# feixh/VISMA

Hardware: AMD Instinct MI355X
Metric: icp_iterations_per_sec (higher is better)
Workload: dtype f32; 1 GPU; C4 S-surf 262144->4194304, 4040 ICP iterations of a fresh registration from T=I (cold pass + warm passes), median of 1; ns=262144, nt=4194304, solver=kabsch, nn=grid, search=exact, parallelism=1 GPU, ONE persistent launch per host loop

## Files before the change

include/visma_icp_testing.h:

```cpp
#ifndef VISMA_ICP_TESTING_H
#define VISMA_ICP_TESTING_H
#include "visma_icp.h"
#ifdef __cplusplus
extern "C" {
#endif

typedef struct {
    int (*set_source)(void *user, const float *xyzw, int64_t ns);
    int (*set_target)(void *user, const float *xyzw, int64_t nt);
    int (*set_target_normals)(void *user, const float *nxyzw, int64_t nt);
    int (*nn_pass)(void *user, const double T_centred[16], double max_dist);
    int (*reduce)(void *user, const double T_centred[16], const double frame_offset[3],
                  int point_to_plane, double stats[VISMA_ICP_NSTATS]);
    int (*get_correspondences)(void *user, int32_t *tgt_idx_per_src, float *d2);
} visma_icp_engine;
VISMA_ICP_API int visma_icp_create_with_engine(visma_icp_ctx **out,
                                               const visma_icp_engine *engine,
                                               void *user);

VISMA_ICP_API int visma_icp_get_search_kernel_used(visma_icp_ctx *ctx, int *kernel);
VISMA_ICP_API int visma_icp_forget_winners(visma_icp_ctx *ctx);

VISMA_ICP_API int visma_icp_set_device_loop(visma_icp_ctx *ctx, int enabled);

VISMA_ICP_API int visma_icp_test_stall_command(visma_icp_ctx *ctx, int nth, double ms);

VISMA_ICP_API int visma_icp_get_sweep_info(visma_icp_ctx *ctx, double *launches, double *aborts);

VISMA_ICP_API int visma_icp_plan_ring_grid(const float mn[3], const float mx[3], double max_dist, double cell, int dims[3],
                                           double *cell_out, int *rings);
VISMA_ICP_API int visma_icp_ring_visiting_order(int rings, int capacity, short *dy, short *dz, float *base, int *nrows);

VISMA_ICP_API int visma_icp_get_tile_config(int *s_tile, int *t_chunk, int *block);
VISMA_ICP_API int visma_icp_get_launch_config(visma_icp_ctx *ctx, int *src_tiles,
                                              int *tgt_splits);

VISMA_ICP_API int visma_icp_last_mesh_kernel_ms(visma_icp_ctx *ctx, double *query_ms, double *build_ms);
VISMA_ICP_API int visma_icp_set_mesh_search(visma_icp_ctx *ctx, int method);

VISMA_ICP_API int visma_icp_selftest_so3(const double *w, double *R, double *w_back, int n);
VISMA_ICP_API int visma_icp_selftest_so3_jac(const double *w, int n, double *R, double *dR_dw,
                                             double *w_back, double *dw_dR, double *proj);

VISMA_ICP_API int visma_icp_selftest_se3(const double *g, const double *h, const double *v, int n,
                                         double *gh, double *gv, double *g_inv);

#ifdef __cplusplus
}
#endif
#endif
```

visma_amd/csrc/driver.cpp:

```cpp
#include "driver_ctx.hpp"
#ifdef VISMA_TEST_SEAMS
#include "../../include/visma_icp_testing.h"
#endif

namespace {

#ifdef VISMA_TEST_SEAMS
class HookEngine : public Engine {
public:
    HookEngine(const visma_icp_engine &vt, void *user) : vt_(vt), user_(user) {}
    int set_source(const float *p, int64_t n) override { ns_ = n; return wrap(vt_.set_source(user_, p, n)); }
    int set_target(const float *p, int64_t n) override { nt_ = n; has_normals_ = false; return wrap(vt_.set_target(user_, p, n)); }
    int set_target_normals(const float *p, int64_t n) override
    {
        if (!vt_.set_target_normals) { err_ = "engine has no normals support"; return VISMA_ICP_ERR_ENGINE; }
        has_normals_ = true;
        return wrap(vt_.set_target_normals(user_, p, n));
    }
    int nn_pass(const Mat4 &Tc, double r) override { return wrap(vt_.nn_pass(user_, Tc.m, r)); }
    int reduce(const Mat4 &Tc, bool plane, const double offset[3], double *st) override
    {
        const double zero[3] = {0, 0, 0};
        return wrap(vt_.reduce(user_, Tc.m, offset ? offset : zero, plane ? 1 : 0, st));
    }
    int get_correspondences(int32_t *idx, float *d2) override
    {
        std::vector<float> tmp;
        if (!d2) { tmp.resize((size_t)(ns_ > 0 ? ns_ : 1)); d2 = tmp.data(); }
        return wrap(vt_.get_correspondences(user_, idx, d2));
    }

private:
    int wrap(int rc)
    {
        if (rc == 0) return VISMA_ICP_OK;
        err_ = "engine callback returned " + std::to_string(rc);
        return VISMA_ICP_ERR_ENGINE;
    }
    visma_icp_engine vt_;
    void *user_;
};
#endif


}

namespace {

void pack_f64_to(const double *xyz, int64_t n, int stride, const double c[3], float *out, bool par)
{
    auto body = [&](int64_t ch) {
        const int64_t lo = ch * kHostChunk, hi = std::min(n, lo + kHostChunk);
        for (int64_t i = lo; i < hi; i++) {
            const double *p = xyz + (size_t)i * stride;
            out[4 * i + 0] = (float)(p[0] - c[0]);
            out[4 * i + 1] = (float)(p[1] - c[1]);
            out[4 * i + 2] = (float)(p[2] - c[2]);
            out[4 * i + 3] = 0.f;
        }
    };
    const int64_t nch = (n + kHostChunk - 1) / kHostChunk;
    if (par) parallel_for(nch, 1, body);
    else for (int64_t ch = 0; ch < nch; ch++) body(ch);
}

int pack_f64(const double *xyz, int64_t n, int stride, const double c[3], std::vector<float> &out)
{
    out.resize((size_t)(n > 0 ? n : 1) * 4);
    pack_f64_to(xyz, n, stride, c, out.data(), false);
    return 0;
}

void pack_f32_to(const float *xyz, int64_t n, int stride, float *out)
{
    for (int64_t i = 0; i < n; i++) {
        const float *p = xyz + (size_t)i * stride;
        out[4 * i + 0] = p[0];
        out[4 * i + 1] = p[1];
        out[4 * i + 2] = p[2];
        out[4 * i + 3] = 0.f;
    }
}

void centroid_f64(const double *xyz, int64_t n, int stride, double c[3], bool par)
{
    c[0] = c[1] = c[2] = 0.0;
// ... 886 lines not shown
{
    if (!(share > 0.0) || share > 1.0) return VISMA_ICP_ERR_INVALID;
    persist_cu_share_ref().store(share);
    return VISMA_ICP_OK;
}

int visma_icp_get_persistent_info(visma_icp_ctx *ctx, visma_icp_persistent_info *out)
{
    CTX_CHECK();
    if (!out || out->struct_size < (int)sizeof(visma_icp_persistent_info))
        return ctx->fail(VISMA_ICP_ERR_INVALID, "visma_icp_persistent_info: set struct_size = sizeof(visma_icp_persistent_info)");
    const int sz = out->struct_size;
    std::memset(out, 0, sizeof(*out));
    out->struct_size = sz;
    out->cu_share = 1.0;
    ctx->eng->get_persistent_info(out);
    return VISMA_ICP_OK;
}

int visma_icp_set_ring_search(visma_icp_ctx *ctx, int mode)
{
    CTX_CHECK();
    ctx->eng->set_ring_search(mode);
    return VISMA_ICP_OK;
}

int visma_icp_get_ring_search(visma_icp_ctx *ctx, int *rings, double *cell, double *occupancy)
{
    CTX_CHECK();
    ctx->eng->get_ring_search(rings, cell, occupancy);
    return VISMA_ICP_OK;
}

int visma_icp_get_sweep_info(visma_icp_ctx *ctx, double *launches, double *aborts)
{
    CTX_CHECK();
    ctx->eng->get_sweep_info(launches, aborts);
    return VISMA_ICP_OK;
}

int visma_icp_test_stall_command(visma_icp_ctx *ctx, int nth, double ms)
{
    CTX_CHECK();
    if (nth < 0 || !(ms >= 0.0) || ms > 10000.0) return ctx->fail(VISMA_ICP_ERR_INVALID, "bad stall arguments");
    ctx->eng->stall_command(nth, ms);
    return VISMA_ICP_OK;
}

int visma_icp_set_profiling(visma_icp_ctx *ctx, int enabled)
{
    CTX_CHECK();
    ctx->eng->set_profiling(enabled);
    return VISMA_ICP_OK;
}

int visma_icp_get_timing(visma_icp_ctx *ctx, visma_icp_timing *out, int reset)
{
    CTX_CHECK();
    if (!out) return ctx->fail(VISMA_ICP_ERR_INVALID, "out is NULL");
    ctx->eng->get_timing(out, reset != 0);
    return VISMA_ICP_OK;
}

int visma_icp_get_timing_sized(visma_icp_ctx *ctx, void *out, size_t struct_size, int reset)
{
    CTX_CHECK();
    if (!out) return ctx->fail(VISMA_ICP_ERR_INVALID, "out is NULL");
    visma_icp_timing t;
    ctx->eng->get_timing(&t, reset != 0);
    std::memcpy(out, &t, struct_size < sizeof(t) ? struct_size : sizeof(t));
    return VISMA_ICP_OK;
}

int visma_icp_plan_ring_grid(const float mn[3], const float mx[3], double max_dist, double cell, int dims[3], double *cell_out, int *rings)
{
    if (!mn || !mx) return VISMA_ICP_ERR_INVALID;
    const visma::GridParams g = visma::grid_plan_ring(mn, mx, max_dist, cell, visma::kGridMaxCells);
    if (dims) for (int a = 0; a < 3; a++) dims[a] = g.dim[a];
    if (cell_out) *cell_out = (double)g.h;
    if (rings) *rings = g.ring;
    return VISMA_ICP_OK;
}

int visma_icp_ring_visiting_order(int rings, int capacity, short *dy, short *dz, float *base, int *nrows)
{
    const std::vector<visma::RingRow> rows = visma::ring_visiting_order(rings);
    if (nrows) *nrows = (int)rows.size();
    if (rows.empty()) return VISMA_ICP_ERR_INVALID;
    for (int k = 0; k < (int)rows.size() && k < capacity; k++) {
        if (dy) dy[k] = rows[k].dy;
        if (dz) dz[k] = rows[k].dz;
        if (base) base[k] = rows[k].base;
    }
    return VISMA_ICP_OK;
}

int visma_icp_get_tile_config(int *s_tile, int *t_chunk, int *block)
{
    if (s_tile) *s_tile = kSTile;
    if (t_chunk) *t_chunk = kTChunk;
    if (block) *block = kBlock;
    return VISMA_ICP_OK;
}

int visma_icp_get_launch_config(visma_icp_ctx *ctx, int *src_tiles, int *tgt_splits)
{
    CTX_CHECK();
    int a = 0, b = 0;
    ctx->eng->launch_config(&a, &b);
    if (src_tiles) *src_tiles = a;
    if (tgt_splits) *tgt_splits = b;
    return VISMA_ICP_OK;
}

int visma_icp_comm_unique_id(void *out_id)
{
    if (!out_id) return VISMA_ICP_ERR_INVALID;
    if (!g_rccl.load()) { g_create_error = g_rccl.error; return VISMA_ICP_ERR_RCCL; }
    NcclId id;
    int rc = g_rccl.GetUniqueId(&id);
    if (rc != 0) { g_create_error = "ncclGetUniqueId failed"; return VISMA_ICP_ERR_RCCL; }
    std::memcpy(out_id, &id, sizeof(id));
    return VISMA_ICP_OK;
}

int visma_icp_comm_init(visma_icp_ctx *ctx, int rank, int nranks, const void *unique_id)
{
    CTX_CHECK();
    if (!unique_id || nranks < 1 || rank < 0 || rank >= nranks) return ctx->fail(VISMA_ICP_ERR_INVALID, "bad comm arguments");
    int rc = ctx->eng->comm_init(rank, nranks, unique_id);
    if (rc) return ctx->eng_fail(rc);
    ctx->rank = rank;
    ctx->nranks = nranks;
    return VISMA_ICP_OK;
}

int visma_icp_comm_ipc_export(visma_icp_ctx *ctx, void *out_handle)
{
    CTX_CHECK();
    if (!out_handle) return ctx->fail(VISMA_ICP_ERR_INVALID, "out_handle is NULL");
    int rc = ctx->eng->ipc_export(out_handle);
    if (rc) return ctx->eng_fail(rc);
    return VISMA_ICP_OK;
}

int visma_icp_comm_ipc_init(visma_icp_ctx *ctx, int rank, int nranks, const void *handles)
{
    CTX_CHECK();
    if (!handles || nranks < 1 || rank < 0 || rank >= nranks) return ctx->fail(VISMA_ICP_ERR_INVALID, "bad comm arguments");
    int rc = ctx->eng->ipc_init(rank, nranks, handles);
    if (rc) return ctx->eng_fail(rc);
    ctx->rank = rank;
    ctx->nranks = nranks;
    return VISMA_ICP_OK;
}

int visma_icp_set_allreduce(visma_icp_ctx *ctx, visma_icp_allreduce_fn fn, void *user, int rank, int nranks)
{
    CTX_CHECK();
    if (nranks < 1 || rank < 0 || rank >= nranks) return ctx->fail(VISMA_ICP_ERR_INVALID, "bad rank arguments");
    ctx->host_allreduce = fn;
    ctx->host_allreduce_user = user;
    ctx->rank = rank;
    ctx->nranks = nranks;
    return VISMA_ICP_OK;
}
// ... 46 lines not shown
```

visma_amd/csrc/grid.hip:

```cpp
#include "device_common.h"

#include <stdlib.h>
#include <algorithm>

#include <math.h>
#include <string.h>

namespace visma {

__device__ __forceinline__ unsigned f2ord(float f)
{
    const unsigned u = __float_as_uint(f);
    return (u & 0x80000000u) ? ~u : (u | 0x80000000u);
}

__global__ void bbox_init_kernel(unsigned *box)
{
    if (threadIdx.x < 3) box[threadIdx.x] = 0xFFFFFFFFu;
    else if (threadIdx.x < 6) box[threadIdx.x] = 0u;
}

__global__ __launch_bounds__(256) void bbox_kernel(const float4 *__restrict__ pts, int n,
                                                   unsigned *__restrict__ box)
{
    float mn[3] = {INFINITY, INFINITY, INFINITY}, mx[3] = {-INFINITY, -INFINITY, -INFINITY};
    for (int i = blockIdx.x * 256 + threadIdx.x; i < n; i += gridDim.x * 256) {
        const float4 q = pts[i];
        mn[0] = fminf(mn[0], q.x); mx[0] = fmaxf(mx[0], q.x);
        mn[1] = fminf(mn[1], q.y); mx[1] = fmaxf(mx[1], q.y);
        mn[2] = fminf(mn[2], q.z); mx[2] = fmaxf(mx[2], q.z);
    }
#pragma unroll
    for (int a = 0; a < 3; a++) {
#pragma unroll
        for (int off = 32; off > 0; off >>= 1) {
            mn[a] = fminf(mn[a], __shfl_down(mn[a], off, 64));
            mx[a] = fmaxf(mx[a], __shfl_down(mx[a], off, 64));
        }
    }
    __shared__ float wmn[4][3], wmx[4][3];
    const int w = threadIdx.x >> 6;
    if ((threadIdx.x & 63) == 0) {
#pragma unroll
        for (int a = 0; a < 3; a++) { wmn[w][a] = mn[a]; wmx[w][a] = mx[a]; }
    }
    __syncthreads();
    if (threadIdx.x < 3) {
        const int a = threadIdx.x;
        const float lo = fminf(fminf(wmn[0][a], wmn[1][a]), fminf(wmn[2][a], wmn[3][a]));
        const float hi = fmaxf(fmaxf(wmx[0][a], wmx[1][a]), fmaxf(wmx[2][a], wmx[3][a]));
        atomicMin(&box[a], f2ord(lo));
        atomicMax(&box[3 + a], f2ord(hi));
    }
}

__global__ __launch_bounds__(256) void cell_count_kernel(const float4 *__restrict__ pts, int n,
                                                         GridParams g,
                                                         uint2 *__restrict__ cell_rank,
                                                         unsigned *__restrict__ count)
{
    const int i = blockIdx.x * 256 + threadIdx.x;
    if (i >= n) return;
    const float4 q = pts[i];
    int cx = cell_coord(q.x, g.mn[0], g.inv_h, g.dim[0]);
    int cy = cell_coord(q.y, g.mn[1], g.inv_hs, g.dim[1]);
    int cz = cell_coord(q.z, g.mn[2], g.inv_hs, g.dim[2]);
    cx = min(max(cx, 0), g.dim[0] - 1);
    cy = min(max(cy, 0), g.dim[1] - 1);
    cz = min(max(cz, 0), g.dim[2] - 1);
    const unsigned c = (unsigned)((cz * g.dim[1] + cy) * g.dim[0] + cx);
    cell_rank[i] = make_uint2(c, atomicAdd(&count[c], 1u));
}

constexpr int kScanPerBlock = 2048;

__global__ __launch_bounds__(256) void scan_block_sum_kernel(const unsigned *__restrict__ count,
                                                             long long n,
                                                             unsigned *__restrict__ bsum)
{
    __shared__ unsigned w[4];
    const long long base = (long long)blockIdx.x * kScanPerBlock + threadIdx.x * 8;
    unsigned s = 0;
#pragma unroll
// ... 12 lines not shown
    const int per = (nb + 1023) / 1024;
    const int lo = threadIdx.x * per, hi = min(lo + per, nb);
    unsigned s = 0;
    for (int i = lo; i < hi; i++) s += bsum[i];
    part[threadIdx.x] = s;
    __syncthreads();
    for (int off = 1; off < 1024; off <<= 1) {
        unsigned v = (threadIdx.x >= off) ? part[threadIdx.x - off] : 0u;
        __syncthreads();
        part[threadIdx.x] += v;
        __syncthreads();
    }
    unsigned run = part[threadIdx.x] - s;
    for (int i = lo; i < hi; i++) {
        const unsigned v = bsum[i];
        bsum[i] = run;
        run += v;
    }
}

__global__ __launch_bounds__(256) void scan_apply_kernel(const unsigned *__restrict__ count,
                                                         long long n,
                                                         const unsigned *__restrict__ bsum,
                                                         unsigned *__restrict__ start)
{
    __shared__ unsigned tsum[256];
    const long long base = (long long)blockIdx.x * kScanPerBlock + threadIdx.x * 8;
    unsigned v[8], s = 0;
#pragma unroll
    for (int k = 0; k < 8; k++) {
        v[k] = (base + k < n) ? count[base + k] : 0u;
        s += v[k];
    }
    tsum[threadIdx.x] = s;
    __syncthreads();
    for (int off = 1; off < 256; off <<= 1) {
        unsigned t = (threadIdx.x >= off) ? tsum[threadIdx.x - off] : 0u;
        __syncthreads();
        tsum[threadIdx.x] += t;
        __syncthreads();
    }
    unsigned run = bsum[blockIdx.x] + tsum[threadIdx.x] - s;
#pragma unroll
    for (int k = 0; k < 8; k++) {
        if (base + k < n) start[base + k] = run;
        run += v[k];
    }
    if (base <= n - 1 && n - 1 < base + 8) start[n] = run;
}

__global__ void scan_total_kernel(const unsigned *__restrict__ count, long long n, unsigned *__restrict__ start)
{
    start[n] = start[n - 1] + count[n - 1];
}

__global__ __launch_bounds__(256) void cell_scatter_kernel(const float4 *__restrict__ pts, int n,
                                                           const uint2 *__restrict__ cell_rank,
                                                           const unsigned *__restrict__ start,
                                                           float4 *__restrict__ sorted,
                                                           const Pt64 *__restrict__ pts64,
                                                           Pt64 *__restrict__ sorted64)
{
    const int i = blockIdx.x * 256 + threadIdx.x;
    if (i >= n) return;
    const uint2 cr = cell_rank[i];
    const unsigned pos = start[cr.x] + cr.y;
    const float4 q = pts[i];
    sorted[pos] = make_float4(q.x, q.y, q.z, __uint_as_float((unsigned)i));
    if (pts64) {
        Pt64 q8 = pts64[i];
        q8.w = (unsigned long long)(unsigned)i;
        sorted64[pos] = q8;
    }
}

__global__ void pack12_kernel(const float4 *__restrict__ src, float *__restrict__ dst, long long n)
{
    const long long i = (long long)blockIdx.x * blockDim.x + threadIdx.x;
    if (i < n) { const float4 p = src[i]; dst[3 * i] = p.x; dst[3 * i + 1] = p.y; dst[3 * i + 2] = p.z; }
}
hipError_t launch_pack12(const float4 *src, float *dst, int64_t n, hipStream_t stream)
{
    if (n > 0) hipLaunchKernelGGL(pack12_kernel, dim3((unsigned)((n + 255) / 256)), dim3(256), 0, stream, src, dst, (long long)n);
    return hipGetLastError();
}

hipError_t launch_grid_bbox(const float4 *tgt, int64_t nt, unsigned *box6, hipStream_t stream)
{
    hipLaunchKernelGGL(bbox_init_kernel, dim3(1), dim3(64), 0, stream, box6);
    if (nt > 0) {
        int blocks = (int)((nt + 255) / 256);
        if (blocks > 1024) blocks = 1024;
        hipLaunchKernelGGL(bbox_kernel, dim3(blocks), dim3(256), 0, stream, tgt, (int)nt, box6);
    }
    return hipGetLastError();
}

void grid_decode_bbox(const unsigned box6[6], float mn[3], float mx[3])
{
    for (int a = 0; a < 6; a++) {
        const unsigned o = box6[a];
        const unsigned u = (o & 0x80000000u) ? (o & 0x7FFFFFFFu) : ~o;
        float f;
        memcpy(&f, &u, sizeof(f));
        (a < 3 ? mn[a] : mx[a - 3]) = f;
    }
}

GridParams grid_plan(const float mn[3], const float mx[3], double max_dist, int64_t max_cells, int max_sub)
{
    GridParams g;
    float h = (float)(max_dist * 1.001);
    if (const char *e = getenv("VISMA_ICP_GRID_CELL")) {
        const double f = atof(e);
        if (f >= 1.0 && f <= 64.0) h = (float)(max_dist * 1.001 * f);
    }
    if (!(h > 0.f) || !isfinite(h)) h = 1.0f;
    double ext[3];
    for (int a = 0; a < 3; a++) {
        ext[a] = (double)mx[a] - (double)mn[a];
        if (!(ext[a] >= 0.0) || !isfinite(ext[a])) ext[a] = 0.0;
    }
    for (;;) {
        double n = 1.0;
        bool too_long = false;
        for (int a = 0; a < 3; a++) {
            double d = floor(ext[a] / h) + 1.0;
            if (d > 2.0e9) d = 2.0e9;
            if (d > (double)kGridMaxDim) too_long = true;
            g.dim[a] = (int)d;
            n *= d;
        }
        if (n <= (double)max_cells && !too_long) break;
        h *= 1.26f;
    }
    g.sub = 1;
    if (max_sub >= 2) {
        const double dy = floor(ext[1] / (0.5 * h)) + 1.0, dz = floor(ext[2] / (0.5 * h)) + 1.0;
        if ((double)g.dim[0] * dy * dz <= (double)kGridMaxCellsFine) {
            g.sub = 2;
            g.dim[1] = (int)dy;
            g.dim[2] = (int)dz;
        }
    }
    for (int a = 0; a < 3; a++) g.mn[a] = mn[a];
    g.h = h;
    g.inv_h = 1.0f / h;
    g.hs = g.sub == 2 ? 0.5f * h : h;
    g.inv_hs = 1.0f / g.hs;
    g.ncell = (int64_t)g.dim[0] * g.dim[1] * g.dim[2];
    g.ring = 0;
    return g;
}

GridParams grid_plan_ring(const float mn[3], const float mx[3], double max_dist, double cell, int64_t max_cells)
{
    GridParams g = grid_plan(mn, mx, max_dist, max_cells);
    float h = (float)cell;
    if (!(h > 0.f) || !isfinite(h) || !(h < g.h)) return g;
    h = std::max(h, (float)(max_dist * 1.001 / (double)(kRingMaxRings - 2)));
    double ext[3];
    for (int a = 0; a < 3; a++) {
        ext[a] = (double)mx[a] - (double)mn[a];
        if (!(ext[a] >= 0.0) || !isfinite(ext[a])) ext[a] = 0.0;
    }
    GridParams f = g;
// ... 536 lines not shown
                    w8.w = 0xFFFFFFFFull | lbw;
                    if (bpos != 0xFFFFFFFFu) { w8 = sorted64[bpos]; w8.w = (w8.w & 0xFFFFFFFFull) | lbw; }
                    prevq_out[i] = w8;
                }
            }
            if constexpr (S64) {
#ifdef VISMA_GRID_DEBUG_TRIPS
                {
                    int wmax = dbg_trips, wmax_m = bpos == 0xFFFFFFFFu ? 0 : dbg_trips;
                    for (int m = 32; m > 0; m >>= 1) {
                        wmax = max(wmax, __shfl_xor(wmax, m, 64));
                        wmax_m = max(wmax_m, __shfl_xor(wmax_m, m, 64));
                    }
                    idx_out[i] = dbg_trips | ((bpos != 0xFFFFFFFFu) << 7) | (wmax << 8) | (wmax_m << 16);
                }
#else
                idx_out[i] = (bpos == 0xFFFFFFFFu) ? -1 : (int)bidx;
#endif
                d2_out[i] = (float)bd;
                if (d64_out) d64_out[i] = bd;
            } else {
                idx_out[i] = (bpos == 0xFFFFFFFFu) ? -1 : (int)(unsigned)bkey;
                d2_out[i] = __uint_as_float((unsigned)(bkey >> 32));
            }
        }
        if ((it % G) == sub) { keep_s = s4; keep_i = i; keep_pos = bpos; }
        if constexpr (KEEPQ) { keep_p[0] = pxd; keep_p[1] = pyd; keep_p[2] = pzd; }
        if (!ONE && (it % G) == G - 1) flush();
    }
    flush();
    block_reduce_store<NACC>(acc, partials, fold.tickets != nullptr);
    if (cand_count) {
        unsigned long long c = ncand, ca = ncand_all;
#pragma unroll
        for (int o = 32; o > 0; o >>= 1) {
            c += __shfl_down(c, o, 64);
            ca += __shfl_down(ca, o, 64);
        }
        if ((threadIdx.x & 63) == 0 && ca) {
            unsigned long long *slot = cand_count + 2 * (blockIdx.x & 4095);
            atomicAdd(slot, c);
            atomicAdd(slot + 1, ca);
        }
    }
    if (fold.tickets) fused_fold<PLANE, kBlock, false, kSolveInFold>(fold, partials, row0, lb, bpp, prob);
}

template <bool PLANE, int G, int U>
static void launch_grid_t(int nblocks, hipStream_t stream, const float4 *src, int ns,
                          const float4 *sorted, const unsigned *start, const GridParams &g,
                          const float4 *nrm, const Xform32 &T32, const Xform64 &T64,
                          const Offset64 &off, float r2f, int *idx_out, float *d2_out,
                          double *partials, unsigned long long *cand, const DevIcpState *st,
                          int nprob, long long out_stride, const Pt64 *src64, const Pt64 *sorted64, double r2d,
                          const Pt64 *nrm64, int exact, const FoldArgs &fold, double *d64_out, Pt64 *prevq_out)
{
    const long long total_groups = (long long)nblocks * (kBlock / G);
    const bool one = ((long long)ns + total_groups - 1) / total_groups <= G;
#define VISMA_GRID_LAUNCH(ONE_, F64_, HYB_)                                                                     \
    hipLaunchKernelGGL((nn_grid_reduce_kernel<PLANE, G, U, ONE_, F64_, HYB_>), dim3(nblocks * nprob),             \
                       dim3(kBlock), 0, stream, src, ns, sorted, start, g, nrm, T32, T64, off, r2f, idx_out,      \
                       d2_out, partials, cand, st, nblocks, out_stride, (const ProbDesc *)nullptr, nprob, src64,  \
                       sorted64, r2d, nrm64, fold, d64_out, prevq_out)
    if (src64 && exact) {
        if (one) VISMA_GRID_LAUNCH(true, false, true); else VISMA_GRID_LAUNCH(false, false, true);
    } else if (src64) {
        if (one) VISMA_GRID_LAUNCH(true, true, false); else VISMA_GRID_LAUNCH(false, true, false);
    } else {
        if (one) VISMA_GRID_LAUNCH(true, false, false); else VISMA_GRID_LAUNCH(false, false, false);
    }
#undef VISMA_GRID_LAUNCH
}

hipError_t launch_nn_grid_reduce(const float4 *src, int64_t ns, const float4 *sorted,
                                 const unsigned *start, const GridParams &g,
                                 const float4 *tgt_normals, const Xform32 &T32, const Xform64 &T64,
                                 const double frame_offset[3], float r2f, int point_to_plane,
                                 int32_t *idx_out, float *d2_out, double *partials,
                                 int max_partial_blocks, int *nblocks_out, int lanes_per_query,
                                 unsigned long long *cand_count, const DevIcpState *st,
                                 int nprob, int64_t out_stride, hipStream_t stream, const Pt64 *src64,
                                 const Pt64 *sorted64, double r2d, const Pt64 *nrm64, int exact,
                                 const FoldArgs *fold, double *d64_out, Pt64 *prevq_io, int warm, const Xform64 *Tprev,
                                 const PersistArgs *persist, Pt64 *ru_io, const RingTable *ring)
{
    if ((src64 == nullptr) != (sorted64 == nullptr)) return hipErrorInvalidValue;
    if (persist && !(lanes_per_query == kCoopLanes && src64 && exact && g.sub == 1 && prevq_io)) return hipErrorInvalidValue;
    Offset64 off;
    for (int a = 0; a < 3; a++) off.v[a] = frame_offset ? frame_offset[a] : 0.0;
    const FoldArgs fa = fold ? *fold : FoldArgs{};
    const int G = lanes_per_query % 100;
    int U = lanes_per_query / 100;
    if (U == 0) U = (G >= 8) ? 2 : 4;
    int64_t want = (ns * G + kBlock - 1) / kBlock;
    int nblocks = (int)(want > max_partial_blocks ? max_partial_blocks : want);
    if (nblocks < 1) nblocks = 1;
    if (g.ring > 0) {
        if (!src64 || persist || !ring) return hipErrorInvalidValue;
        hipError_t e = launch_nn_ring(G, nblocks, nprob, (int)ns, src64, sorted64, exact ? (const float *)sorted : nullptr, start, g,
                                      *ring, tgt_normals, nrm64, T64, off, r2f,
                                      point_to_plane, idx_out, d2_out, d64_out, prevq_io, warm & 1, partials, cand_count, st,
                                      (long long)out_stride, fa, stream);
        if (nblocks_out) *nblocks_out = nblocks;
        return e;
    }
    if (lanes_per_query == kCoopLanes) {
        if (src64 && exact && g.sub == 1 && prevq_io) {
            const bool one = (ns + (int64_t)nblocks * kBlock - 1) / ((int64_t)nblocks * kBlock) <= 1;
            hipError_t e = launch_nn_coop(nblocks * nprob, nblocks, nprob, nullptr, (int)ns, (const float *)sorted, start, g,
                                          tgt_normals, nrm64, T64, off, r2f, point_to_plane, one ? 1 : 0, idx_out, d2_out,
                                          partials, cand_count, st, (long long)out_stride, src64, sorted64, fa, d64_out,
                                          prevq_io, warm, stream, Tprev, persist, ru_io);
            if (nblocks_out) *nblocks_out = nblocks;
            return e;
        }
        U = 8;
    }
#define VISMA_GRID_CASE(GG, UU)                                                                    \
    if (G == GG && U == UU) {                                                                      \
        if (point_to_plane)                                                                        \
            launch_grid_t<true, GG, UU>(nblocks, stream, src, (int)ns, sorted, start, g,           \
                                        tgt_normals, T32, T64, off, r2f, idx_out, d2_out,          \
                                        partials, cand_count, st, nprob, (long long)out_stride, src64, sorted64, r2d, nrm64, exact, fa, d64_out, prevq_io);   \
        else                                                                                       \
            launch_grid_t<false, GG, UU>(nblocks, stream, src, (int)ns, sorted, start, g,          \
                                         tgt_normals, T32, T64, off, r2f, idx_out, d2_out,         \
                                         partials, cand_count, st, nprob, (long long)out_stride, src64, sorted64, r2d, nrm64, exact, fa, d64_out, prevq_io);  \
        launched = true;                                                                           \
    }
    bool launched = false;
    VISMA_GRID_CASE(1, 8) VISMA_GRID_CASE(1, 12) VISMA_GRID_CASE(2, 4) VISMA_GRID_CASE(2, 8)
    VISMA_GRID_CASE(4, 8) VISMA_GRID_CASE(8, 4)
    if (!launched) return hipErrorInvalidValue;
#undef VISMA_GRID_CASE
    if (nblocks_out) *nblocks_out = nblocks;
    return hipGetLastError();
}

template <int G, int U, bool ONE, bool F64, bool HYB, bool PLANE = false>
static void launch_grid_batch_t(int total_blocks, hipStream_t stream, const float4 *src,
                                const float4 *sorted, const unsigned *start, const ProbDesc *descs,
                                int nprob, int *idx_out, float *d2_out, double *partials,
                                const DevIcpState *st, const Pt64 *src64, const Pt64 *sorted64, const FoldArgs &fold,
                                unsigned long long *cand, const float4 *nrm = nullptr, const Pt64 *nrm64 = nullptr,
                                Pt64 *prevq_out = nullptr)
{
    const Xform32 T32{};
    const Xform64 T64{};
    const Offset64 off{};
    const GridParams g{};
    hipLaunchKernelGGL((nn_grid_reduce_kernel<PLANE, G, U, ONE, F64, HYB>), dim3(total_blocks), dim3(kBlock), 0, stream,
                       src, 0, sorted, start, g, nrm, T32, T64, off, 0.f, idx_out,
                       d2_out, partials, cand, st, 1, 0ll, descs, nprob, src64, sorted64, 0.0,
                       nrm64, fold, (double *)nullptr, prevq_out);
}

hipError_t launch_nn_grid_reduce_batch(const float4 *src, const float4 *sorted, const unsigned *start,
                                       const ProbDesc *descs, int nprob, int total_blocks,
                                       int32_t *idx_out, float *d2_out, double *partials,
                                       int lanes_per_query, int one_per_lane, const DevIcpState *st,
                                       hipStream_t stream, const Pt64 *src64, const Pt64 *sorted64, int exact,
                                       const FoldArgs *fold, unsigned long long *cand_count,
                                       const float4 *nrm, const Pt64 *nrm64, Pt64 *prevq_io, int warm)
{
    if (!st || !descs || (src64 == nullptr) != (sorted64 == nullptr)) return hipErrorInvalidValue;
    const bool plane = nrm != nullptr || nrm64 != nullptr;
    if (plane && src64 && !exact) return hipErrorInvalidValue;
    const FoldArgs fa = fold ? *fold : FoldArgs{};
    const int G = lanes_per_query % 100;
    int U = lanes_per_query / 100;
    if (lanes_per_query == kCoopLanes) {
        if (src64 && exact && prevq_io) {
            const Xform64 T64{};
            const Offset64 off{};
            const GridParams g{};
            return launch_nn_coop(total_blocks, 1, nprob, descs, 0, (const float *)sorted, start, g, nrm, nrm64, T64, off,
                                  0.f, plane ? 1 : 0, one_per_lane, idx_out, d2_out, partials, cand_count, st, 0ll, src64,
                                  sorted64, fa, nullptr, prevq_io, warm, stream);
        }
        U = 8;
    }
    bool launched = false;
#define VISMA_BATCH_ARGS total_blocks, stream, src, sorted, start, descs, nprob, idx_out, d2_out, partials, st
#define VISMA_BATCH_CASE(GG, UU)                                                                              \
    if (G == GG && U == UU && plane) {                                                                        \
        if (src64 && one_per_lane)                                                                            \
            launch_grid_batch_t<GG, UU, true, false, true, true>(VISMA_BATCH_ARGS, src64, sorted64, fa, cand_count, nrm, nrm64, prevq_io);   \
        else if (src64)                                                                                       \
            launch_grid_batch_t<GG, UU, false, false, true, true>(VISMA_BATCH_ARGS, src64, sorted64, fa, cand_count, nrm, nrm64, prevq_io);  \
        else if (one_per_lane)                                                                                \
            launch_grid_batch_t<GG, UU, true, false, false, true>(VISMA_BATCH_ARGS, nullptr, nullptr, fa, cand_count, nrm, nrm64, prevq_io); \
        else                                                                                                  \
            launch_grid_batch_t<GG, UU, false, false, false, true>(VISMA_BATCH_ARGS, nullptr, nullptr, fa, cand_count, nrm, nrm64, prevq_io); \
        launched = true;                                                                                      \
    } else if (G == GG && U == UU) {                                                                          \
// ... 23 lines not shown
```

visma_amd/csrc/grid_coop.hip:

```cpp
#include <cstdlib>

#include "device_common.h"
#include "grid_coop_probe.h"

namespace visma {

namespace {

struct P12 { float x, y, z; };
#ifndef VISMA_COOP_RU
#define VISMA_COOP_RU 0
#endif
#ifndef VISMA_COOP_CAP
#define VISMA_COOP_CAP (VISMA_COOP_RU ? 344 : 352)
#endif
constexpr bool kCoopRu = VISMA_COOP_RU != 0;
constexpr int kCoopCap = VISMA_COOP_CAP;
#ifndef VISMA_COOP_DEPTH
#define VISMA_COOP_DEPTH 7
#endif
constexpr int kCoopDepth = VISMA_COOP_DEPTH;
#ifndef VISMA_COOP_ROOM
#define VISMA_COOP_ROOM 0.04f
#endif
constexpr float kCoopRoom = VISMA_COOP_ROOM;

__device__ __forceinline__ float octet_min(float d)
{
    float r;
    asm volatile("s_nop 1\n\t"
                 "v_min_f32_dpp %0, %1, %1 quad_perm:[1,0,3,2] row_mask:0xf bank_mask:0xf\n\t"
                 "s_nop 1\n\t"
                 "v_min_f32_dpp %0, %0, %0 quad_perm:[2,3,0,1] row_mask:0xf bank_mask:0xf\n\t"
                 "s_nop 1\n\t"
                 "v_min_f32_dpp %0, %0, %0 row_half_mirror row_mask:0xf bank_mask:0xf"
                 : "=&v"(r)
                 : "v"(d));
    return r;
}

__device__ __forceinline__ unsigned pack_sec(float sec, float third, unsigned lane)
{
    if constexpr (!kCoopRu) return __float_as_uint(sec);
    return (__float_as_uint(sec) & 0xFFFF0000u) | (((__float_as_uint(third) >> 18) & 0x1FFFu) << 3) | (lane & 7u);
}
__device__ __forceinline__ float sec_of(unsigned w) { return __uint_as_float(kCoopRu ? (w & 0xFFFF0000u) : w); }
[[maybe_unused]] __device__ __forceinline__ float third_of(unsigned w) { return __uint_as_float(((w >> 3) & 0x1FFFu) << 18); }

__device__ __forceinline__ unsigned wave_scan_incl(unsigned v, int)
{
    v += (unsigned)__builtin_amdgcn_update_dpp(0, (int)v, 0x111, 0xf, 0xf, false);
    v += (unsigned)__builtin_amdgcn_update_dpp(0, (int)v, 0x112, 0xf, 0xf, false);
    v += (unsigned)__builtin_amdgcn_update_dpp(0, (int)v, 0x114, 0xf, 0xf, false);
    v += (unsigned)__builtin_amdgcn_update_dpp(0, (int)v, 0x118, 0xf, 0xf, false);
    v += (unsigned)__builtin_amdgcn_update_dpp(0, (int)v, 0x142, 0xa, 0xf, false);
    v += (unsigned)__builtin_amdgcn_update_dpp(0, (int)v, 0x143, 0xc, 0xf, false);
    return v;
}

}

struct CoopRes {
    double (*q64)[3];
    float *idx;
    float *lb;
    float *lb3;
    int first;
    double sx, sy, sz;
    int have_src;
};

template <int NTH>
__device__ __forceinline__ void coop_query_range(int ns, int bpp, int lb, int tid, int &vb, int &per_group, long long &i_begin,
                                                 long long &i_end)
{
    vb = lb;
    if ((bpp & 7) == 0) vb = (lb & 7) * (bpp >> 3) + (lb >> 3);
    const int total_groups = bpp * NTH;
    per_group = (ns + total_groups - 1) / total_groups;
    const int gid = vb * NTH + tid;
    i_begin = (long long)gid * per_group;
    i_end = i_begin + per_group < ns ? i_begin + per_group : ns;
}

template <bool PLANE, bool ONE, int NTH, bool PERSIST = false>
__device__ __forceinline__ bool coop_body(
    int ns, const float *__restrict__ s12f, const unsigned *__restrict__ start, GridParams g,
    const float4 *__restrict__ nrm, Xform64 T64, Offset64 off, float r2f, int *__restrict__ idx_out,
    float *__restrict__ d2_out, double *__restrict__ partials, unsigned long long *__restrict__ cand_count,
    const DevIcpState *__restrict__ st, int bpp, long long out_stride, const ProbDesc *__restrict__ descs,
    int nprob, const Pt64 *__restrict__ src64, const Pt64 *__restrict__ sorted64,
    const Pt64 *__restrict__ nrm64, const FoldArgs &fold, double *__restrict__ d64_out,
    Pt64 *__restrict__ wst_io, int warm, Xform64 Tprev, Pt64 *__restrict__ ru_io, unsigned *work_out = nullptr,
    const CoopRes res = CoopRes{})
{
    constexpr int NACC = Acc<PLANE>::N;
    const P12 *s12 = reinterpret_cast<const P12 *>(s12f);
    int prob, lb;
    long long row0;
    if (descs) {
        if (warm & 2) {
            prob = reinterpret_cast<const int *>(descs + nprob)[blockIdx.x];
        } else {
            int lo = 0, hi = nprob - 1;
            while (lo < hi) {
                const int mid = (lo + hi + 1) >> 1;
                if (descs[mid].first_block <= (int)blockIdx.x) lo = mid; else hi = mid - 1;
            }
            prob = lo;
        }
        const ProbDesc d = descs[prob];
        lb = (int)blockIdx.x - d.first_block;
        bpp = d.nblocks;
        src64 += d.src_off;
        ns = d.ns;
        s12 += d.sorted_off;
        sorted64 += d.sorted_off;
        if constexpr (PLANE) {
            if (nrm) nrm += d.sorted_off;
            if (nrm64) nrm64 += d.sorted_off;
        }
        row0 = d.first_block;
        start += d.start_off;
        g = d.g;
        out_stride = 0;
        idx_out += d.out_off;
        d2_out += d.out_off;
        wst_io += d.out_off;
        if (ru_io) ru_io += d.out_off;
    } else {
        prob = blockIdx.x / bpp;
        lb = blockIdx.x - prob * bpp;
        row0 = (long long)prob * bpp;
    }
    if (st) st += prob;
    {
        Xform32 T32_unused;
        if (!load_loop_state(st, T32_unused, T64, off, r2f)) return false;
        if (st) {
            warm &= ~4;
            if (st->have_prev && !(warm & 8)) {
                warm |= 4;
#pragma unroll
                for (int k = 0; k < 12; k++) Tprev.m[k] = st->Tc_prev[k];
            }
        }
        if (!(warm & 1)) warm &= ~4;
    }
    const double r2d = (double)r2f;
    COOP_PROBE_BEGIN();
    idx_out += (long long)prob * out_stride;
    d2_out += (long long)prob * out_stride;
    wst_io += (long long)prob * out_stride;
    if (ru_io) ru_io += (long long)prob * out_stride;
    double acc[NACC];
#pragma unroll
    for (int a = 0; a < NACC; a++) acc[a] = 0.0;

    const int tid = thread_number<PERSIST, NTH>(), lane = tid & 63, wave = tid >> 6;
    const int oct = lane >> 3, l8 = lane & 7;
    constexpr int NW = NTH / 64;
    constexpr unsigned kCapAll = (unsigned)(NW * kCoopCap);
    int vb, per_group;
    long long i_begin, i_end;
    coop_query_range<NTH>(ns, bpp, lb, tid, vb, per_group, i_begin, i_end);

    __shared__ float4 s_qp[NTH];
    __shared__ uint2 s_item[kCapAll];
    __shared__ unsigned s_sec[kCapAll];
    __shared__ double s_p64[NTH][3];
    __shared__ double s_q64_own[PERSIST ? 1 : NTH][3];
    __shared__ float s_dprev_own[PERSIST ? 1 : NTH];
    double (*s_q64)[3] = s_q64_own;
    float *s_dprev = s_dprev_own;
    if constexpr (PERSIST) { s_q64 = res.q64; s_dprev = res.idx; }
    __shared__ unsigned short s_home[NTH];
    __shared__ unsigned s_need[NW];
    __shared__ unsigned s_m[NW];
    __shared__ unsigned short s_queue[NW][64];

    auto emit = [&](long long i, unsigned ht, bool cert, double bd, unsigned bidx, bool found, double qx, double qy, double qz,
                    float lb_new) {
        if constexpr (PERSIST) {
            res.lb[ht] = lb_new;
            return;
        }
        const unsigned long long lbw = (unsigned long long)__float_as_uint(lb_new) << 32;
        idx_out[i] = found ? (int)bidx : -1;
        if (cert) {
            reinterpret_cast<unsigned *>(&wst_io[i].w)[1] = __float_as_uint(lb_new);
        } else {
            Pt64 o8;
            o8.x = o8.y = o8.z = __longlong_as_double(-1ll);
            o8.w = 0xFFFFFFFFull | lbw;
            if (found) { o8.x = qx; o8.y = qy; o8.z = qz; o8.w = (unsigned long long)bidx | lbw; }
            wst_io[i] = o8;
        }
        d2_out[i] = (float)bd;
        if (d64_out) d64_out[i] = bd;
    };
    auto emit_ru = [&](long long i, unsigned ht, bool have, double ux, double uy, double uz, unsigned uidx, float lb3) {
        if constexpr (kCoopRu) {
            if (!ru_io) return;
            Pt64 o8;
            o8.x = o8.y = o8.z = __longlong_as_double(-1ll);
            o8.w = ~0ull;
            if (have) { o8.x = ux; o8.y = uy; o8.z = uz; o8.w = (unsigned long long)uidx | ((unsigned long long)__float_as_uint(lb3) << 32); }
            ru_io[i] = o8;
            if constexpr (PERSIST) res.lb3[ht] = have ? lb3 : __uint_as_float(0xFFFFFFFFu);
        }
    };
    auto query_p = [&](unsigned h, double (&out)[3]) { out[0] = s_p64[h][0]; out[1] = s_p64[h][1]; out[2] = s_p64[h][2]; };
    auto moments = [&](double pxd, double pyd, double pzd, unsigned bidx, double qx, double qy, double qz) {
        double nx = 0.0, ny = 0.0, nz = 0.0;
        if (PLANE) {
            if (nrm64) { const Pt64 n8 = nrm64[bidx]; nx = n8.x; ny = n8.y; nz = n8.z; }
            else { const float4 n4 = nrm[bidx]; nx = n4.x; ny = n4.y; nz = n4.z; }
        }
        accumulate_pq_d<PLANE>(acc, pxd, pyd, pzd, qx, qy, qz, nx, ny, nz, off);
    };
    auto list_rows = [&](const float px, const float py, const float pz, const float E, const float bound0, const bool want,
                         unsigned (&xb)[9], unsigned (&xe)[9], float &lbgeo2, unsigned &looked) {
        const int cx = cell_coord(px, g.mn[0], g.inv_h, g.dim[0]);
        const int cy = cell_coord(py, g.mn[1], g.inv_hs, g.dim[1]);
        const int cz = cell_coord(pz, g.mn[2], g.inv_hs, g.dim[2]);
        const int x0 = max(cx - 1, 0), x1 = min(cx + 1, g.dim[0] - 1);
        const int span = x1 + 1 - x0;
        typedef unsigned u4a __attribute__((ext_vector_type(4), aligned(4)));
        const bool yok[3] = {cy - 1 >= 0 && cy - 1 < g.dim[1], cy >= 0 && cy < g.dim[1], cy + 1 >= 0 && cy + 1 < g.dim[1]};
        const bool zok[3] = {cz - 1 >= 0 && cz - 1 < g.dim[2], cz >= 0 && cz < g.dim[2], cz + 1 >= 0 && cz + 1 < g.dim[2]};
        const int row_c = (cz * g.dim[1] + cy) * g.dim[0] + x0, pitch_y = g.dim[0], pitch_z = g.dim[1] * g.dim[0];
        auto load_row = [&](int k, bool wanted) {
            const bool ok = wanted && span > 0 && zok[k / 3] && yok[k % 3];
            u4a v = {0u, 0u, 0u, 0u};
            if (ok) v = *reinterpret_cast<const u4a *>(reinterpret_cast<const char *>(start) + (unsigned)(row_c + (k / 3 - 1) * pitch_z + (k % 3 - 1) * pitch_y) * 4u);
            return v;
        };
        const float fx = (px - g.mn[0]) * g.inv_h - (float)cx;
        const float fy = (py - g.mn[1]) * g.inv_hs - (float)cy;
        const float fz = (pz - g.mn[2]) * g.inv_hs - (float)cz;
        const float mgn = 1e-3f + 4.0f * E * g.inv_hs;
        const float lo_x = fmaxf(fx - mgn, 0.f), hi_x = fmaxf(1.0f - fx - mgn, 0.f);
        const float lo_y = fmaxf(fy - mgn, 0.f), hi_y = fmaxf(1.0f - fy - mgn, 0.f);
// ... 153 lines not shown
                float lb3 = __uint_as_float((unsigned)(u8.w >> 32));
                if constexpr (PERSIST) { if (!res.first) lb3 = res.lb3[tid]; }
                const float t3 = (lb3 - del) * (1.0f - 2.4e-7f);
                if (ru_io && active && has_w && has_u) {
                    if (cert) {
                        if constexpr (PERSIST) res.lb3[tid] = t3;
                        else reinterpret_cast<unsigned *>(&ru_io[i].w)[1] = __float_as_uint(t3);
                    } else if (lb_old > 0.f && t3 > 0.f) {
                        const unsigned uidx = (unsigned)u8.w;
                        const double dx = u8.x - hp[0], dy = u8.y - hp[1], dz = u8.z - hp[2];
                        double d2u = dx * dx;
                        d2u += dy * dy;
                        d2u += dz * dz;
                        const bool u_wins = d2u < d2w || (d2u == d2w && uidx < widx);
                        const double dm = u_wins ? d2u : d2w, dother = u_wins ? d2w : d2u;
                        if (dm < r2d && dm < (double)t3 * (double)t3 * (1.0 - 1e-6)) {
                            cert = true;
                            const float lbn = fminf(t3, sqrtf((float)dother) * (1.0f - 1e-6f));
                            if (u_wins) {
                                const Pt64 ow = w8;
                                w8.x = u8.x; w8.y = u8.y; w8.z = u8.z;
                                w8.w = (unsigned long long)uidx | ((unsigned long long)__float_as_uint(lbn) << 32);
                                widx = uidx;
                                emit_ru(i, (unsigned)tid, true, ow.x, ow.y, ow.z, (unsigned)ow.w, t3);
                                if constexpr (!PERSIST) wst_io[i] = w8;
                            } else {
                                if constexpr (PERSIST) res.lb3[tid] = t3;
                                else reinterpret_cast<unsigned *>(&ru_io[i].w)[1] = __float_as_uint(t3);
                            }
                            emit(i, (unsigned)tid, true, dm, widx, true, w8.x, w8.y, w8.z, lbn);
                        }
                    }
                } else if (ru_io && active && cert) {
                    if constexpr (PERSIST) res.lb3[tid] = __uint_as_float(0xFFFFFFFFu);
                }
            }
        }
        const bool need = active && !cert;
        const bool cfound = cert && has_w;
        s_p64[tid][0] = hp[0]; s_p64[tid][1] = hp[1]; s_p64[tid][2] = hp[2];
        if (need) {
            const float dp = sqdist_f32(make_float4((float)w8.x, (float)w8.y, (float)w8.z, 0.f), (float)hp[0], (float)hp[1], (float)hp[2]);
            const float sq = sqrtf(dp) + kCoopRoom * sqrtf(r2f);
            s_dprev[tid] = sq * sq;
        } else {
            s_q64[tid][0] = w8.x; s_q64[tid][1] = w8.y; s_q64[tid][2] = w8.z;
            s_dprev[tid] = __uint_as_float(cfound ? widx : 0xFFFFFFFFu);
        }
        if (cand_count) {
            const unsigned cc = (unsigned)__builtin_popcountll(__builtin_amdgcn_ballot_w64(cert));
            if (lane == 0 && cc) atomicAdd(cand_count + 2 * 4096 + (blockIdx.x & 4095), (unsigned long long)cc);
        }
        const unsigned long long needers = __builtin_amdgcn_ballot_w64(need);
        const unsigned rank = (unsigned)__builtin_popcountll(needers & ((1ull << lane) - 1ull));
        if (need) s_queue[wave][rank] = (unsigned short)tid;
        if (lane == 0) s_need[wave] = (unsigned)__builtin_popcountll(needers);
        COOP_MARK(9);
        __syncthreads();
        COOP_MARK(10);
        set_phase_prio(1);
        unsigned nq_all = 0;
        unsigned home = 0;
#pragma unroll
        for (int w = 0; w < NW; w++) {
            const unsigned c = (unsigned)__builtin_amdgcn_readfirstlane((int)s_need[w]);
            if ((unsigned)tid >= nq_all && (unsigned)tid < nq_all + c) home = s_queue[w][(unsigned)tid - nq_all];
            nq_all += c;
        }
        const bool searching = (unsigned)(wave * 64) < nq_all;
        const bool sact = (unsigned)tid < nq_all;
        if (nq_all != 0u) {
            unsigned xb[9], xe[9];
            float lbgeo2 = 0.f;
            unsigned nq = 0, off_q = 0;
            if (searching) {
                s_home[tid] = (unsigned short)home;
                double hq[3];
                query_p(home, hq);
                const double pxd = hq[0], pyd = hq[1], pzd = hq[2];
                const float dprev = sact ? s_dprev[home] : __uint_as_float(~0u);
                const float px = (float)pxd, py = (float)pyd, pz = (float)pzd;
                COOP_MARK(0);
                const float rup = sqrtf(r2f) * (1.0f + 2.4e-7f);
                const float E = 2.4e-7f * (fabsf(px) + fabsf(py) + fabsf(pz) + rup) + 4.8e-7f * rup;
                const float tlim = rup + 2.0f * E;
                const float L = tlim * tlim * (1.0f + 6e-7f);
                const float W = (4.0f * E * tlim + 4.0f * E * E) * (1.0f + 1e-6f) + L * 5e-7f;
                s_qp[tid] = make_float4(px, py, pz, W);
                float bound0 = L;
                if (dprev < L) bound0 = dprev;
                unsigned looked;
                list_rows(px, py, pz, E, bound0, sact, xb, xe, lbgeo2, looked);
                asm volatile("" : "+v"(lbgeo2));
                if (cand_count) {
                    unsigned long long c = 0, ca = looked;
#pragma unroll
                    for (int k = 0; k < 9; k++) c += xe[k] - xb[k];
#pragma unroll
                    for (int o = 32; o > 0; o >>= 1) {
                        c += __shfl_down(c, o, 64);
                        ca += __shfl_down(ca, o, 64);
                    }
#ifndef VISMA_COOP_LB_PROBE
                    if (lane == 0 && ca) {
                        unsigned long long *slot = cand_count + 2 * (blockIdx.x & 4095);
                        atomicAdd(slot, c);
                        atomicAdd(slot + 1, ca);
                    }
#endif
                }
                COOP_MARK(1);
#pragma unroll
                for (int k = 0; k < 9; k++) nq += (xe[k] - xb[k] + 7u) >> 3;
                const unsigned incl = wave_scan_incl(nq, lane);
                off_q = incl - nq;
                if (lane == 63) s_m[wave] = incl;
            } else {
                if (lane == 0) s_m[wave] = 0u;
            }
            __syncthreads();
            unsigned m_all = 0;
#pragma unroll
            for (int w = 0; w < NW; w++) {
                const unsigned c = (unsigned)__builtin_amdgcn_readfirstlane((int)s_m[w]);
                if (w < wave) off_q += c;
                m_all += c;
            }
            if (work_out) *work_out = nq_all | (m_all << 12);
            float gh0 = INFINITY, gh1 = INFINITY, gh2 = INFINITY;
            float gsec = INFINITY;
            unsigned gb0 = 0xFFFFFFFFu, gb1 = 0xFFFFFFFFu, gm0 = 0u, gm1 = 0u;
            unsigned gs0 = 0x7F800000u | (0x1FE0u << 3);
            auto chunk_insert = [&](float m, unsigned b, unsigned flags, unsigned side) {
                const bool c1 = m < gh0, c2 = m < gh1;
                gh2 = __builtin_amdgcn_fmed3f(gh1, gh2, m);
                gh1 = __builtin_amdgcn_fmed3f(gh0, gh1, m);
                gh0 = fminf(gh0, m);
                gb1 = c2 ? b : gb1; gm1 = c2 ? flags : gm1;
                gb1 = c1 ? gb0 : gb1; gm1 = c1 ? gm0 : gm1;
                gb0 = c1 ? b : gb0; gm0 = c1 ? flags : gm0;
                if constexpr (kCoopRu) gs0 = c1 ? side : gs0;
            };
            for (unsigned w0 = 0; w0 < m_all; w0 += kCapAll) {
                if (searching) {
                    const unsigned own = (unsigned)tid << 4;
                    unsigned j = off_q - w0;
#pragma unroll
                    for (int k = 0; k < 9; k++) {
                        unsigned b = xb[k];
                        while (b < xe[k]) {
                            if (j < kCapAll) s_item[j] = make_uint2(b, own | (min(xe[k] - b, 8u) << 16));
                            j++;
                            b += 8u;
                        }
                    }
                    COOP_MARK(2);
                }
                __syncthreads();
                set_phase_prio(2);
                const unsigned mw = min(m_all - w0, kCapAll);
                for (unsigned tb = 0; tb < mw; tb += (unsigned)(NW * 8 * kCoopDepth)) {
                    const unsigned t = tb + (unsigned)(wave * 8 + oct);
                    P12 c4[kCoopDepth];
                    unsigned meta[kCoopDepth];
#pragma unroll
                    for (int u = 0; u < kCoopDepth; u++) {
                        const unsigned c = t + (unsigned)(u * NW * 8);
                        uint2 dsc = make_uint2(0u, 0u);
                        if (c < mw) dsc = s_item[c];
                        meta[u] = dsc.y;
                        c4[u] = *reinterpret_cast<const P12 *>(reinterpret_cast<const char *>(s12) + (((dsc.x * 3u) << 2) + (unsigned)l8 * 12u));
                    }
#pragma unroll
                    for (int u = 0; u < kCoopDepth; u++) {
                        const unsigned c = t + (unsigned)(u * NW * 8);
                        const unsigned cnt = meta[u] >> 16;
                        const float4 p = *reinterpret_cast<const float4 *>(reinterpret_cast<const char *>(s_qp) + (meta[u] & 0xFFF0u));
                        float d = sqdist_f32(make_float4(c4[u].x, c4[u].y, c4[u].z, 0.f), p.x, p.y, p.z);
                        const bool mine = (unsigned)l8 < cnt;
                        d = mine ? d : INFINITY;
                        const float m = octet_min(d);
                        const bool fl = d <= m + p.w;
                        const unsigned long long bal = __builtin_amdgcn_ballot_w64(fl);
                        const unsigned flags = (unsigned)(bal >> (oct * 8)) & 0xFFu;
                        const float dn = fl ? INFINITY : d;
                        const float sec = octet_min(dn);
                        unsigned secl = 0u;
                        float third = INFINITY;
                        if constexpr (kCoopRu) {
                            const unsigned long long bs = __builtin_amdgcn_ballot_w64(dn == sec && sec < INFINITY);
                            const unsigned b8 = (unsigned)(bs >> (oct * 8)) & 0xFFu;
                            secl = b8 ? (unsigned)__builtin_ctz(b8) : 0u;
                            third = octet_min((b8 != 0u && (unsigned)l8 == secl) ? INFINITY : dn);
                        }
                        if (l8 == 0 && mine) {
                            s_item[c].y = (__float_as_uint(m) & 0xFFFFFF00u) | flags;
                            s_sec[c] = pack_sec(sec, third, secl);
                        }
                    }
                }
                if (searching) COOP_MARK(3);
                __syncthreads();
                set_phase_prio(3);
                if (searching) {
                    for (unsigned c0 = 0; __builtin_amdgcn_ballot_w64(c0 < nq) != 0ull; c0 += 4u) {
                        uint2 r[4];
                        unsigned rs[4];
                        bool in[4];
#pragma unroll
                        for (int u = 0; u < 4; u++) {
                            const unsigned j = off_q - w0 + c0 + (unsigned)u;
                            in[u] = c0 + (unsigned)u < nq && j < kCapAll;
                            r[u] = s_item[in[u] ? j : 0u];
                            rs[u] = s_sec[in[u] ? j : 0u];
                        }
#pragma unroll
                        for (int u = 0; u < 4; u++) {
                            chunk_insert(in[u] ? __uint_as_float(r[u].y & 0xFFFFFF00u) : INFINITY, r[u].x, r[u].y & 0xFFu, rs[u]);
                            gsec = fminf(gsec, in[u] ? sec_of(rs[u]) : INFINITY);
                        }
                    }
                    COOP_MARK(4);
                }
                if (w0 + kCapAll < m_all) __syncthreads();
            }
            if constexpr (kCoopRu) __syncthreads();
            if (searching) {
                const bool need = sact, active = sact;
                float lb_new = 0.f;
                double bd = r2d;
                unsigned bidx = 0xFFFFFFFFu, bpos = 0xFFFFFFFFu;
                Pt64 bq = Pt64{0.0, 0.0, 0.0, 0ull};
                auto tail = [&](const double pxd, const double pyd, const double pzd, const float px, const float py, const float pz,
                                const float W) {
                const float rup = sqrtf(r2f) * (1.0f + 2.4e-7f);
                const float E = 2.4e-7f * (fabsf(px) + fabsf(py) + fabsf(pz) + rup) + 4.8e-7f * rup;
                const float tlim = rup + 2.0f * E;
                const float L = tlim * tlim * (1.0f + 6e-7f);
                auto rank = [&](const Pt64 &c8, unsigned pos) {
                    const double dx = c8.x - pxd, dy = c8.y - pyd, dz = c8.z - pzd;
                    double d = dx * dx;
                    d += dy * dy;
                    d += dz * dz;
                    const unsigned id = (unsigned)c8.w;
                    const bool lt = d < bd || (d == bd && id < bidx && bidx != 0xFFFFFFFFu);
                    bd = lt ? d : bd;
                    bidx = lt ? id : bidx;
                    bpos = lt ? pos : bpos;
                    bq.x = lt ? c8.x : bq.x; bq.y = lt ? c8.y : bq.y; bq.z = lt ? c8.z : bq.z; bq.w = lt ? c8.w : bq.w;
                };
                bool slow = false;
                const float g_up = gh0 * (1.0f + 6.2e-5f);
                int n = 0;
                unsigned rupos = 0xFFFFFFFFu;
                float lb3_2 = 0.f;
                if (need && gh0 < L) {
                    const float thr = g_up + W;
                    unsigned c[4] = {0u, 0u, 0u, 0u};
                    slow = gh2 <= thr;
                    auto add = [&](unsigned b, unsigned flags) {
                        while (flags) {
                            const unsigned pos = b + (unsigned)__builtin_ctz(flags);
                            flags &= flags - 1u;
                            if (n == 0) c[0] = pos; else if (n == 1) c[1] = pos; else if (n == 2) c[2] = pos; else if (n == 3) c[3] = pos;
                            else slow = true;
                            n++;
                        }
                    };
                    add(gb0, gm0);
                    if (gh1 <= thr) add(gb1, gm1);
                    if constexpr (kCoopRu) {
                        if (ru_io && n == 1 && !slow) {
                            const float secA = sec_of(gs0);
                            if (secA < INFINITY && secA <= gh1) {
                                rupos = gb0 + (gs0 & 7u);
                                lb3_2 = fminf(gh1, third_of(gs0));
                            } else if (gh1 < INFINITY && __builtin_popcount(gm1) == 1) {
                                rupos = gb1 + (unsigned)__builtin_ctz(gm1);
                                lb3_2 = fminf(gh2, gsec);
                            }
                            lb3_2 = fminf(lb3_2, lbgeo2);
                        }
                    }
                    Pt64 c8a = Pt64{0.0, 0.0, 0.0, 0ull}, c8b = c8a;
                    if (n > 0) c8a = sorted64[c[0]];
                    if (n > 1) c8b = sorted64[c[1]];
                    if (n > 0) rank(c8a, c[0]);
                    if (n > 1) rank(c8b, c[1]);
                    if (n > 2) rank(sorted64[c[2]], c[2]);
                    if (n > 3) rank(sorted64[c[3]], c[3]);
                }
                for (unsigned long long rem = __builtin_amdgcn_ballot_w64(slow); rem; rem &= rem - 1ull) {
                    const int q = (int)__builtin_ctzll(rem);
                    auto bcast_u = [&](unsigned v) { return (unsigned)__builtin_amdgcn_readlane((int)v, q); };
                    auto bcast_f = [&](float v) { return __uint_as_float(bcast_u(__float_as_uint(v))); };
                    auto bcast_d = [&](double v) {
                        const unsigned long long u = (unsigned long long)__double_as_longlong(v);
                        return __longlong_as_double((long long)(((unsigned long long)bcast_u((unsigned)(u >> 32)) << 32) | bcast_u((unsigned)u)));
                    };
                    const float qx = bcast_f(px), qy = bcast_f(py), qz = bcast_f(pz);
                    const double qxd = bcast_d(pxd), qyd = bcast_d(pyd), qzd = bcast_d(pzd);
                    const float qrup = rup, qE = bcast_f(E);
                    const float sl = fminf(sqrtf(bcast_f(g_up)), qrup) + 2.0f * qE;
                    const float Ls = sl * sl * (1.0f + 6e-7f);
                    unsigned qb[9], pre[10];
                    pre[0] = 0u;
                    {
                        unsigned sb[9], se[9], looked_unused;
                        float geo_unused;
                        list_rows(px, py, pz, E, Ls, lane == q, sb, se, geo_unused, looked_unused);
        #pragma unroll
                        for (int k = 0; k < 9; k++) {
                            qb[k] = bcast_u(sb[k]);
                            pre[k + 1] = pre[k] + (bcast_u(se[k]) - qb[k]);
                        }
                    }
                    double ld = r2d;
                    unsigned lid = 0xFFFFFFFFu, lpos = 0xFFFFFFFFu;
                    Pt64 lq = Pt64{0.0, 0.0, 0.0, 0ull};
                    for (unsigned f0 = 0; f0 < pre[9]; f0 += 128u) {
                        unsigned j[2];
                        bool in[2];
                        P12 t[2];
        #pragma unroll
                        for (int u = 0; u < 2; u++) {
                            const unsigned f = f0 + (unsigned)u * 64u + (unsigned)lane;
                            in[u] = f < pre[9];
                            unsigned jj = 0u;
        #pragma unroll
                            for (int k = 0; k < 9; k++)
                                if (f >= pre[k] && f < pre[k + 1]) jj = qb[k] + (f - pre[k]);
                            j[u] = jj;
                            t[u] = P12{0.f, 0.f, 0.f};
                            if (in[u]) t[u] = s12[jj];
                        }
                        Pt64 c8[2];
        #pragma unroll
                        for (int u = 0; u < 2; u++) {
                            in[u] = in[u] && sqdist_f32(make_float4(t[u].x, t[u].y, t[u].z, 0.f), qx, qy, qz) <= Ls;
                            c8[u] = Pt64{0.0, 0.0, 0.0, 0ull};
                            if (in[u]) c8[u] = sorted64[j[u]];
                        }
        #pragma unroll
                        for (int u = 0; u < 2; u++)
                            if (in[u]) {
                                const double dx = c8[u].x - qxd, dy = c8[u].y - qyd, dz = c8[u].z - qzd;
                                double d = dx * dx;
                                d += dy * dy;
                                d += dz * dz;
                                const unsigned id = (unsigned)c8[u].w;
                                const bool lt = d < ld || (d == ld && id < lid && lid != 0xFFFFFFFFu);
                                if (lt) { ld = d; lid = id; lpos = j[u]; lq = c8[u]; }
                            }
                    }
                    double rd = ld;
                    unsigned rid = lid;
        #pragma unroll
                    for (int o = 32; o > 0; o >>= 1) {
                        const double od = __shfl_xor(rd, o, 64);
                        const unsigned oid = (unsigned)__shfl_xor((int)rid, o, 64);
                        const bool lt = oid != 0xFFFFFFFFu && (od < rd || (od == rd && oid < rid));
                        rd = lt ? od : rd;
                        rid = lt ? oid : rid;
                    }
                    if (rid != 0xFFFFFFFFu) {
                        const unsigned long long holders = __builtin_amdgcn_ballot_w64(lid == rid && ld == rd);
                        const int wl = (int)__builtin_ctzll(holders);
                        auto from_w = [&](unsigned v) { return (unsigned)__builtin_amdgcn_readlane((int)v, wl); };
                        auto from_w64 = [&](unsigned long long u) { return ((unsigned long long)from_w((unsigned)(u >> 32)) << 32) | from_w((unsigned)u); };
                        Pt64 w8;
                        w8.x = __longlong_as_double((long long)from_w64((unsigned long long)__double_as_longlong(lq.x)));
                        w8.y = __longlong_as_double((long long)from_w64((unsigned long long)__double_as_longlong(lq.y)));
                        w8.z = __longlong_as_double((long long)from_w64((unsigned long long)__double_as_longlong(lq.z)));
                        w8.w = from_w64(lq.w);
                        const unsigned wpos = from_w(lpos);
                        if (lane == q) {
                            const bool lt = rd < bd || (rd == bd && rid < bidx && bidx != 0xFFFFFFFFu);
                            if (lt) { bd = rd; bidx = rid; bpos = wpos; bq = w8; }
                        }
                    }
                }
                if (need) {
                    float lb2 = fminf(lbgeo2, fminf(gh1, gsec));
                    if (bpos == 0xFFFFFFFFu) lb2 = fminf(lb2, gh0);
                    float lb = sqrtf(lb2) * (1.0f - 1e-6f) - 4.0f * E;
                    if (slow || n > 1) lb = 0.f;
                    lb_new = fminf(fmaxf(lb, 0.f), 3.0e38f);
#ifdef VISMA_COOP_LB_PROBE
                    if (cand_count && bpos != 0xFFFFFFFFu && !(slow || n > 1)) {
                        const float cb = fminf(gh1, gsec);
                        if (cb < lbgeo2) {
                            unsigned long long *slot = cand_count + 2 * (blockIdx.x & 4095);
                            atomicAdd(slot, (unsigned long long)((sqrtf(fminf(lbgeo2, 4.0f * r2f)) - sqrtf(cb)) * 1e6f));
                            atomicAdd(slot + 1, 1ull);
                        }
                    }
#endif
                }
                const bool found = bpos != 0xFFFFFFFFu;
                COOP_MARK(5);
                if (active) {
                    const long long i = (long long)(vb * NTH + (int)s_home[tid]) * per_group + it;
                    emit(i, (unsigned)s_home[tid], false, bd, bidx, found, bq.x, bq.y, bq.z, lb_new);
                    if constexpr (kCoopRu) {
                        const float lb3 = sqrtf(lb3_2) * (1.0f - 1e-6f) - 4.0f * E;
                        const bool have = found && rupos != 0xFFFFFFFFu && !(slow || n > 1) && lb3 > 0.f && lb_new > 0.f;
                        if (ru_io) s_item[s_home[tid]] = make_uint2(have ? rupos : 0xFFFFFFFFu, __float_as_uint(fminf(lb3, 3.0e38f)));
                    }
                }
                if (active) {
                    const unsigned h = s_home[tid];
                    const double none = __longlong_as_double(-1ll);
                    s_q64[h][0] = found ? bq.x : none; s_q64[h][1] = found ? bq.y : none; s_q64[h][2] = found ? bq.z : none;
                    s_dprev[h] = __uint_as_float(found ? bidx : 0xFFFFFFFFu);
                }
                };
                const float4 me = s_qp[tid];
                const unsigned h = s_home[tid];
                double hq[3];
                query_p(h, hq);
                tail(hq[0], hq[1], hq[2], me.x, me.y, me.z, me.w);
                COOP_MARK(11);
            }
        }
        __syncthreads();
        COOP_MARK(12);
        set_phase_prio(4);
        if constexpr (kCoopRu) {
            ru_go = false;
            if (ru_io && ((needers >> lane) & 1ull)) {
                const uint2 h = s_item[tid];
                ru_go = true;
                ru_it = it;
                ru_lb3 = __uint_as_float(h.y);
                ru_have = h.x != 0xFFFFFFFFu;
                if (ru_have) ru_pending = sorted64[h.x];
            }
        }
        {
            const unsigned pidx = __float_as_uint(s_dprev[tid]);
            if (active && pidx != 0xFFFFFFFFu) {
                double hq[3];
                query_p((unsigned)tid, hq);
                moments(hq[0], hq[1], hq[2], pidx, s_q64[tid][0], s_q64[tid][1], s_q64[tid][2]);
            }
        }
        if constexpr (!ONE) {
            ru_finish();
            __syncthreads();
        }
    };
    if constexpr (ONE) {
        round(0);
        COOP_MARK(13);
    } else {
        for (int it = 0; it < per_group; it++) round(it);
    }
    COOP_MARK(6);
    COOP_WAVE_DONE();
    bool published = false;
    if constexpr (PERSIST) {
        const unsigned tag = fold_row_tag(fold.seq);
        block_reduce_store<NACC, NW, true>(acc, partials, true, fold.rows_tagged, tag);
        ru_finish();
        COOP_MARK(7);
        published = polled_fold<PLANE, NTH>(fold, lb, bpp, tag);
    } else {
        block_reduce_store<NACC, NW, false>(acc, partials, fold.tickets != nullptr);
        if constexpr (ONE) ru_finish();
        COOP_MARK(7);
        if (fold.tickets) published = fused_fold<PLANE, NTH, false, false>(fold, partials, row0, lb, bpp, prob);
    }
    COOP_MARK(8);
    return published;
}

#define VISMA_COOP_PARAMS                                                                                         \
    int ns, const float *__restrict__ s12f, const unsigned *__restrict__ start, GridParams g,                    \
        const float4 *__restrict__ nrm, Xform64 T64, Offset64 off, float r2f, int *__restrict__ idx_out,         \
        float *__restrict__ d2_out, double *__restrict__ partials, unsigned long long *__restrict__ cand_count,  \
        const DevIcpState *__restrict__ st, int bpp, long long out_stride, const ProbDesc *__restrict__ descs,   \
        int nprob, const Pt64 *__restrict__ src64, const Pt64 *__restrict__ sorted64,                            \
        const Pt64 *__restrict__ nrm64, const FoldArgs fold, double *__restrict__ d64_out,                       \
        Pt64 *__restrict__ wst_io, int warm, Xform64 Tprev, Pt64 *__restrict__ ru_io
#define VISMA_COOP_ARGS                                                                                          \
    ns, s12f, start, g, nrm, T64, off, r2f, idx_out, d2_out, partials, cand_count, st, bpp, out_stride, descs,   \
        nprob, src64, sorted64, nrm64, fold, d64_out, wst_io, warm, Tprev, ru_io
template <bool PLANE>
__global__ __launch_bounds__(kBlock) __attribute__((amdgpu_waves_per_eu(4, 4))) void nn_coop_kernel_one(VISMA_COOP_PARAMS)
{
    (void)coop_body<PLANE, true, kBlock>(VISMA_COOP_ARGS);
}
template <bool PLANE>
__global__ __launch_bounds__(kBlock) void nn_coop_kernel_many(VISMA_COOP_PARAMS)
{
    (void)coop_body<PLANE, false, kBlock>(VISMA_COOP_ARGS);
}

__device__ __forceinline__ unsigned long long persist_wait(const PersistArgs &pa, unsigned tag, bool poller, int pass, int lane)
{
    const bool mine = lane < kPersistWords;
    unsigned long long w = 0ull;
    const bool direct = pa.direct != 0;
    if (poller && lane == 0)
        __hip_atomic_store(pa.relay + kPersistPublished, (unsigned long long)tag, __ATOMIC_RELAXED, __HIP_MEMORY_SCOPE_AGENT);
    long long t_ref = (long long)wall_clock64();
    bool published = poller;
    for (;;) {
        if (mine) {
            if (poller || direct) w = __hip_atomic_load(pa.host_cmd + lane, __ATOMIC_RELAXED, __HIP_MEMORY_SCOPE_SYSTEM);
            else w = __hip_atomic_load(pa.relay + lane, __ATOMIC_RELAXED, __HIP_MEMORY_SCOPE_AGENT);
        }
        const bool ok = !mine || (unsigned)(w >> 32) == tag;
        if (__builtin_amdgcn_ballot_w64(ok) == ~0ull) break;
        const long long now = (long long)wall_clock64();
        bool all_here = true, dead = false;
        if (!published) {
            const unsigned long long m = __hip_atomic_load(pa.relay + kPersistPublished, __ATOMIC_RELAXED, __HIP_MEMORY_SCOPE_AGENT);
            if ((unsigned)m == tag) { published = true; t_ref = now; }
            else {
                all_here = __hip_atomic_load(pa.relay + kPersistStarted, __ATOMIC_RELAXED, __HIP_MEMORY_SCOPE_AGENT) >= (unsigned long long)gridDim.x;
                dead = __hip_atomic_load(pa.relay + kPersistDead, __ATOMIC_RELAXED, __HIP_MEMORY_SCOPE_AGENT) != 0ull;
            }
        }
        const long long limit = published ? pa.wait_ticks : (!all_here ? (pa.start_ticks > 0 ? pa.start_ticks : pa.wait_ticks) : pa.hard_ticks);
        if (dead || now - t_ref > limit) {
            w = ((unsigned long long)tag << 32) | (lane == kPersistWords - 1 ? kPersistAbort : 0u);
            if (lane == 0) {
                __hip_atomic_store(pa.relay + kPersistDead, 1ull, __ATOMIC_RELAXED, __HIP_MEMORY_SCOPE_AGENT);
                __hip_atomic_store(pa.host_flag, (unsigned)pass, __ATOMIC_RELAXED, __HIP_MEMORY_SCOPE_SYSTEM);
            }
            break;
        }
#ifndef VISMA_PERSIST_SLEEP
#define VISMA_PERSIST_SLEEP 1
#endif
        if (poller) __builtin_amdgcn_s_sleep(1); else __builtin_amdgcn_s_sleep(VISMA_PERSIST_SLEEP);
    }
    if (poller && mine && !direct) __hip_atomic_store(pa.relay + lane, w, __ATOMIC_RELAXED, __HIP_MEMORY_SCOPE_AGENT);
    return w;
}

struct CoopPersistParams {
    int ns; const float *s12f; const unsigned *start; GridParams g; const float4 *nrm; Xform64 T64; Offset64 off; float r2f;
    int *idx_out; float *d2_out; double *partials; unsigned long long *cand_count; int bpp; const Pt64 *src64;
    const Pt64 *sorted64; const Pt64 *nrm64; FoldArgs fold; Pt64 *wst_io; int warm; Xform64 Tprev; PersistArgs pa;
    Pt64 *ru_io;
};

template <class T>
__device__ __forceinline__ T ld_karg(const T __attribute__((address_space(4))) *p)
{
    static_assert(sizeof(T) % 4 == 0, "words");
    constexpr int N = (int)(sizeof(T) / 4);
    union U { T v; unsigned w[N]; __device__ U() {} } u;
    typedef const unsigned __attribute__((address_space(4))) *WordPtr;
    const WordPtr pw = (WordPtr)p;
#pragma unroll
    for (int k = 0; k < N; k++) u.w[k] = pw[k];
    return u.v;
}

template <bool PLANE>
__global__ __launch_bounds__(kBlock) __attribute__((amdgpu_waves_per_eu(4, 4))) void nn_coop_kernel_persist(const CoopPersistParams P)
{
    __shared__ unsigned s_tw[2][24];
    __shared__ unsigned s_cmdw;
    __shared__ double r_q64[kBlock][3];
    __shared__ float r_idx[kBlock], r_lb[kBlock], r_lb3[kCoopRu ? kBlock : 1];
    if (threadIdx.x == 0) {
        __hip_atomic_fetch_add(P.pa.relay + kPersistStarted, 1ull, __ATOMIC_RELAXED, __HIP_MEMORY_SCOPE_AGENT);
#pragma unroll
        for (int k = 0; k < 12; k++) {
            const unsigned long long c = (unsigned long long)__double_as_longlong(P.T64.m[k]);
            const unsigned long long q = (unsigned long long)__double_as_longlong(P.Tprev.m[k]);
            s_tw[0][2 * k] = (unsigned)c; s_tw[0][2 * k + 1] = (unsigned)(c >> 32);
            s_tw[1][2 * k] = (unsigned)q; s_tw[1][2 * k + 1] = (unsigned)(q >> 32);
        }
    }
    __syncthreads();
    typedef const CoopPersistParams __attribute__((address_space(4))) *KernargPtr;
#ifndef VISMA_PERSIST_PREFETCH
#define VISMA_PERSIST_PREFETCH 1
#endif
    double nsx = 0.0, nsy = 0.0, nsz = 0.0;
    const int tag_shift = P.pa.wait_first ? 1 : 0;
    if (P.pa.wait_first) {
        const int tidx = thread_number<true>();
        if (tidx < 64) {
            const unsigned long long cw = persist_wait(P.pa, P.pa.tag0, blockIdx.x == 0, 0, tidx);
            if (tidx < 24) s_tw[0][tidx] = (unsigned)cw;
            if (tidx == kPersistWords - 1) s_cmdw = (unsigned)cw;
        }
        __syncthreads();
        if ((unsigned)__builtin_amdgcn_readfirstlane((int)s_cmdw) != kPersistGo) return;
    }
    for (int pass = 1;; pass++) {
        KernargPtr kp = (KernargPtr)__builtin_amdgcn_kernarg_segment_ptr();
        asm volatile("" : "+s"(kp));
#define VISMA_KARG(F_) ld_karg(&kp->F_)
        const unsigned long long t_begin = VISMA_KARG(pa.timeline) ? wall_clock64() : 0ull;
        unsigned work = 0u;
        const int cur = (pass - 1) & 1;
        Xform64 Tc, Tp;
#pragma unroll
        for (int k = 0; k < 12; k++) {
            const unsigned lo = (unsigned)__builtin_amdgcn_readfirstlane((int)s_tw[cur][2 * k]);
            const unsigned hi = (unsigned)__builtin_amdgcn_readfirstlane((int)s_tw[cur][2 * k + 1]);
            Tc.m[k] = __longlong_as_double((long long)(((unsigned long long)hi << 32) | lo));
            Tp.m[k] = 0.0;
        }
        if (pass == 1 || !VISMA_PERSIST_PP_LDS) {
#pragma unroll
            for (int k = 0; k < 12; k++) {
                const unsigned plo = (unsigned)__builtin_amdgcn_readfirstlane((int)s_tw[cur ^ 1][2 * k]);
                const unsigned phi = (unsigned)__builtin_amdgcn_readfirstlane((int)s_tw[cur ^ 1][2 * k + 1]);
                Tp.m[k] = __longlong_as_double((long long)(((unsigned long long)phi << 32) | plo));
            }
        }
        int w = VISMA_KARG(warm);
        if (pass > 1) { w |= 1; if (!(w & 8)) w |= 4; }
        FoldArgs f{};
        f.tickets = VISMA_KARG(fold.tickets); f.partials2 = VISMA_KARG(fold.partials2);
        f.ticket_stride = VISMA_KARG(fold.ticket_stride); f.stats_out = VISMA_KARG(fold.stats_out);
        f.stats_stride = VISMA_KARG(fold.stats_stride); f.host_out = VISMA_KARG(fold.host_out);
        f.seq = VISMA_KARG(fold.seq) + (unsigned long long)(pass - 1);
        f.ipc_n = VISMA_KARG(fold.ipc_n); f.ipc_rank = VISMA_KARG(fold.ipc_rank); f.ipc_seq_dev = VISMA_KARG(fold.ipc_seq_dev);
        f.ipc_flag = VISMA_KARG(fold.ipc_flag); f.ipc_spins = VISMA_KARG(fold.ipc_spins); f.peer_table = VISMA_KARG(fold.peer_table);
        f.rows_tagged = VISMA_KARG(fold.rows_tagged); f.rows2_tagged = VISMA_KARG(fold.rows2_tagged);
        f.dead_flag = VISMA_KARG(fold.dead_flag); f.poll_ticks = VISMA_KARG(fold.poll_ticks);
        const bool published = coop_body<PLANE, true, kBlock, true>(
            VISMA_KARG(ns), VISMA_KARG(s12f), VISMA_KARG(start), VISMA_KARG(g), VISMA_KARG(nrm), Tc, VISMA_KARG(off), VISMA_KARG(r2f),
            VISMA_KARG(idx_out), VISMA_KARG(d2_out), VISMA_KARG(partials), VISMA_KARG(cand_count), nullptr, VISMA_KARG(bpp), 0ll,
            nullptr, 1, VISMA_KARG(src64), VISMA_KARG(sorted64), VISMA_KARG(nrm64), f, nullptr, VISMA_KARG(wst_io), w, Tp,
            VISMA_KARG(ru_io), t_begin ? &work : nullptr, CoopRes{r_q64, r_idx, r_lb, r_lb3, pass == 1 ? 1 : 0, nsx, nsy, nsz,
                                                                        (VISMA_PERSIST_PREFETCH && pass > 1) ? 1 : 0});
        const PersistArgs pa = VISMA_KARG(pa);
        if (pa.timeline && pass <= pa.timeline_passes && thread_number<true>() == 0) {
            unsigned long long *slot = pa.timeline + ((unsigned long long)(pass - 1) * gridDim.x + blockIdx.x) * 2ull;
            slot[0] = t_begin;
            slot[1] = (wall_clock64() & 0xFFFFFFFFFFFull) | ((unsigned long long)work << 44);
        }
        bool last = pass >= pa.max_passes;
        nsx = nsy = nsz = 0.0;
        if (VISMA_PERSIST_PREFETCH && !last) {
            const int tidx = thread_number<true>();
            const int bpp = VISMA_KARG(bpp);
            int vb, per_group;
            long long i_begin, i_end;
            coop_query_range<kBlock>(VISMA_KARG(ns), bpp, (int)blockIdx.x % bpp, tidx, vb, per_group, i_begin, i_end);
            if (i_begin < i_end) {
                const Pt64 s8 = VISMA_KARG(src64)[i_begin];
                nsx = s8.x; nsy = s8.y; nsz = s8.z;
            }
        }
        if (!last) {
            const int tidx = thread_number<true>();
            if (tidx < 64) {
                const bool poller = __builtin_amdgcn_readfirstlane((int)published) != 0;
                const unsigned long long cw = persist_wait(pa, pa.tag0 + (unsigned)(pass - 1 + tag_shift), poller, pass, tidx);
                if (tidx < 24) s_tw[cur ^ 1][tidx] = (unsigned)cw;
                if (tidx == kPersistWords - 1) s_cmdw = (unsigned)cw;
            }
            __syncthreads();
            asm volatile("" : "+v"(nsx), "+v"(nsy), "+v"(nsz));
            const unsigned cmd = (unsigned)__builtin_amdgcn_readfirstlane((int)s_cmdw);
            last = cmd != kPersistGo;
        }
        if (last) {
            const int tidx = thread_number<true>();
            const int bpp = VISMA_KARG(bpp);
            int vb, per_group;
            long long i_begin, i_end;
            coop_query_range<kBlock>(VISMA_KARG(ns), bpp, (int)blockIdx.x % bpp, tidx, vb, per_group, i_begin, i_end);
            if (i_begin < i_end) {
                const unsigned pid = __float_as_uint(r_idx[tidx]);
                Pt64 o8;
                o8.x = r_q64[tidx][0]; o8.y = r_q64[tidx][1]; o8.z = r_q64[tidx][2];
                o8.w = (unsigned long long)pid | ((unsigned long long)__float_as_uint(r_lb[tidx]) << 32);
                float d2 = VISMA_KARG(r2f);
                if (pid != 0xFFFFFFFFu) {
                    double Tl[12];
#pragma unroll
                    for (int k = 0; k < 12; k++)
                        Tl[k] = __longlong_as_double((long long)(((unsigned long long)s_tw[cur][2 * k + 1] << 32) | s_tw[cur][2 * k]));
                    const Pt64 s8 = VISMA_KARG(src64)[i_begin];
                    const double sv[3] = {s8.x, s8.y, s8.z};
                    double hp[3];
                    se3_act(Tl, sv, hp);
                    const double dx = o8.x - hp[0], dy = o8.y - hp[1], dz = o8.z - hp[2];
                    double d = dx * dx;
                    d += dy * dy;
                    d += dz * dz;
                    d2 = (float)d;
                }
                VISMA_KARG(idx_out)[i_begin] = (int)pid;
                VISMA_KARG(d2_out)[i_begin] = d2;
                VISMA_KARG(wst_io)[i_begin] = o8;
                if constexpr (kCoopRu) {
                    Pt64 *ru = VISMA_KARG(ru_io);
                    if (ru) reinterpret_cast<unsigned *>(&ru[i_begin].w)[1] = __float_as_uint(r_lb3[tidx]);
                }
            }
            break;
        }
#undef VISMA_KARG
    }
}
#undef VISMA_COOP_PARAMS
#undef VISMA_COOP_ARGS

#define VISMA_COOP_LAUNCH(KERNEL_)                                                                               \
    hipLaunchKernelGGL(KERNEL_, dim3(total_blocks), dim3(kBlock), 0, stream, ns, s12, start, g, nrm, T64, off,   \
                       r2f, idx_out, d2_out, partials, cand_count, st, bpp, out_stride, descs, nprob, src64,     \
                       sorted64, nrm64, fold, d64_out, wst_io, warm, Tp, ru_io)

hipError_t launch_nn_coop(int total_blocks, int bpp, int nprob, const ProbDesc *descs, int ns, const float *s12,
                          const unsigned *start, const GridParams &g, const float4 *nrm, const Pt64 *nrm64,
                          const Xform64 &T64, const Offset64 &off, float r2f, int point_to_plane, int one,
                          int32_t *idx_out, float *d2_out, double *partials, unsigned long long *cand_count,
                          const DevIcpState *st, long long out_stride, const Pt64 *src64, const Pt64 *sorted64,
                          const FoldArgs &fold, double *d64_out, Pt64 *wst_io, int warm, hipStream_t stream,
                          const Xform64 *Tprev, const PersistArgs *persist, Pt64 *ru_io)
{
    if (!src64 || !sorted64 || !s12 || !wst_io) return hipErrorInvalidValue;
    if (persist) {
        if (fold.solve) return hipErrorInvalidValue;
        if (descs || nprob != 1 || !one || st || !fold.rows_tagged || !fold.rows2_tagged || !fold.dead_flag || !fold.host_out ||
            (fold.ipc_n > 1 && !fold.peer_table) || d64_out ||
            persist->max_passes < 1 || !persist->host_cmd || !persist->relay || !persist->host_flag ||
            total_blocks > coop_persist_capacity(point_to_plane))
            return hipErrorInvalidValue;
        CoopPersistParams P{};
        P.ns = ns; P.s12f = s12; P.start = start; P.g = g; P.nrm = nrm; P.T64 = T64; P.off = off; P.r2f = r2f;
        P.idx_out = idx_out; P.d2_out = d2_out; P.partials = partials; P.cand_count = cand_count; P.bpp = bpp;
        P.src64 = src64; P.sorted64 = sorted64; P.nrm64 = nrm64; P.fold = fold; P.wst_io = wst_io;
        if (Tprev) { P.Tprev = *Tprev; warm |= 4; } else warm &= ~4;
        P.warm = warm; P.pa = *persist; P.ru_io = ru_io;
        if (point_to_plane) hipLaunchKernelGGL(nn_coop_kernel_persist<true>, dim3(total_blocks), dim3(kBlock), 0, stream, P);
        else hipLaunchKernelGGL(nn_coop_kernel_persist<false>, dim3(total_blocks), dim3(kBlock), 0, stream, P);
        return hipGetLastError();
    }
    static const int forced = [] {
        const char *e = std::getenv("VISMA_ICP_COOP_KERNEL");
        return !e ? 0 : (e[0] == 'c' ? 1 : (e[0] == 'w' ? 2 : 0));
    }();
    if (forced == 2 || (forced == 0 && (descs || nprob > 1)))
        return launch_nn_wave(total_blocks, bpp, nprob, descs, ns, s12, start, g, nrm, nrm64, T64, off, r2f, point_to_plane, one,
                              idx_out, d2_out, partials, cand_count, st, out_stride, src64, sorted64, fold, d64_out, wst_io,
                              warm & (3 | 8), stream);
    if (fold.solve) return hipErrorInvalidValue;
    Xform64 Tp{};
    if (Tprev) { Tp = *Tprev; warm |= 4; } else warm &= ~4;
    if (point_to_plane) {
        if (one) VISMA_COOP_LAUNCH(nn_coop_kernel_one<true>); else VISMA_COOP_LAUNCH(nn_coop_kernel_many<true>);
    } else {
        if (one) VISMA_COOP_LAUNCH(nn_coop_kernel_one<false>); else VISMA_COOP_LAUNCH(nn_coop_kernel_many<false>);
    }
    return hipGetLastError();
}
#undef VISMA_COOP_LAUNCH

int coop_persist_capacity(int point_to_plane)
{
    static int cap[2][64];
    static bool known[2][64];
    int dev = 0;
    if (hipGetDevice(&dev) != hipSuccess || dev < 0 || dev >= 64) { (void)hipGetLastError(); return 0; }
    const int p = point_to_plane ? 1 : 0;
    if (!known[p][dev]) {
        int per_cu = 0, cus = 0;
        hipError_t e = point_to_plane
                           ? hipOccupancyMaxActiveBlocksPerMultiprocessor(&per_cu, nn_coop_kernel_persist<true>, kBlock, 0)
                           : hipOccupancyMaxActiveBlocksPerMultiprocessor(&per_cu, nn_coop_kernel_persist<false>, kBlock, 0);
        if (e == hipSuccess) e = hipDeviceGetAttribute(&cus, hipDeviceAttributeMultiprocessorCount, dev);
        if (e != hipSuccess) { (void)hipGetLastError(); per_cu = 0; cus = 0; }
        cap[p][dev] = per_cu * cus;
        known[p][dev] = true;
    }
    return cap[p][dev];
}

}
```

visma_amd/csrc/hip_engine.hpp:

```cpp
#pragma once
#include "engine.hpp"

namespace visma {
namespace drv {

class HipEngine : public Engine {
public:
    explicit HipEngine(int device) : device_(device) {}
    ~HipEngine() override
    {
        if (!inited_) { (void)hipGetLastError(); return; }
        (void)hipSetDevice(device_);
        if (sess_live_) (void)end_session();
        if (comm_) g_rccl.CommDestroy(comm_);
        for (int r = 0; r < ipc_n_; r++)
            if (r != ipc_rank_ && peers_.box[r]) (void)hipIpcCloseMemHandle(peers_.box[r]);
        free_dev(d_mbox_); free_dev(d_ipc_flag_); free_dev(d_raw_); free_dev(d_sorted12_); free_dev(bt_sorted12_);
        free_dev(d_pend_count_); free_dev(d_pend_q32_); free_dev(d_pend_q64_); free_dev(d_pend_best_); free_dev(d_pend_idx_);
        for (hipEvent_t e : ev_) (void)hipEventDestroy(e);
        free_dev(d_src_); free_dev(d_tgt_); free_dev(d_nrm_); free_dev(d_keys_); free_dev(d_gkeys_);
        free_dev(d_claim_); free_dev(d_d64_);
        free_dev(d_src64_); free_dev(d_tgt64_); free_dev(d_sorted64_); free_dev(d_nrm64_);
        for (int i = 0; i < 4; i++) if (pin_[i]) (void)hipHostFree(pin_[i]);
        free_dev(d_idx_); free_dev(d_d2_); free_dev(d_pos_); free_dev(d_ru_); free_dev(d_partials_); free_dev(d_stats_);
        if (d_vox_out_) (void)hipFree(d_vox_out_);
        free_dev(d_box_); free_dev(d_sorted_); free_dev(d_cell_of_); free_dev(d_count_); free_dev(d_occ_); free_dev(d_ring_tab_);
        free_dev(d_start_); free_dev(d_bsum_); free_dev(d_cand_); free_dev(d_state_);
        free_dev(d_partials2_); free_dev(d_tickets_); free_dev(d_tstats_); free_dev(d_second_);
        free_dev(bt_src_); free_dev(bt_idx_); free_dev(bt_d2_); free_dev(bt_pos_); free_dev(bt_tgt_); free_dev(bt_sorted_);
        free_dev(bt_nrm_); free_dev(bt_nrm64_); free_dev(bt_raw_);
        free_dev(bt_src64_); free_dev(bt_tgt64_); free_dev(bt_sorted64_);
        free_dev(bt_cell_of_); free_dev(bt_count_); free_dev(bt_start_); free_dev(bt_bsum_); free_dev(bt_descs_);
        if (h_state_) (void)hipHostFree(h_state_);
        if (h_stats_) (void)hipHostFree(h_stats_);
        if (h_cmd_ && !cmd_direct_) (void)hipHostFree(h_cmd_);
        if (d_cmd_block_) (void)hipFree(d_cmd_block_);
        if (h_flag_) (void)hipHostFree(h_flag_);
        free_dev(d_relay_); free_dev(d_timeline_); free_dev(d_peer_table_); free_dev(d_fold_tag_);
        if (d_sweep_relay_) (void)hipFree(d_sweep_relay_);
        pool_trim(0);
        if (d_raw_src_) (void)hipFree(d_raw_src_);
        if (stream_src_) (void)hipStreamDestroy(stream_src_);
        if (stream_) (void)hipStreamDestroy(stream_);
    }

    int init();

    int set_target_f64(const double *xyz, int64_t nt, int stride, double *c, bool compute_centre, bool want64) override;
    bool last_upload_f32_ = false;
    bool host_box_valid_ = false;
    float host_mn_[3] = {0, 0, 0}, host_mx_[3] = {0, 0, 0};

    int set_target_voxel_f64(const double *xyz, int64_t n, int stride, double voxel, double *c, bool compute_centre,
                             bool want64, int64_t *nt_out) override;
    int get_voxel_target(double *out, int64_t n) override
    {
        HIP_TRY(hipSetDevice(device_));
        if (n != vox_out_n_) { err_ = "no down-sampled target of that size"; return VISMA_ICP_ERR_STATE; }
        if (n > 0) HIP_TRY(hipMemcpy(out, d_vox_out_, sizeof(double) * 3 * (size_t)n, hipMemcpyDeviceToHost));
        return VISMA_ICP_OK;
    }
    double *d_vox_out_ = nullptr;
    int64_t vox_out_n_ = -1;
    int prepare_search(int64_t ns, bool want64, double max_dist) override;
    int64_t prepared_ns_ = -1;
    bool prepared_want64_ = false;
    int begin_raw_source(int64_t ns, bool want64, std::vector<int32_t> &order);
    int ensure_raw(size_t points)
    {
        if (points * 24 > raw_bytes_) {
            free_dev(d_raw_);
            int rc = pool_alloc(&d_raw_, points * 24);
            if (rc) return rc;
            raw_bytes_ = points * 24;
        }
        return VISMA_ICP_OK;
    }
    int finish_raw_source(int64_t ns, const double *c, std::vector<int32_t> &order, const void *raw = nullptr, hipStream_t st = nullptr);
    int set_source_f64(const double *xyz, int64_t ns, int stride, const double *c, bool want64,
                       std::vector<int32_t> &order) override;
    int set_source_meshes_f64(const MeshSource *meshes, int n_meshes, int quirks, unsigned long long seed, const double *c,
                              bool want64, std::vector<int32_t> &order, int64_t *ns_out) override;
    int get_mesh_source(double *out, int64_t ns) override
    {
        HIP_TRY(hipSetDevice(device_));
        if (ns != raw_source_points_ || !d_raw_) { err_ = "no mesh-sampled source of that size on this context"; return VISMA_ICP_ERR_STATE; }
        if (ns > 0) HIP_TRY(hipMemcpy(out, d_raw_, sizeof(double) * 3 * (size_t)ns, hipMemcpyDeviceToHost));
        return VISMA_ICP_OK;
    }
    int64_t raw_source_points_ = 0;
    int set_source64(const Pt64 *src) override
    {
        HIP_TRY(hipSetDevice(device_));
        free_dev(d_src64_); free_dev(d_sorted64_); free_dev(d_nrm64_);
        grid_valid_ = false;
        { int irc = invalidate_pos(); if (irc) return irc; }
        if (!src || !d_tgt64_) { err_ = "set_source64 without an f64 target"; return VISMA_ICP_ERR_STATE; }
        { int prc = pool_alloc(&d_src64_, sizeof(Pt64) * (size_t)std::max<int64_t>(ns_, 1)); if (prc) return prc; }
        if (ns_ > 0) HIP_TRY(hipMemcpyAsync(d_src64_, src, sizeof(Pt64) * ns_, hipMemcpyHostToDevice, stream_));
        HIP_TRY(hipStreamSynchronize(stream_));
        return VISMA_ICP_OK;
    }
    void *d_raw_ = nullptr;
    size_t raw_bytes_ = 0;
    void *d_sorted12_ = nullptr;
    const float4 *search_sorted() const
    {
        if (exact_ && d_src64_ && d_sorted64_ && d_sorted12_) return (const float4 *)d_sorted12_;
        return (const float4 *)d_sorted_;
    }
    int set_clouds64(const Pt64 *src, const Pt64 *tgt) override
    {
        HIP_TRY(hipSetDevice(device_));
        free_dev(d_src64_); free_dev(d_tgt64_); free_dev(d_sorted64_); free_dev(d_nrm64_);
        grid_valid_ = false;
        { int irc = invalidate_pos(); if (irc) return irc; }
        if (!src || !tgt) return VISMA_ICP_OK;
        { int prc = pool_alloc(&d_src64_, sizeof(Pt64) * (size_t)std::max<int64_t>(ns_, 1)); if (prc) return prc; }
        { int prc = pool_alloc(&d_tgt64_, sizeof(Pt64) * (size_t)std::max<int64_t>(nt_, 1)); if (prc) return prc; }
        if (ns_ > 0) HIP_TRY(hipMemcpyAsync(d_src64_, src, sizeof(Pt64) * ns_, hipMemcpyHostToDevice, stream_));
        if (nt_ > 0) HIP_TRY(hipMemcpyAsync(d_tgt64_, tgt, sizeof(Pt64) * nt_, hipMemcpyHostToDevice, stream_));
        HIP_TRY(hipStreamSynchronize(stream_));
        return VISMA_ICP_OK;
    }
    bool search_is_f64() const override { return last_mode_ == 2; }
    bool search_is_exact() const override { return last_mode_ != 0; }
    int grid_search_mode() const { return (use_grid_ && d_src64_ && d_sorted64_) ? (exact_ ? 1 : 2) : (brute_exact() ? 1 : 0); }
    bool brute_exact() const { return !use_grid_ && exact_ && d_src64_ && d_tgt64_ && !tshard_; }
    int ensure_second(int64_t ns_pad, int splits);
    void *d_pend_count_ = nullptr, *d_pend_q32_ = nullptr, *d_pend_q64_ = nullptr, *d_pend_best_ = nullptr,
         *d_pend_idx_ = nullptr;
    BruteExact bex_store_{};
    const BruteExact *bex_ptr()
    {
        if (!brute_exact()) return nullptr;
        bex_store_ = brute_ex();
        return &bex_store_;
    }
    BruteExact brute_ex() const
    {
        BruteExact e;
        e.src64 = (const Pt64 *)d_src64_;
        e.tgt64 = (const Pt64 *)d_tgt64_;
        e.nrm64 = (const Pt64 *)d_nrm64_;
        e.second = (const float *)d_second_;
        e.nt = nt_;
        e.pend = BrutePend{};
        if (d_pend_count_ && 2 * reduce_max_blocks() <= (int)partial_rows_) {
            e.pend.count = (int *)d_pend_count_;
            e.pend.q32 = (float4 *)d_pend_q32_;
            e.pend.q64 = (Pt64 *)d_pend_q64_;
            e.pend.best = (unsigned long long *)d_pend_best_;
            e.pend.best_idx = (unsigned *)d_pend_idx_;
        }
        return e;
    }
    void set_exact(bool on) override { exact_ = on; }
    int set_target_normals64(const Pt64 *n) override;

    float *staging(int slot, size_t nfloats) override
    {
        slot &= 3;
        if (pin_cap_[slot] < nfloats) {
            if (pin_[slot]) (void)hipHostFree(pin_[slot]);
            pin_[slot] = nullptr;
            pin_cap_[slot] = 0;
            const size_t want = nfloats + nfloats / 4 + 1024;
            if (hipSetDevice(device_) != hipSuccess ||
                hipHostMalloc((void **)&pin_[slot], want * sizeof(float), hipHostMallocDefault) != hipSuccess) {
                (void)hipGetLastError();
                pin_[slot] = nullptr;
                return Engine::staging(slot, nfloats);
            }
            pin_cap_[slot] = want;
        }
        return pin_[slot];
    }
    int set_source(const float *xyzw, int64_t ns) override
    {
        HIP_TRY(hipSetDevice(device_));
        int rc = ensure_source(ns);
        if (rc) return rc;
        if (ns > 0) HIP_TRY(hipMemcpyAsync(d_src_, xyzw, sizeof(float4) * ns, hipMemcpyHostToDevice, stream_));
        HIP_TRY(hipStreamSynchronize(stream_));
        return VISMA_ICP_OK;
    }
    int set_source_device(const void *d, int64_t ns) override
    {
        HIP_TRY(hipSetDevice(device_));
        int rc = ensure_source(ns);
        if (rc) return rc;
        if (ns > 0) HIP_TRY(hipMemcpyAsync(d_src_, d, sizeof(float4) * ns, hipMemcpyDeviceToDevice, stream_));
// ... 229 lines not shown
    NcclComm comm_ = nullptr;
    void *d_mbox_ = nullptr, *d_ipc_flag_ = nullptr;
    IpcPeers peers_{};
    int ipc_rank_ = 0, ipc_n_ = 0;
    unsigned long long *ipc_seq_dev() const { return reinterpret_cast<unsigned long long *>((char *)d_ipc_flag_ + 8); }
    bool tshard_ = false;
    int64_t tgt_offset_ = 0, tgt_global_ = 0, gkeys_cap_ = 0;
    void *d_gkeys_ = nullptr, *d_claim_ = nullptr, *d_d64_ = nullptr;
    int64_t d64_cap_ = 0;
    bool shard_f64_protocol() const { return tshard_ && d_src64_ && d_tgt64_ && nn_mode_ != VISMA_ICP_NN_BRUTE; }
    double *shard_d64()
    {
        if (!shard_f64_protocol()) return nullptr;
        if (ns_ > d64_cap_) {
            free_dev(d_d64_);
            if (hipMalloc(&d_d64_, sizeof(double) * std::max<int64_t>(ns_, 1)) != hipSuccess) { (void)hipGetLastError(); d_d64_ = nullptr; d64_cap_ = 0; return nullptr; }
            d64_cap_ = ns_;
        }
        return (double *)d_d64_;
    }
    std::vector<unsigned long long> h_gkeys_;
    visma_icp_minreduce_fn minreduce_ = nullptr;
    void *minreduce_user_ = nullptr;
    int nn_mode_ = VISMA_ICP_NN_AUTO;
    bool use_grid_ = false, grid_valid_ = false, grid_pending_ = false, brute_reduced_ = false;
    double grid_radius_ = 0.0;
    GridParams grid_{};
    void *d_box_ = nullptr, *d_sorted_ = nullptr, *d_cell_of_ = nullptr, *d_count_ = nullptr;
    void *d_start_ = nullptr, *d_bsum_ = nullptr, *d_cand_ = nullptr;
    void *d_state_ = nullptr;
    DevIcpState *h_state_ = nullptr;
    int state_cap_ = 0;
    size_t partial_rows_ = 0;
    void *bt_src_ = nullptr, *bt_idx_ = nullptr, *bt_d2_ = nullptr, *bt_pos_ = nullptr, *bt_tgt_ = nullptr, *bt_sorted_ = nullptr;
    void *bt_src64_ = nullptr, *bt_tgt64_ = nullptr, *bt_sorted64_ = nullptr;
    int64_t bt_src64_cap_ = 0, bt_tgt64_cap_ = 0;
    void *bt_sorted12_ = nullptr;
    int64_t bt_sorted12_cap_ = 0;
    void *bt_raw_ = nullptr;
    size_t bt_raw_bytes_ = 0;
    void *bt_nrm_ = nullptr, *bt_nrm64_ = nullptr;
    int64_t bt_nrm_cap_ = 0, bt_nrm64_cap_ = 0;
    void *bt_cell_of_ = nullptr, *bt_count_ = nullptr, *bt_start_ = nullptr, *bt_bsum_ = nullptr, *bt_descs_ = nullptr;
    int64_t bt_src_cap_ = 0, bt_tgt_cap_ = 0, bt_cell_cap_ = 0, bt_out_cap_ = 0;
    int bt_bsum_cap_ = 0;
    size_t bt_desc_cap_ = 0;
    std::vector<char> bt_desc_host_;
    int64_t view_offset_ = 0, loop_out_stride_ = 0;
    static constexpr int kGridMaxBlocks = 32768;
    double r2d_ = 0.0;
    const Pt64 *f64_src() const { return d_sorted64_ ? (const Pt64 *)d_src64_ : nullptr; }
    const Pt64 *f64_sorted() const { return d_src64_ ? (const Pt64 *)d_sorted64_ : nullptr; }
    int grid_sub_ = 1;
    int grid_blocks_env_ = 0;
    int grid_blocks() const
    {
        if (grid_blocks_env_ > 0) return grid_blocks_env_;
        if (grid_.ring > 0) return (int)std::min<int64_t>(kGridMaxBlocks, std::max<int64_t>(1024, (ns_ * (ring_lanes() - 200) + kBlock - 1) / kBlock));
        if (ns_ <= 262144) return 1024;
        return (int)std::min<int64_t>(kGridMaxBlocks, (ns_ + kBlock - 1) / kBlock);
    }
    void *d_pos_ = nullptr;
    bool pos_fresh_ = false;
    void *d_ru_ = nullptr;
    int runner_up_ = 0;
    Pt64 *ru_state() const { return runner_up_ ? (Pt64 *)d_ru_ : nullptr; }
    Xform64 prev_T_{};
    bool prev_T_valid_ = false;
    int cert_enabled_ = 1;
    const Xform64 *cert_prev() const { return (cert_enabled_ && prev_T_valid_ && pos_fresh_) ? &prev_T_ : nullptr; }
    void note_state_pass(const Xform64 &T) { prev_T_ = T; prev_T_valid_ = true; }
    int last_kernel_ = 0;
    int coop_enabled_ = 1;
    int invalidate_pos()
    {
        pos_fresh_ = false;
        prev_T_valid_ = false;
        if (d_pos_ && aux_cap_ > 0) HIP_TRY(hipMemsetAsync(d_pos_, 0xFF, sizeof(Pt64) * (size_t)aux_cap_, stream_));
        if (d_ru_ && aux_cap_ > 0) HIP_TRY(hipMemsetAsync(d_ru_, 0xFF, sizeof(Pt64) * (size_t)aux_cap_, stream_));
        return VISMA_ICP_OK;
    }
    bool coop_ok() const
    {
        return coop_enabled_ && exact_ && d_src64_ && d_sorted64_ && d_sorted12_ && d_pos_ && grid_.sub == 1 && grid_.ring == 0 &&
               (nt_ + kSortedSlack) * 12 < (1ll << 32);
    }
    int pass_kernel(int lanes) const { return grid_.ring > 0 ? 3 : ((lanes == kCoopLanes && coop_ok()) ? 2 : 1); }
    int pass_lanes(int nprob = 1) const
    {
        if (grid_.ring > 0) return ring_lanes();
        if (grid_lanes_ > 0) return grid_lanes_;
        if (coop_ok() && pos_fresh_) return kCoopLanes;
        if (nprob == 1 && cold_in_launch_ && ns_ >= cold_in_launch_min_ns_ && loop_scope_ && loop_budget_ >= 2 && coop_ok() &&
            persist_static_ok())
            return kCoopLanes;
        return grid_lanes(nprob);
    }
    int cold_in_launch_ = 0;
    int64_t cold_in_launch_min_ns_ = 131072;
    int grid_lanes_ = 0;
    int ring_lanes_ = 8;
    bool ring_lanes_auto_ = true;
    double ring_lanes_t84_ = 1.6, ring_lanes_t42_ = 0.8;
    int ring_lanes() const { return 200 + ((ring_lanes_auto_ && !pos_fresh_) ? 8 : ring_lanes_); }
    void note_ring_stats(const double *stats)
    {
        if (!ring_lanes_auto_ || grid_.ring <= 0) return;
        ring_lanes_ = 8;
        if (stats[0] > 0.0 && stats[1] >= 0.0 && loop_scope_) {
            const double cells = std::sqrt(stats[1] / stats[0]) / (double)grid_.h;
            ring_lanes_ = cells < ring_lanes_t42_ ? 2 : (cells < ring_lanes_t84_ ? 4 : 8);
            while (ring_lanes_ < 8 && ns_ * ring_lanes_ < 8192 * 64) ring_lanes_ *= 2;
        }
    }
    int ring_mode_ = -1;
    double ring_occ_min_ = 48.0, ring_occ_target_ = 8.0;
    double ring_occ_min_single_ = 20.0;
    bool caller_sweep_ = false, ring_for_sweep_ = false;
    int ring_flips_ = 0;
    double ring_threshold() const { return (caller_sweep_ || ring_flips_ >= 3) ? ring_occ_min_ : std::min(ring_occ_min_single_, ring_occ_min_); }
    bool ring_replan_needed() const
    {
        if (ring_mode_ != -1 || !(grid_occupancy_ > 0.0) || ring_flips_ >= 3) return false;
        if (!(grid_occupancy_ >= ring_occ_min_single_ && grid_occupancy_ < ring_occ_min_)) return false;
        return ring_for_sweep_ != caller_sweep_;
    }
    void *d_occ_ = nullptr, *d_ring_tab_ = nullptr;
    int ring_tab_rings_ = 0;
    RingTable ring_tab_{nullptr, 0};
    static int nrows_of_rings(int rings) { return (2 * rings + 1) * (2 * rings + 1); }
    const RingTable *ring_table() const { return grid_.ring > 0 ? &ring_tab_ : nullptr; }
    double grid_occupancy_ = 0.0;
    int grid_lanes(int nprob = 1) const
    {
        if (grid_.ring > 0) return ring_lanes();
        if (grid_lanes_ > 0) return grid_lanes_;
        const int64_t q = ns_ * (int64_t)nprob;
        if (f64_src() && exact_)
            return nprob > 1 ? (q <= 32768 ? 408 : (q <= 98304 ? 402 : 801))
                             : (q <= 32768 ? 804 : (q <= 98304 ? 802 : (q <= 196608 ? 1201 : 801)));
        if (f64_src())
            return q <= 32768 ? 408 : (nprob > 1 ? 402 : (q <= 131072 ? 802 : 801));
        if (nprob > 1) return q <= 32768 ? 804 : 402;
        return ns_ <= 32768 ? 804 : (ns_ <= 98304 ? 802 : 1201);
    }
    int64_t sorted_cap_ = 0, cell_cap_ = 0;

    bool exact_ = true;
    int tile_enabled_ = 0;
    int fused_fold_ = 1;
    int tile_config_ = -1;
    int tile_fallback_ = 0;
    int tile_fused_fold_ = 1;
    void *d_partials2_ = nullptr, *d_tickets_ = nullptr, *d_tstats_ = nullptr;
    size_t tickets_cap_ = 0;
    Xform64 T64_last_{};
    void *d_second_ = nullptr;
    size_t second_bytes_ = 0;
    int last_mode_ = 0;
    bool use_tile() const
    {
#ifdef VISMA_WITH_TILE
        return tile_enabled_ && use_grid_ && exact_ && d_src64_ && d_sorted64_ && grid_.sub == 1 && grid_.ring == 0 && !tshard_;
#else
        return false;
#endif
    }
// ... 140 lines not shown
```

visma_amd/csrc/hip_engine_clouds.cpp:

```cpp
#include "hip_engine.hpp"

namespace visma {
namespace drv {

int HipEngine::init()
{
    int count = 0;
    if (hipGetDeviceCount(&count) != hipSuccess || count <= 0) {
        err_ = "no HIP device visible (this library has no CPU fallback)";
        return VISMA_ICP_ERR_NO_DEVICE;
    }
    if (device_ < 0 || device_ >= count) {
        err_ = "device index out of range";
        return VISMA_ICP_ERR_INVALID;
    }
    HIP_TRY(hipSetDevice(device_));
    hipDeviceProp_t prop;
    HIP_TRY(hipGetDeviceProperties(&prop, device_));
    if (std::strncmp(prop.gcnArchName, "gfx950", 6) != 0) {
        err_ = std::string("device is ") + prop.gcnArchName + ", this build targets gfx950 only";
        return VISMA_ICP_ERR_NO_DEVICE;
    }
    HIP_TRY(hipStreamCreateWithFlags(&stream_, hipStreamNonBlocking));
    HIP_TRY(hipStreamCreateWithFlags(&stream_src_, hipStreamNonBlocking));
    if (const char *e = std::getenv("VISMA_ICP_UPLOAD_OVERLAP")) upload_overlap_ = std::atoi(e) != 0;
    if (const char *e = std::getenv("VISMA_ICP_GRID_SUB")) {
        const int v = std::atoi(e);
        if (v == 1 || v == 2) grid_sub_ = v;
    }
    if (const char *e = std::getenv("VISMA_ICP_GRID_BLOCKS")) {
        const int v = std::atoi(e);
        if (v >= 1 && v <= kGridMaxBlocks) grid_blocks_env_ = v;
    }
    HIP_TRY(hipMalloc(&d_partials_, sizeof(double) * kReduceAcc * kGridMaxBlocks));
    partial_rows_ = (size_t)kGridMaxBlocks;
    HIP_TRY(hipMalloc(&d_stats_, sizeof(double) * kNStats));
    HIP_TRY(hipMalloc(&d_cand_, 3 * 4096 * sizeof(unsigned long long)));
    HIP_TRY(hipMemset(d_cand_, 0, 3 * 4096 * sizeof(unsigned long long)));
    if (const char *e = std::getenv("VISMA_ICP_COOP")) coop_enabled_ = std::atoi(e) != 0;
    if (const char *e = std::getenv("VISMA_ICP_CERT")) cert_enabled_ = std::atoi(e) != 0;
    if (const char *e = std::getenv("VISMA_ICP_RUNNER_UP")) runner_up_ = std::atoi(e) != 0;
    if (const char *e = std::getenv("VISMA_ICP_GRID_LANES")) {
        const int v = std::atoi(e);
        if (v > 0) grid_lanes_ = v;
    }
    if (const char *e = std::getenv("VISMA_ICP_TILE")) tile_enabled_ = std::atoi(e) != 0;
    if (const char *e = std::getenv("VISMA_ICP_TILE_CONFIG")) { const int v = std::atoi(e); if (v >= 0 && v <= 10) tile_config_ = v; }
    if (const char *e = std::getenv("VISMA_ICP_TILE_FALLBACK")) tile_fallback_ = std::atoi(e) != 0;
    if (const char *e = std::getenv("VISMA_ICP_TILE_FOLD")) tile_fused_fold_ = std::atoi(e) != 0;
    if (const char *e = std::getenv("VISMA_ICP_FUSED_FOLD")) fused_fold_ = std::atoi(e) != 0;
    if (const char *e = std::getenv("VISMA_ICP_SOLVE_IN_FOLD")) solve_in_fold_ = std::atoi(e) != 0;
    HIP_TRY(hipHostMalloc(&h_stats_, sizeof(double) * 2 * kNStats,
                          hipHostMallocMapped | hipHostMallocCoherent));
    std::memset(h_stats_, 0, sizeof(double) * 2 * kNStats);
    HIP_TRY(hipHostGetDevicePointer((void **)&h_stats_dev_, h_stats_, 0));
    if (const char *e = std::getenv("VISMA_ICP_PERSIST")) persist_enabled_ = std::atoi(e) != 0;
    if (const char *e = std::getenv("VISMA_ICP_PERSIST_EARLY")) persist_early_ = std::atoi(e) != 0;
    if (const char *e = std::getenv("VISMA_ICP_SWEEP_PERSIST")) sweep_persist_ = std::atoi(e) != 0;
    if (const char *e = std::getenv("VISMA_ICP_RING")) ring_mode_ = std::atoi(e) > 0 ? 1 : 0;
    if (const char *e = std::getenv("VISMA_ICP_RING_LANES")) { const int v = std::atoi(e); if (v == 1 || v == 2 || v == 4 || v == 8) { ring_lanes_ = v; ring_lanes_auto_ = false; } }
    if (const char *e = std::getenv("VISMA_ICP_RING_T84")) { const double v = std::atof(e); if (v >= 0.0) ring_lanes_t84_ = v; }
    if (const char *e = std::getenv("VISMA_ICP_RING_T42")) { const double v = std::atof(e); if (v >= 0.0) ring_lanes_t42_ = v; }
    if (const char *e = std::getenv("VISMA_ICP_RING_OCCUPANCY")) { const double v = std::atof(e); if (v >= 1.0) ring_occ_min_ = v; }
    if (const char *e = std::getenv("VISMA_ICP_RING_TARGET")) { const double v = std::atof(e); if (v >= 1.0 && v <= 1024.0) ring_occ_target_ = v; }
    if (const char *e = std::getenv("VISMA_ICP_PERSIST_RANKS")) persist_ranks_ = std::atoi(e) != 0;
    if (const char *e = std::getenv("VISMA_ICP_COLD_IN_LAUNCH")) cold_in_launch_ = std::atoi(e) != 0;
    if (const char *e = std::getenv("VISMA_ICP_COLD_IN_LAUNCH_MIN_NS")) cold_in_launch_min_ns_ = std::max<long long>(0, std::atoll(e));
    if (const char *e = std::getenv("VISMA_ICP_PERSIST_TIMEOUT_MS")) { const double v = std::atof(e); if (v >= 1.0 && v <= 5000.0) persist_timeout_ms_ = v; }
    if (const char *e = std::getenv("VISMA_ICP_PERSIST_PRIO")) { const int v = std::atoi(e); if (v >= 0 && v <= 2) persist_prio_ = v; }
    if (const char *e = std::getenv("VISMA_ICP_PERSIST_START_MS")) { const double v = std::atof(e); if (v >= 0.0 && v <= 5000.0) persist_start_ms_ = v; }
    if (const char *e = std::getenv("VISMA_ICP_PERSIST_TIMELINE")) timeline_path_ = e;
    {
        int large_bar = 0;
        if (hipDeviceGetAttribute(&large_bar, hipDeviceAttributeIsLargeBar, device_) != hipSuccess) { (void)hipGetLastError(); large_bar = 0; }
        const char *e = std::getenv("VISMA_ICP_PERSIST_CMD");
        const bool want_direct = e ? (e[0] == 'd') : large_bar != 0;
        if (want_direct && large_bar &&
            hipExtMallocWithFlags(&d_cmd_block_, sizeof(unsigned long long) * 64, hipDeviceMallocFinegrained) == hipSuccess) {
            HIP_TRY(hipMemset(d_cmd_block_, 0, sizeof(unsigned long long) * 64));
            HIP_TRY(hipDeviceSynchronize());
            h_cmd_ = h_cmd_dev_ = (unsigned long long *)d_cmd_block_;
            cmd_direct_ = true;
        } else {
// ... 453 lines not shown
        free_dev(d_idx_); free_dev(d_d2_); free_dev(d_pos_); free_dev(d_ru_);
        HIP_TRY(hipMalloc(&d_idx_, sizeof(int32_t) * (ns_pad > 0 ? ns_pad : 1)));
        HIP_TRY(hipMalloc(&d_d2_, sizeof(float) * (ns_pad > 0 ? ns_pad : 1)));
        HIP_TRY(hipMalloc(&d_pos_, sizeof(Pt64) * (ns_pad > 0 ? ns_pad : 1)));
        if (runner_up_) HIP_TRY(hipMalloc(&d_ru_, sizeof(Pt64) * (ns_pad > 0 ? ns_pad : 1)));
        aux_cap_ = ns_pad;
        return invalidate_pos();
    }
    return VISMA_ICP_OK;
}

int HipEngine::choose_mode(double max_dist)
{
    if (nn_mode_ == VISMA_ICP_NN_BRUTE || nt_ == 0) { use_grid_ = false; return VISMA_ICP_OK; }
    {
        int rc = ensure_f64_views();
        if (rc) return rc;
    }
    if (grid_valid_ && grid_radius_ == max_dist && ring_replan_needed()) {
        ring_flips_++;
        grid_valid_ = false;
    }
    if (!(grid_valid_ && grid_radius_ == max_dist)) {
        int rc = build_grid(max_dist);
        if (rc) return rc;
    }
    if (nn_mode_ == VISMA_ICP_NN_GRID) { use_grid_ = true; return VISMA_ICP_OK; }
    use_grid_ = grid_.ncell >= 512;
    if (shard_f64_protocol()) use_grid_ = true;
    if (!use_grid_ && d_src64_ && d_tgt64_ && (double)ns_ * (double)nt_ <= 2.0e8) use_grid_ = true;
    return VISMA_ICP_OK;
}

int HipEngine::build_grid(double max_dist)
{
    int e0 = -1;
    if (profiling_) { e0 = next_event_pair(); HIP_TRY(hipEventRecord(ev_[e0], stream_)); }
    float mn[3], mx[3];
    static const bool check_box = std::getenv("VISMA_ICP_CHECK_BOX") != nullptr;
    if (!host_box_valid_ || check_box) {
        if (!d_box_) HIP_TRY(hipMalloc(&d_box_, sizeof(unsigned) * 8));
        HIP_TRY(launch_grid_bbox((const float4 *)d_tgt_, nt_, (unsigned *)d_box_, stream_));
        unsigned box[6];
        HIP_TRY(hipMemcpyAsync(box, d_box_, sizeof(box), hipMemcpyDeviceToHost, stream_));
        HIP_TRY(hipStreamSynchronize(stream_));
        grid_decode_bbox(box, mn, mx);
        if (host_box_valid_ && (std::memcmp(mn, host_mn_, sizeof(mn)) != 0 || std::memcmp(mx, host_mx_, sizeof(mx)) != 0)) {
            err_ = "bounding box from the staging pass differs from the device's";
            return VISMA_ICP_ERR_ENGINE;
        }
    } else {
        std::memcpy(mn, host_mn_, sizeof(mn));
        std::memcpy(mx, host_mx_, sizeof(mx));
    }
    grid_ = grid_plan(mn, mx, max_dist, kGridMaxCells, grid_sub_);
    grid_occupancy_ = 0.0;
    auto build = [&]() -> int {
        if ((int64_t)nt_ > sorted_cap_) {
            free_dev(d_sorted_); free_dev(d_cell_of_);
            HIP_TRY(hipMalloc(&d_sorted_, sizeof(float4) * (nt_ + kSortedSlack)));
            HIP_TRY(hipMalloc(&d_cell_of_, 2 * sizeof(unsigned) * nt_));
            sorted_cap_ = nt_;
        }
        if (grid_.ncell + 1 > cell_cap_) {
            free_dev(d_count_); free_dev(d_start_); free_dev(d_bsum_);
            HIP_TRY(hipMalloc(&d_count_, sizeof(unsigned) * (grid_.ncell + 1)));
            HIP_TRY(hipMalloc(&d_start_, sizeof(unsigned) * (grid_.ncell + 8)));
            HIP_TRY(hipMemsetAsync(d_start_, 0, sizeof(unsigned) * (grid_.ncell + 8), stream_));
            HIP_TRY(hipMalloc(&d_bsum_, sizeof(unsigned) * (grid_scan_blocks(grid_.ncell) + 1)));
            cell_cap_ = grid_.ncell + 1;
        }
        free_dev(d_sorted64_);
        if (d_tgt64_ && d_src64_) { int prc = pool_alloc(&d_sorted64_, sizeof(Pt64) * (size_t)std::max<int64_t>(nt_, 1)); if (prc) return prc; }
        HIP_TRY(launch_grid_build((const float4 *)d_tgt_, nt_, grid_, (unsigned *)d_cell_of_,
                                  (unsigned *)d_count_, (unsigned *)d_bsum_, (unsigned *)d_start_,
                                  (float4 *)d_sorted_, stream_, d_sorted64_ ? (const Pt64 *)d_tgt64_ : nullptr,
                                  (Pt64 *)d_sorted64_));
        free_dev(d_sorted12_);
        if (d_sorted64_) {
            int prc = pool_alloc(&d_sorted12_, sizeof(float) * 3 * (size_t)(nt_ + kSortedSlack));
            if (prc) return prc;
            HIP_TRY(launch_pack12((const float4 *)d_sorted_, (float *)d_sorted12_, nt_, stream_));
        }
        return VISMA_ICP_OK;
    };
    {
        int brc = build();
        if (brc) return brc;
    }
    const bool ring_possible = ring_mode_ != 0 && d_tgt64_ && d_src64_ && nt_ > 0 && grid_sub_ <= 1 && grid_.sub == 1 &&
                               nn_mode_ != VISMA_ICP_NN_BRUTE;
    const double occ_guess = (double)nt_ / (double)std::max<int64_t>(grid_.ncell, 1) *
                             (double)std::max(grid_.dim[0], std::max(grid_.dim[1], grid_.dim[2]));
    ring_for_sweep_ = caller_sweep_;
    if (ring_possible && (ring_mode_ > 0 || occ_guess >= ring_occ_min_)) {
        if (!d_occ_) HIP_TRY(hipMalloc(&d_occ_, sizeof(unsigned long long)));
        HIP_TRY(hipMemsetAsync(d_occ_, 0, sizeof(unsigned long long), stream_));
        HIP_TRY(launch_count_occupied((const unsigned *)d_count_, grid_.ncell, (unsigned long long *)d_occ_, stream_));
        unsigned long long occupied = 0ull;
        HIP_TRY(hipMemcpyAsync(&occupied, d_occ_, sizeof(occupied), hipMemcpyDeviceToHost, stream_));
        HIP_TRY(hipStreamSynchronize(stream_));
        grid_occupancy_ = occupied ? (double)nt_ / (double)occupied : 0.0;
        if (grid_occupancy_ > ring_occ_target_ && (ring_mode_ > 0 || grid_occupancy_ >= ring_threshold())) {
            const double cell = (double)grid_.h * std::sqrt(ring_occ_target_ / grid_occupancy_);
            const GridParams fine = grid_plan_ring(mn, mx, max_dist, cell, kGridMaxCells);
            if (fine.ring > 0) {
                if (!d_ring_tab_ || ring_tab_rings_ != fine.ring) {
                    free_dev(d_ring_tab_);
                    ring_tab_rings_ = 0;
                    int nrows = 0;
                    HIP_TRY(build_ring_table(fine.ring, &d_ring_tab_, &nrows));
                    ring_tab_rings_ = fine.ring;
                }
                grid_ = fine;
                ring_tab_ = RingTable{(const RingRow *)d_ring_tab_, nrows_of_rings(fine.ring)};
                int brc = build();
                if (brc) return brc;
            }
        }
    }
    if (profiling_) { HIP_TRY(hipEventRecord(ev_[e0 + 1], stream_)); pending_.push_back({e0, 2}); }
    grid_valid_ = true;
    grid_radius_ = max_dist;
    return invalidate_pos();
}

int HipEngine::collect_timing()
{
    for (const auto &p : pending_) {
        float ms = 0.f;
        HIP_TRY(hipEventElapsedTime(&ms, ev_[p.first], ev_[p.first + 1]));
        if (p.second == 0) { timing_.nn_ms += ms; timing_.nn_launches++; }
        else if (p.second == 1) { timing_.reduce_ms += ms; timing_.reduce_launches++; }
        else { timing_.aux_ms += ms; timing_.aux_launches++; }
    }
    pending_.clear();
    for (const auto &p : sess_pending_) {
        float ms = 0.f;
        HIP_TRY(hipEventElapsedTime(&ms, ev_[p.first], ev_[p.first + 1]));
        timing_.nn_ms += ms;
        timing_.nn_launches += p.second;
        timing_.persist_ms += ms;
        timing_.persist_launches += 1.0;
        timing_.persist_passes += (double)p.second;
    }
    sess_pending_.clear();
    ev_used_ = 0;
    return VISMA_ICP_OK;
}

int HipEngine::ensure_tile_buffers(size_t rows, size_t ticket_words)
{
    if (rows > partial_rows_) {
        free_dev(d_partials_);
        HIP_TRY(hipMalloc(&d_partials_, sizeof(double) * kReduceAcc * rows));
        partial_rows_ = rows;
    }
    if (ticket_words > tickets_cap_) {
        free_dev(d_partials2_); free_dev(d_tickets_);
        HIP_TRY(hipMalloc(&d_partials2_, sizeof(double) * kReduceAcc * ticket_words));
        HIP_TRY(hipMalloc(&d_tickets_, sizeof(unsigned) * ticket_words));
        HIP_TRY(hipMemsetAsync(d_tickets_, 0, sizeof(unsigned) * ticket_words, stream_));
        tickets_cap_ = ticket_words;
    }
    if (!d_tstats_) {
        HIP_TRY(hipMalloc(&d_tstats_, sizeof(unsigned long long) * 24 * 512));
// ... 25 lines not shown
```

visma_amd/csrc/hip_engine_passes.cpp:

```cpp
#include "hip_engine.hpp"

#if defined(__x86_64__) || defined(_M_X64)
#include <immintrin.h>
#define VISMA_STORE_FENCE() _mm_sfence()
#else
#define VISMA_STORE_FENCE() std::atomic_thread_fence(std::memory_order_seq_cst)
#endif

namespace visma {
namespace drv {

int HipEngine::nn_pass(const Mat4 &Tc, double max_dist)
{
    HIP_TRY(hipSetDevice(device_));
    if (!d_src_ || !d_tgt_) { err_ = "clouds not set"; return VISMA_ICP_ERR_STATE; }
    last_was_batch_ = false;
    if (sess_live_ && (float)(max_dist * max_dist) != sess_r2f_) {
        int rc = end_session();
        if (rc) return rc;
    }
    const int64_t ns_min_pad = ((ns_ + kBlock - 1) / kBlock) * kBlock;
    for (int i = 0; i < 12; i++) { T32_.m[i] = (float)Tc.m[i]; T64_last_.m[i] = Tc.m[i]; }
    r2f_ = (float)(max_dist * max_dist);
    r2d_ = (double)r2f_;
// ... 221 lines not shown
        seen = all_tagged();
        if (!seen) {
            timing_.persist_aborts += 1.0; persist_aborts_total_ += 1.0;
            if (trace_persist())
                std::fprintf(stderr, "[visma_icp] persistent launch gave up: pass %d of %d, its flag %u, tag %u (first %u)\n", sess_pass_, sess_max_,
                             *reinterpret_cast<volatile unsigned *>(h_flag_), cmd_tag_, sess_tag0_);
            finish_session();
            persist_cooldown_ = kPersistCooldownLoops;
            in_session = false;
            if (d_tickets_ && tickets_cap_ > 0) HIP_TRY(hipMemsetAsync(d_tickets_, 0, sizeof(unsigned) * tickets_cap_, stream_));
            { int irc = invalidate_pos(); if (irc) return irc; }
            int nblocks = 1;
            int rc = launch_grid_pass(T64, plane, offset, seq, false, nullptr, &nblocks, &ipc_done);
            if (rc) return rc;
            seen = wait_published();
        }
    }
    if (in_session && seen && posted) note_state_pass(T64);
    if (!in_session && seen && sess_live_ && sess_early_) t_stats_seen_ = std::chrono::steady_clock::now();
    if (in_session && seen) {
        const auto now = std::chrono::steady_clock::now();
        if (posted && trace_persist()) wait_us_ += std::chrono::duration<double, std::micro>(now - t_posted_).count();
        t_stats_seen_ = now;
    }
    if (in_session && seen && sess_live_ && sess_pass_ >= sess_max_) finish_session();
    if (!seen) {
        HIP_TRY(hipStreamSynchronize(stream_));
        if (!all_tagged()) {
            int flag = 0;
            if (d_ipc_flag_) (void)hipMemcpy(&flag, d_ipc_flag_, sizeof(int), hipMemcpyDeviceToHost);
            err_ = flag ? "all-reduce: rank " + std::to_string(flag - 1) + " never delivered its statistics"
                        : std::string("statistics were not published");
            return VISMA_ICP_ERR_HIP;
        }
    }
    std::atomic_thread_fence(std::memory_order_acquire);
    for (int i = 0; i < kNStats; i++) {
        const unsigned long long v = g[2 * i];
        std::memcpy(&stats[i], &v, sizeof(double));
    }
    note_ring_stats(stats);
    return sess_live_ ? VISMA_ICP_OK : maybe_collect_timing();
}

int HipEngine::launch_grid_pass(const Xform64 &T64, bool plane, const double offset[3], unsigned long long seq, bool prof,
                                const PersistArgs *persist, int *nblocks_out, bool *ipc_done, bool early)
{
    const bool ipc = ipc_n_ > 1;
    double *pub = (comm_ || ipc) ? nullptr : h_stats_dev_;
    const bool fused = fused_fold_ && !tshard_;
    const int lanes = pass_lanes();
    int nblocks = 1, e0 = -1;
    FoldArgs fa{};
    if (fused) {
        int rc = make_fold(grid_launch_blocks(ns_, lanes, grid_blocks()), 1, (double *)d_stats_, 0,
                           ipc ? h_stats_dev_ : pub, seq, &fa);
        if (rc) return rc;
        if (ipc) { add_ipc(&fa); *ipc_done = true; }
        if (persist) {
            constexpr size_t kRows = 2048, kGroups = (kRows + kFoldGroup - 1) / kFoldGroup, kRowBytes = 32 * 16;
            static_assert(kFoldGroup >= 1 && kGroups <= kRows, "group rows of the polled fold");
            if (!d_fold_tag_) {
                HIP_TRY(hipMalloc(&d_fold_tag_, (kRows + kGroups) * kRowBytes));
                HIP_TRY(hipMemsetAsync(d_fold_tag_, 0, (kRows + kGroups) * kRowBytes, stream_));
            }
            if ((size_t)grid_launch_blocks(ns_, lanes, grid_blocks()) > kRows) { err_ = "persistent launch larger than its fold rows"; return VISMA_ICP_ERR_STATE; }
            if (seq % kFoldTagPeriod + (unsigned long long)persist->max_passes >= kFoldTagPeriod)
                HIP_TRY(hipMemsetAsync(d_fold_tag_, 0, (kRows + kGroups) * kRowBytes, stream_));
            fa.rows_tagged = d_fold_tag_;
            fa.rows2_tagged = (char *)d_fold_tag_ + kRows * kRowBytes;
            fa.dead_flag = (unsigned long long *)d_relay_ + kPersistDead;
            fa.poll_ticks = persist->hard_ticks;
        }
    }
    if (prof) { e0 = next_event_pair(); HIP_TRY(hipEventRecord(ev_[e0], stream_)); }
    HIP_TRY(launch_nn_grid_reduce((const float4 *)d_src_, ns_, search_sorted(),
                                  (const unsigned *)d_start_, grid_, (const float4 *)d_nrm_,
                                  T32_, T64, offset, r2f_, plane ? 1 : 0, (int32_t *)d_idx_,
                                  (float *)d_d2_, (double *)d_partials_, grid_blocks(),
                                  &nblocks, lanes,
                                  prof ? (unsigned long long *)d_cand_ : nullptr, nullptr,
                                  1, 0, stream_, f64_src(), f64_sorted(), r2d_, (const Pt64 *)d_nrm64_,
                                  exact_ ? 1 : 0, fused ? &fa : nullptr, shard_d64(), (Pt64 *)d_pos_, 1 | (persist ? persist_prio_ << 5 : 0), cert_prev(), persist, ru_state(),
                                  ring_table()));
    if (!early) {
        last_kernel_ = pass_kernel(lanes);
        pos_fresh_ = d_pos_ != nullptr;
        note_state_pass(T64);
    }
    if (prof) {
        HIP_TRY(hipEventRecord(ev_[e0 + 1], stream_));
        if (persist) sess_e0_ = e0;
        else pending_.push_back({e0, 0});
    }
    if (!tshard_ && !fused) {
        if (prof) { e0 = next_event_pair(); HIP_TRY(hipEventRecord(ev_[e0], stream_)); }
        HIP_TRY(launch_finalize((const double *)d_partials_, nblocks, plane ? 1 : 0,
                                (double *)d_stats_, stream_, pub, seq));
        if (prof) { HIP_TRY(hipEventRecord(ev_[e0 + 1], stream_)); pending_.push_back({e0, 1}); }
    }
    *nblocks_out = nblocks;
    return VISMA_ICP_OK;
}

namespace {
std::atomic<int> g_persist_slot[64];
}

bool HipEngine::persist_possible(int lanes, int nblocks, bool fused, bool plane) const
{
    static const bool trace = std::getenv("VISMA_ICP_PERSIST_TRACE") != nullptr;
    auto no = [&](const char *why) {
        if (trace) std::fprintf(stderr, "[visma_icp] no persistent launch: %s\n", why);
        return false;
    };
    if (!persist_enabled_) return no("switched off");
    if (persist_cooldown_ > 0) return no("cooling down after a launch that gave up");
    if (!fused || tshard_ || comm_ || minreduce_ || (ipc_n_ > 1 && !persist_ranks_ok())) return no("sharded ranks / fold in a second launch");
    if (lanes != kCoopLanes || !coop_ok()) return no("not a pass of the certificate kernel");
    if (grid_lanes_ > 0 && grid_lanes_ != kCoopLanes) return no("lanes forced");
    if (std::getenv("VISMA_ICP_COOP_KERNEL")) return no("kernel forced");
    if ((int64_t)nblocks * kBlock < ns_) return no("several queries per lane");
    const int cap = coop_persist_capacity(plane ? 1 : 0);
    persist_slots_seen_ = cap;
    const int allowed = (int)((double)cap * persist_cu_share());
    if (trace) std::fprintf(stderr, "[visma_icp] persistent launch: %d workgroups, device holds %d, this process may hold %d\n", nblocks, cap, allowed);
    return nblocks <= allowed;
}

void HipEngine::fill_persist_args(PersistArgs *pa)
{
    pa->host_cmd = h_cmd_dev_;
    pa->relay = (unsigned long long *)d_relay_;
    pa->direct = cmd_direct_ ? 1 : 0;
    pa->host_flag = h_flag_dev_;
    pa->max_passes = sess_max_;
    pa->tag0 = sess_tag0_;
    pa->wait_ticks = (long long)(4.0 * persist_timeout_ms_ * 1e5) + 1000000ll;
    pa->hard_ticks = 60ll * 100000000ll;
    pa->start_ticks = (long long)(persist_start_ms_ * 1e5);
}

int HipEngine::start_session(const Xform64 &, bool plane, const double offset[3], unsigned long long seq, int, bool prof)
{
    if (device_ < 0 || device_ >= 64) return VISMA_ICP_OK;
    int expect = 0;
    if (!g_persist_slot[device_].compare_exchange_strong(expect, 1)) return VISMA_ICP_OK;
    sess_dev_slot_ = device_;
    sess_live_ = true;
    sess_pass_ = 0;
    sess_max_ = std::min(loop_budget_, 1 << 20);
    sess_tag0_ = cmd_tag_ + 1u;
    if (sess_tag0_ == 0u || sess_tag0_ + (unsigned)sess_max_ < sess_tag0_) { cmd_tag_ = 0u; sess_tag0_ = 1u; }
    cmd_tag_ = sess_tag0_ - 1u;
    sess_seq0_ = seq;
    sess_plane_ = plane;
    sess_prof_ = prof;
    sess_r2f_ = r2f_;
    for (int a = 0; a < 3; a++) sess_off_[a] = offset[a];
    sess_e0_ = -1;
    *reinterpret_cast<volatile unsigned *>(h_flag_) = 0u;
    return VISMA_ICP_OK;
}

void HipEngine::post_command(const Xform64 &T64, unsigned cmd)
{
    const unsigned tag = ++cmd_tag_;
    volatile unsigned long long *c = h_cmd_;
    const unsigned long long t = (unsigned long long)tag << 32;
    for (int k = 0; k < 12; k++) {
        unsigned long long b;
        std::memcpy(&b, &T64.m[k], sizeof(b));
        c[2 * k] = (b & 0xFFFFFFFFull) | t;
        c[2 * k + 1] = (b >> 32) | t;
    }
    c[kPersistWords - 1] = (unsigned long long)cmd | t;
    std::atomic_thread_fence(std::memory_order_release);
    if (cmd_direct_) VISMA_STORE_FENCE();
}

void HipEngine::finish_session()
{
    if (!sess_live_) return;
    sess_live_ = false;
    sess_early_ = false;
    if (host_gaps_ > 0) {
        std::fprintf(stderr, "[visma_icp] persistent launch: %d passes; host: statistics seen -> command posted %.2f us, command posted -> statistics seen %.2f us (averages)\n",
                     sess_pass_, host_gap_us_ / host_gaps_, wait_us_ / host_gaps_);
        host_gap_us_ = wait_us_ = 0.0;
        host_gaps_ = 0;
    }
    if (d_timeline_ && timeline_passes_ > 0 && !timeline_path_.empty()) {
        if (hipStreamSynchronize(stream_) == hipSuccess) {
            const size_t n = (size_t)2 * timeline_passes_ * timeline_blocks_;
            std::vector<unsigned long long> buf(n + 3);
            buf[0] = (unsigned long long)timeline_passes_; buf[1] = (unsigned long long)timeline_blocks_; buf[2] = (unsigned long long)sess_pass_;
            if (hipMemcpy(buf.data() + 3, d_timeline_, n * sizeof(unsigned long long), hipMemcpyDeviceToHost) == hipSuccess)
                if (FILE *f = std::fopen(timeline_path_.c_str(), "ab")) { std::fwrite(buf.data(), sizeof(unsigned long long), buf.size(), f); std::fclose(f); }
        }
        (void)hipGetLastError();
        timeline_passes_ = 0;
    }
    if (sess_e0_ >= 0) sess_pending_.push_back({sess_e0_, std::max(sess_pass_, 1)});
    sess_e0_ = -1;
    if (sess_dev_slot_ >= 0) g_persist_slot[sess_dev_slot_].store(0);
    sess_dev_slot_ = -1;
}

int HipEngine::end_session()
{
    if (!sess_live_) return VISMA_ICP_OK;
    if ((sess_pass_ >= 1 || sess_early_) && sess_pass_ < sess_max_) {
        Xform64 none{};
        post_command(none, kPersistStop);
    }
    hipError_t e = hipStreamSynchronize(stream_);
    finish_session();
    if (e != hipSuccess) { err_ = std::string("persistent launch: ") + hipGetErrorString(e); (void)hipGetLastError(); return VISMA_ICP_ERR_HIP; }
    return VISMA_ICP_OK;
}

int HipEngine::get_correspondences(int32_t *idx, float *d2)
{
    HIP_TRY(hipSetDevice(device_));
    if (sess_live_) { int src = end_session(); if (src) return src; }
    if (!have_pass_) { err_ = "no nn_pass yet"; return VISMA_ICP_ERR_STATE; }
#ifdef VISMA_WITH_TILE
    if (use_grid_ && grid_pending_ && use_tile()) {
        const int cfg = tile_config(ns_);
        const int nblocks = tile_blocks(ns_, cfg);
        int rc = ensure_tile_buffers((size_t)nblocks, 1);
        if (rc) return rc;
        TileArgs ta = tile_args(T64_last_, nullptr, false);
        ta.bpp = nblocks;
        HIP_TRY(launch_nn_tile_reduce(ta, 0, cfg, nblocks, stream_));
        grid_pending_ = false;
    } else
#endif
    if (use_grid_ && grid_pending_) {
        const Xform64 T64 = T64_last_;
        int nblocks = 1;
        HIP_TRY(launch_nn_grid_reduce((const float4 *)d_src_, ns_, search_sorted(),
                                      (const unsigned *)d_start_, grid_, (const float4 *)d_nrm_,
                                      T32_, T64, nullptr, r2f_, 0, (int32_t *)d_idx_,
                                      (float *)d_d2_, (double *)d_partials_, reduce_max_blocks(),
                                      &nblocks, (last_kernel_ = pass_kernel(pass_lanes()), pass_lanes()), nullptr, nullptr, 1, 0, stream_,
                                      f64_src(), f64_sorted(), r2d_, (const Pt64 *)d_nrm64_, exact_ ? 1 : 0,
                                      nullptr, nullptr, (Pt64 *)d_pos_, 1, cert_prev(), nullptr, ru_state(), ring_table()));
        pos_fresh_ = d_pos_ != nullptr;
        note_state_pass(T64);
        grid_pending_ = false;
    } else if (!use_grid_ && !brute_reduced_) {
        const Xform64 T64 = T64_last_;
        HIP_TRY(launch_reduce((const float4 *)d_src_, ns_, (const float4 *)d_tgt_,
                              (const float4 *)d_nrm_, (const unsigned long long *)d_keys_,
                              plan_.tgt_splits, ns_pad_, T32_, T64, nullptr, r2f_, 0,
                              (int32_t *)d_idx_, (float *)d_d2_, (double *)d_partials_,
                              reduce_max_blocks(), (double *)d_stats_, nullptr, nullptr, stream_, nullptr, 0, bex_ptr()));
        brute_reduced_ = true;
    }
    HIP_TRY(hipStreamSynchronize(stream_));
    if (ns_ > 0) {
        HIP_TRY(hipMemcpy(idx, (int32_t *)d_idx_ + view_offset_, sizeof(int32_t) * ns_, hipMemcpyDeviceToHost));
        if (d2) HIP_TRY(hipMemcpy(d2, (float *)d_d2_ + view_offset_, sizeof(float) * ns_, hipMemcpyDeviceToHost));
    }
    return VISMA_ICP_OK;
}

int HipEngine::run_loop(const LoopParams &lp, const Mat4 *Tc0s, int nprob, LoopResult *out)
{
    HIP_TRY(hipSetDevice(device_));
    if (sess_live_) { int src = end_session(); if (src) return src; }
    if (nprob < 1) { err_ = "nprob < 1"; return VISMA_ICP_ERR_INVALID; }
    if (!d_src_ || !d_tgt_) { err_ = "clouds not set"; return VISMA_ICP_ERR_STATE; }
    if (ring_lanes_auto_) ring_lanes_ = 8;
    last_was_batch_ = false;
    if (lp.plane && !d_nrm_) { err_ = "point-to-plane needs target normals"; return VISMA_ICP_ERR_STATE; }
    caller_sweep_ = nprob > 1;
    int rc = choose_mode(lp.max_dist);
    if (rc) return rc;
    if (nprob > 1 && !use_grid_ && nn_mode_ == VISMA_ICP_NN_AUTO && grid_valid_ && nt_ > 0) use_grid_ = true;
    r2f_ = (float)(lp.max_dist * lp.max_dist);
    r2d_ = (double)r2f_;
    for (int i = 0; i < 12; i++) T32_.m[i] = (float)lp.Tc0.m[i];
    if (nprob > 1 && (!use_grid_ || comm_ || ipc_n_ > 1)) {
        err_ = "batched loop needs the grid search on a single GPU";
        return VISMA_ICP_ERR_STATE;
    }
    if (tshard_ && !(shard_loop_on_device() && use_grid_)) {
        err_ = "the device loop of a target shard needs the library's RCCL communicator, f64 clouds and the grid search";
        return VISMA_ICP_ERR_STATE;
    }
    const int64_t ns_rounded = ((ns_ + kBlock - 1) / kBlock) * kBlock;
    view_offset_ = 0;
    loop_out_stride_ = ns_rounded;
    last_mode_ = grid_search_mode();
    if (use_grid_) {
        rc = ensure_aux(ns_rounded * nprob);
        if (rc) return rc;
        const size_t rows = (size_t)reduce_max_blocks() * nprob;
        if (rows > partial_rows_) {
            free_dev(d_partials_);
            HIP_TRY(hipMalloc(&d_partials_, sizeof(double) * kReduceAcc * rows));
            partial_rows_ = rows;
        }
    } else {
        plan_ = nn_plan(ns_, nt_pad_);
        ns_pad_ = (int64_t)plan_.src_tiles * kBlock * plan_.spt;
        const size_t need = sizeof(unsigned long long) * (size_t)ns_pad_ * plan_.tgt_splits;
        if (need > keys_bytes_) {
            free_dev(d_keys_);
            HIP_TRY(hipMalloc(&d_keys_, need));
            keys_bytes_ = need;
        }
        rc = ensure_aux(ns_pad_);
        if (rc) return rc;
        if (brute_exact()) { rc = ensure_second(ns_pad_, plan_.tgt_splits); if (rc) return rc; }
    }
    if (nprob > state_cap_) {
        free_dev(d_state_);
        if (h_state_) { (void)hipHostFree(h_state_); h_state_ = nullptr; }
        HIP_TRY(hipMalloc(&d_state_, sizeof(DevIcpState) * nprob));
        HIP_TRY(hipHostMalloc((void **)&h_state_, sizeof(DevIcpState) * nprob, hipHostMallocDefault));
        state_cap_ = nprob;
    }
    for (int b = 0; b < nprob; b++) {
        DevIcpState &h = h_state_[b];
        std::memset(&h, 0, sizeof(h));
        const Mat4 &T0 = Tc0s ? Tc0s[b] : lp.Tc0;
        for (int i = 0; i < 12; i++) h.Tc[i] = T0.m[i];
        for (int a = 0; a < 3; a++) h.centre[a] = lp.centre[a];
// ... 24 lines not shown
            const int cap = nn_wave_sweep_capacity();
            int expect = 0;
            if ((int64_t)nb * kBlock >= ns_ && (int64_t)nb * nprob <= (int64_t)((double)cap * persist_cu_share()) &&
                g_persist_slot[device_].compare_exchange_strong(expect, 1)) {
                struct SlotGuard { int d; ~SlotGuard() { g_persist_slot[d].store(0); } } guard{device_};
                if (nprob > sweep_relay_cap_) {
                    if (d_sweep_relay_) (void)hipFree(d_sweep_relay_);
                    d_sweep_relay_ = nullptr; sweep_relay_cap_ = 0;
                    HIP_TRY(hipMalloc(&d_sweep_relay_, sizeof(unsigned long long) * (32 * (size_t)nprob + 8)));
                    sweep_relay_cap_ = nprob;
                    sweep_tag_ = 0;
                }
                const int rem = lp.passes - done;
                if (sweep_tag_ == 0u || sweep_tag_ + (unsigned)rem + 2u < sweep_tag_) {
                    HIP_TRY(hipMemsetAsync(d_sweep_relay_, 0, sizeof(unsigned long long) * (32 * (size_t)sweep_relay_cap_ + 8), stream_));
                    sweep_tag_ = 1u;
                }
                unsigned long long *dead = (unsigned long long *)d_sweep_relay_ + 32 * (size_t)sweep_relay_cap_;
                HIP_TRY(hipMemsetAsync(dead, 0, sizeof(unsigned long long), stream_));
                FoldArgs fa{};
                rc = make_fold(nb, nprob, st->stats, (long long)(sizeof(DevIcpState) / sizeof(double)), nullptr, 0, &fa);
                if (rc) return rc;
                SweepArgs sa{};
                sa.relay = (unsigned long long *)d_sweep_relay_;
                sa.dead = dead;
                sa.max_passes = rem;
                sa.tag0 = sweep_tag_;
                sa.passes0 = done;
                sa.wait_ticks = (long long)(50.0 * 1e5);
                sweep_tag_ += (unsigned)rem + 1u;
                int e0 = -1;
                if (profiling_) { e0 = next_event_pair(); HIP_TRY(hipEventRecord(ev_[e0], stream_)); }
                HIP_TRY(launch_nn_wave_sweep(nb, nprob, (int)ns_, (const float *)d_sorted12_, (const unsigned *)d_start_, grid_, r2f_,
                                             (int32_t *)d_idx_, (float *)d_d2_, (double *)d_partials_,
                                             profiling_ ? (unsigned long long *)d_cand_ : nullptr, st, loop_out_stride_,
                                             (const Pt64 *)d_src64_, (const Pt64 *)d_sorted64_, fa, (Pt64 *)d_pos_, sa, stream_));
                if (profiling_) { HIP_TRY(hipEventRecord(ev_[e0 + 1], stream_)); pending_.push_back({e0, 0}); }
                last_kernel_ = 2;
                pos_fresh_ = d_pos_ != nullptr;
                prev_T_valid_ = false;
                unsigned long long dead_h = 0ull;
                HIP_TRY(hipMemcpyAsync(h_state_, d_state_, sizeof(DevIcpState) * nprob, hipMemcpyDeviceToHost, stream_));
                HIP_TRY(hipMemcpyAsync(&dead_h, dead, sizeof(dead_h), hipMemcpyDeviceToHost, stream_));
                HIP_TRY(hipStreamSynchronize(stream_));
                sweep_launches_total_ += 1.0;
                rc = maybe_collect_timing();
                if (rc) return rc;
                if (!dead_h) { done = lp.passes; break; }
                sweep_aborts_total_ += 1.0;
                int least = lp.passes;
                bool any = false;
                for (int b = 0; b < nprob; b++)
                    if (h_state_[b].active) { any = true; least = std::min(least, h_state_[b].passes); }
                if (!any) break;
                done = std::max(done, std::min(least, lp.passes - 1));
                n = std::min(chunk, lp.passes - done);
            }
        }
        for (int j = 0; j < n; j++) {
            int nblocks = 1, e0 = -1;
            if (profiling_) { e0 = next_event_pair(); HIP_TRY(hipEventRecord(ev_[e0], stream_)); }
            bool fused = false, solved_in_fold = false;
            if (use_grid_) {
                FoldArgs fa{};
                fused = fused_fold_ != 0 && !tshard_;
                const int lanes = pass_lanes(nprob);
                if (fused) {
                    rc = make_fold(grid_launch_blocks(ns_, lanes, reduce_max_blocks()), nprob,
                                   st->stats, (long long)(sizeof(DevIcpState) / sizeof(double)), nullptr, 0, &fa);
                    if (rc) return rc;
                    if (ipc_n_ > 1) add_ipc(&fa);
                    if (solve_in_fold(lp, lanes, nprob)) fa.solve = st;
                }
                solved_in_fold = fused && fa.solve != nullptr;
                HIP_TRY(launch_nn_grid_reduce((const float4 *)d_src_, ns_, search_sorted(),
                                              (const unsigned *)d_start_, grid_, (const float4 *)d_nrm_,
                                              T32_, T64, nullptr, r2f_, plane, (int32_t *)d_idx_,
                                              (float *)d_d2_, (double *)d_partials_,
                                              reduce_max_blocks(), &nblocks, lanes,
                                              profiling_ ? (unsigned long long *)d_cand_ : nullptr, st,
                                              nprob, loop_out_stride_, stream_, f64_src(), f64_sorted(), r2d_, (const Pt64 *)d_nrm64_,
                                              exact_ ? 1 : 0, fused ? &fa : nullptr, tshard_ ? shard_d64() : nullptr,
                                              (Pt64 *)d_pos_, cert_enabled_ ? 1 : (1 | 8), nullptr, nullptr, nprob == 1 ? ru_state() : nullptr,
                                              ring_table()));
                last_kernel_ = pass_kernel(lanes);
                pos_fresh_ = d_pos_ != nullptr;
                prev_T_valid_ = false;
                if (tshard_) {
                    rc = shard_exchange_on_stream(st, plane, &nblocks);
                    if (rc) return rc;
                }
            } else {
                HIP_TRY(launch_nn_brute((const float4 *)d_src_, ns_, (const float4 *)d_tgt_, nt_pad_,
                                        T32_, r2f_, (unsigned long long *)d_keys_, ns_pad_, plan_, st,
                                        stream_, brute_exact() ? (const Pt64 *)d_src64_ : nullptr, nullptr,
                                        brute_exact() ? (float *)d_second_ : nullptr));
            }
            if (profiling_) { HIP_TRY(hipEventRecord(ev_[e0 + 1], stream_)); pending_.push_back({e0, 0}); }
            if (profiling_) { e0 = next_event_pair(); HIP_TRY(hipEventRecord(ev_[e0], stream_)); }
            if (!use_grid_) {
                HIP_TRY(launch_reduce((const float4 *)d_src_, ns_, (const float4 *)d_tgt_,
                                      (const float4 *)d_nrm_, (const unsigned long long *)d_keys_,
                                      plan_.tgt_splits, ns_pad_, T32_, T64, nullptr, r2f_, plane,
                                      (int32_t *)d_idx_, (float *)d_d2_, (double *)d_partials_,
                                      reduce_max_blocks(), nullptr, st, &nblocks, stream_, nullptr, 0, bex_ptr()));
            }
            if (ipc_n_ > 1) {
                if (!fused) HIP_TRY(launch_finalize_state((const double *)d_partials_, nblocks, st, plane, stream_));
                if (!(fused && use_grid_))
                    HIP_TRY(launch_ipc_allreduce(st->stats, st->stats, peers_, ipc_rank_, ipc_n_, ipc_seq_dev(), nullptr, 0,
                                                 (int *)d_ipc_flag_, stream_));
                HIP_TRY(launch_solve_state(st, 1, stream_));
            } else if (comm_) {
                if (!fused) HIP_TRY(launch_finalize_state((const double *)d_partials_, nblocks, st, plane, stream_));
                int nrc = g_rccl.AllReduce(st->stats, st->stats, kNStats, kNcclFloat64, kNcclSum, comm_, stream_);
                if (nrc != 0) {
                    err_ = std::string("ncclAllReduce: ") + (g_rccl.GetErrorString ? g_rccl.GetErrorString(nrc) : "error");
                    return VISMA_ICP_ERR_RCCL;
                }
                HIP_TRY(launch_solve_state(st, 1, stream_));
            } else if (fused) {
                if (!solved_in_fold) HIP_TRY(launch_solve_state(st, nprob, stream_));
            } else {
                HIP_TRY(launch_finalize_solve((const double *)d_partials_, nblocks, st, plane, nprob, stream_));
            }
            if (profiling_) { HIP_TRY(hipEventRecord(ev_[e0 + 1], stream_)); pending_.push_back({e0, 1}); }
        }
        done += n;
        HIP_TRY(hipMemcpyAsync(h_state_, d_state_, sizeof(DevIcpState) * nprob, hipMemcpyDeviceToHost, stream_));
        int ipc_flag = 0;
        if (ipc_n_ > 1) HIP_TRY(hipMemcpyAsync(&ipc_flag, d_ipc_flag_, sizeof(int), hipMemcpyDeviceToHost, stream_));
        HIP_TRY(hipStreamSynchronize(stream_));
        if (ipc_flag) {
            err_ = "all-reduce: rank " + std::to_string(ipc_flag - 1) + " never delivered its statistics";
            return VISMA_ICP_ERR_HIP;
        }
        rc = maybe_collect_timing();
        if (rc) return rc;
        bool any = false;
        for (int b = 0; b < nprob; b++) any = any || h_state_[b].active;
        if (!any) break;
    }
    for (int b = 0; b < nprob; b++) {
        const DevIcpState &h = h_state_[b];
        out[b].Tc = Mat4::identity();
        for (int i = 0; i < 12; i++) out[b].Tc.m[i] = h.Tc[i];
        out[b].fit = h.fit; out[b].rmse = h.rmse;
        out[b].k = (int64_t)std::llround(h.K);
        out[b].iters = h.iter; out[b].passes = h.passes;
    }
    for (int i = 0; i < 12; i++) T32_.m[i] = (float)h_state_[0].Tc[i];
    have_pass_ = true;
    grid_pending_ = false;
    brute_reduced_ = true;
    return VISMA_ICP_OK;
}

int HipEngine::run_loop_batch(const LoopParams &lp, const std::vector<BatchProblem> &pb, LoopResult *out)
{
    HIP_TRY(hipSetDevice(device_));
    if (sess_live_) { int src = end_session(); if (src) return src; }
    const int B = (int)pb.size();
    if (B < 1) return VISMA_ICP_OK;
    if (comm_) { err_ = "batched loop is single-GPU"; return VISMA_ICP_ERR_STATE; }
    last_was_batch_ = true;
    StageTrace tr("batch/engine");
    std::vector<ProbDesc> descs((size_t)B);
// ... 296 lines not shown
```

visma_amd/csrc/kernels.h:

```cpp
#pragma once

#include <hip/hip_runtime.h>
#include <stdint.h>
#include <vector>

namespace visma {

constexpr int kBlock = 256;
constexpr int kSptLarge = 8;
constexpr int kSptSmall = 2;
constexpr int kSTile = kBlock * kSptLarge;
constexpr int kTChunk = 512;
constexpr int kSub = 64;
constexpr int kReduceAcc = 29;
constexpr int kNStats = 38;

struct Xform32 { float m[12]; };
struct Xform64 { double m[12]; };
struct Offset64 { double v[3]; };
struct Pt64 {
    double x, y, z;
    unsigned long long w;
};

// ... 139 lines not shown
                                     const DevIcpState *st = nullptr);
hipError_t launch_publish_stats(const double *stats, double *host_out, unsigned long long seq,
                                hipStream_t stream);

hipError_t launch_finalize(const double *partials, int nblocks, int point_to_plane,
                           double *stats_out, hipStream_t stream, double *host_out = nullptr,
                           unsigned long long seq = 0);
hipError_t launch_finalize_solve(const double *partials, int nblocks, DevIcpState *st, int plane,
                                 int nprob, hipStream_t stream);
hipError_t launch_finalize_state(const double *partials, int nblocks, DevIcpState *st, int plane,
                                 hipStream_t stream);
hipError_t launch_solve_state(DevIcpState *st, int nprob, hipStream_t stream);


struct GridParams {
    float mn[3];
    float h, inv_h;
    int dim[3];
    int sub;
    float hs, inv_hs;
    int ring;
    int64_t ncell;
};
static_assert(sizeof(GridParams) == 56, "GridParams is a kernel argument of every search kernel");
struct RingRow { short dy, dz; float base; };
struct RingTable { const RingRow *rows; int nrows; };
constexpr int kRingMaxRings = 64;
constexpr int64_t kGridMaxCells = 64ll * 1024 * 1024;
constexpr int64_t kGridMaxCellsFine = 256ll * 1024 * 1024;
constexpr int kGridMaxDim = 2048;

struct ProbDesc {
    long long src_off, sorted_off, start_off, out_off;
    int ns, first_block, nblocks, pad_;
    GridParams g;
};

#ifdef VISMA_WITH_TILE
struct TileArgs {
    const Pt64 *src64;
    int ns;
    const float4 *sorted;
    const Pt64 *sorted64;
    const unsigned *start;
    GridParams g;
    const float4 *nrm;
    const Pt64 *nrm64;
    Xform64 T64;
    Offset64 off;
    float r2f;
    int *idx_out;
    float *d2_out;
    double *partials;
    double *partials2;
    unsigned *tickets;
    int ticket_stride;
    double *stats_out;
    long long stats_stride;
    double *host_out;
    unsigned long long seq;
    unsigned long long *stats;
    const DevIcpState *st;
    int bpp;
    long long out_stride;
    const ProbDesc *descs;
    int nprob;
    int force_fallback;
};
int tile_threads(int config);
hipError_t launch_nn_tile_reduce(const TileArgs &a, int point_to_plane, int config, int total_blocks,
                                 hipStream_t stream);
#endif
hipError_t launch_promote_pt64(const float4 *src, Pt64 *dst, int64_t n, hipStream_t stream);
size_t order_source_scratch_bytes(int64_t n);
hipError_t order_source_device(const double *d_xyz, int64_t n, const double c[3], float4 *d_src, Pt64 *d_src64,
                               int32_t *d_order, void *scratch, size_t scratch_bytes, hipStream_t stream);
hipError_t launch_expand_f64(const double *xyz, int64_t n, const double c[3], float4 *f4, Pt64 *p8, hipStream_t stream,
                             int64_t index0 = 0);
hipError_t launch_expand_f32(const float *xyz, int64_t n, int64_t index0, const double c[3], float4 *f4, Pt64 *p8,
                             hipStream_t stream);

hipError_t launch_grid_bbox(const float4 *tgt, int64_t nt, unsigned *box6, hipStream_t stream);
hipError_t launch_pack12(const float4 *src, float *dst, int64_t n, hipStream_t stream);
void grid_decode_bbox(const unsigned box6[6], float mn[3], float mx[3]);
GridParams grid_plan(const float mn[3], const float mx[3], double max_dist, int64_t max_cells, int max_sub = 1);
GridParams grid_plan_ring(const float mn[3], const float mx[3], double max_dist, double cell, int64_t max_cells);
int grid_scan_blocks(int64_t ncell);

hipError_t point_mesh_distance_device(const double *h_P, int64_t np, const double *h_V, int64_t nv,
                                      const int32_t *h_F, int64_t nf, int method, double *h_d2, int32_t *h_face,
                                      double *h_closest, float *kernel_ms, float *build_ms, hipStream_t stream);
hipError_t sample_mesh_transformed_device(const double *h_V, int64_t nv, const int32_t *h_F, int64_t nf, int64_t n,
                                          int quirks, unsigned long long seed, const double *T16, double *d_out,
                                          int64_t room, int64_t *m_out, hipStream_t stream);
hipError_t sample_mesh_device(const double *h_V, int64_t nv, const int32_t *h_F, int64_t nf, int64_t n,
                              int quirks, unsigned long long seed, const double *h_uniforms,
                              double *h_out, int64_t *n_out, hipStream_t stream);
hipError_t surface_distances_device(const double *h_Vs, int64_t nvs, const int32_t *h_Fs, int64_t nfs,
                                    const double *h_Vt, int64_t nvt, const int32_t *h_Ft, int64_t nft, int64_t n,
                                    int quirks, unsigned long long seed, int method, double *h_dist,
                                    int64_t *n_out, float *kernel_ms, float *build_ms, hipStream_t stream);

constexpr int kNormalsMaxList = 170;
hipError_t estimate_normals_device(const double *h_xyz, int64_t n, const double *h_nrm_in, int search_type,
                                   int knn, double radius, double *h_out, hipStream_t stream);

hipError_t voxel_down_sample_device(const double *h_xyz, const double *h_nrm, const double *h_col,
                                    int64_t n, double voxel, double *h_out_xyz, double *h_out_nrm,
                                    double *h_out_col, int64_t *n_out, int *too_fine,
                                    hipStream_t stream);
hipError_t voxel_down_sample_core(const double *d_xyz, const double *d_nrm, const double *d_col, int64_t n, double voxel,
                                  double **d_oxyz_out, double **d_onrm_out, double **d_ocol_out, int64_t *n_out,
                                  int *too_fine, hipStream_t stream);
hipError_t centroid_device(const double *d_xyz, int64_t n, int64_t chunk, double *d_part, double *d_out, hipStream_t stream);
size_t exclusive_scan_u32_tmp_bytes(long long n);
hipError_t launch_exclusive_scan_u32_lib(const unsigned *in, long long n, unsigned *out, void *tmp, size_t tmp_bytes,
                                         hipStream_t stream);
hipError_t launch_grid_build(const float4 *tgt, int64_t nt, const GridParams &g,
                             unsigned *cell_of, unsigned *count, unsigned *bsum,
                             unsigned *start, float4 *sorted, hipStream_t stream,
                             const Pt64 *tgt64 = nullptr, Pt64 *sorted64 = nullptr);
hipError_t launch_nn_grid_reduce(const float4 *src, int64_t ns, const float4 *sorted,
                                 const unsigned *start, const GridParams &g,
                                 const float4 *tgt_normals, const Xform32 &T32, const Xform64 &T64,
                                 const double frame_offset[3], float r2f, int point_to_plane,
                                 int32_t *idx_out, float *d2_out, double *partials,
                                 int max_partial_blocks, int *nblocks_out, int lanes_per_query,
                                 unsigned long long *cand_count, const DevIcpState *st,
                                 int nprob, int64_t out_stride, hipStream_t stream,
                                 const Pt64 *src64 = nullptr, const Pt64 *sorted64 = nullptr,
                                 double r2d = 0.0, const Pt64 *nrm64 = nullptr, int exact = 0,
                                 const FoldArgs *fold = nullptr, double *d64_out = nullptr,
                                 Pt64 *wst_io = nullptr, int warm = 0, const Xform64 *Tprev = nullptr,
                                 const PersistArgs *persist = nullptr, Pt64 *ru_io = nullptr,
                                 const RingTable *ring = nullptr);
constexpr int kCoopLanes = 9901;
hipError_t launch_nn_wave(int total_blocks, int bpp, int nprob, const ProbDesc *descs, int ns, const float *s12,
                          const unsigned *start, const GridParams &g, const float4 *nrm, const Pt64 *nrm64,
                          const Xform64 &T64, const Offset64 &off, float r2f, int point_to_plane, int one,
                          int32_t *idx_out, float *d2_out, double *partials, unsigned long long *cand_count,
                          const DevIcpState *st, long long out_stride, const Pt64 *src64, const Pt64 *sorted64,
                          const FoldArgs &fold, double *d64_out, Pt64 *prevq_io, int warm, hipStream_t stream);
struct SweepArgs {
    unsigned long long *relay;
    unsigned long long *dead;
    int max_passes;
    unsigned tag0;
    int passes0;
    long long wait_ticks;
};
hipError_t launch_nn_ring(int lanes, int nblocks, int nprob, int ns, const Pt64 *src64, const Pt64 *sorted64, const float *s12, const unsigned *start,
                          const GridParams &g, const RingTable &tab, const float4 *nrm, const Pt64 *nrm64, const Xform64 &T64, const Offset64 &off,
                          float r2f, int point_to_plane, int32_t *idx_out, float *d2_out, double *d64_out, Pt64 *state_io,
                          int warm, double *partials, unsigned long long *cand_count, const DevIcpState *st,
                          long long out_stride, const FoldArgs &fold, hipStream_t stream);
hipError_t build_ring_table(int rings, void **d_tab, int *nrows);
std::vector<RingRow> ring_visiting_order(int rings);
hipError_t launch_count_occupied(const unsigned *count, int64_t n, unsigned long long *out, hipStream_t stream);
int nn_wave_sweep_capacity();
hipError_t launch_nn_wave_sweep(int bpp, int nprob, int ns, const float *s12, const unsigned *start, const GridParams &g,
                                float r2f, int32_t *idx_out, float *d2_out, double *partials, unsigned long long *cand_count,
                                DevIcpState *st, long long out_stride, const Pt64 *src64, const Pt64 *sorted64,
                                const FoldArgs &fold, Pt64 *prevq_io, const SweepArgs &sa, hipStream_t stream);

hipError_t launch_nn_coop(int total_blocks, int bpp, int nprob, const ProbDesc *descs, int ns, const float *s12,
                          const unsigned *start, const GridParams &g, const float4 *nrm, const Pt64 *nrm64,
                          const Xform64 &T64, const Offset64 &off, float r2f, int point_to_plane, int one,
                          int32_t *idx_out, float *d2_out, double *partials, unsigned long long *cand_count,
                          const DevIcpState *st, long long out_stride, const Pt64 *src64, const Pt64 *sorted64,
                          const FoldArgs &fold, double *d64_out, Pt64 *wst_io, int warm, hipStream_t stream,
                          const Xform64 *Tprev = nullptr, const PersistArgs *persist = nullptr, Pt64 *ru_io = nullptr);
int coop_persist_capacity(int point_to_plane);
hipError_t launch_nn_grid_reduce_batch(const float4 *src, const float4 *sorted, const unsigned *start,
                                       const ProbDesc *descs, int nprob, int total_blocks,
                                       int32_t *idx_out, float *d2_out, double *partials,
                                       int lanes_per_query, int one_per_lane, const DevIcpState *st,
                                       hipStream_t stream, const Pt64 *src64 = nullptr,
                                       const Pt64 *sorted64 = nullptr, int exact = 0,
                                       const FoldArgs *fold = nullptr, unsigned long long *cand_count = nullptr,
                                       const float4 *nrm = nullptr, const Pt64 *nrm64 = nullptr,
                                       Pt64 *wst_io = nullptr, int warm = 0);
hipError_t launch_finalize_solve_batch(const double *partials, const ProbDesc *descs, DevIcpState *st,
                                       int nprob, hipStream_t stream, int plane = 0);

hipError_t launch_fill_inf(float4 *dst, int64_t n, hipStream_t stream);
hipError_t launch_pack_float4(const float *src, int stride, float4 *dst, int64_t n,
                              hipStream_t stream);

hipError_t launch_so3_selftest(const double *w, double *R, double *w2, int n,
                               hipStream_t stream);
hipError_t launch_se3_selftest(const double *g, const double *h, const double *v, int n, double *gh, double *gv,
                               double *gi, hipStream_t stream);
hipError_t launch_so3_selftest_jac(const double *w, int n, double *R, double *dR, double *w2, double *dw, double *proj,
                                   hipStream_t stream);

}
```

Measured before the change: 54110 ICP iterations/s.

## Encode sorted target points as packed 21-bit fixed-point words for coop search

Adds a compact 8-byte per-point encoding of the sorted target, storing three 21-bit quantised coordinates relative to the grid origin with a power-of-two step. The cooperative NN kernel now reads these words instead of 12-byte float triples. It computes distances in the quantised frame with a widened tolerance band so exact rescoring still yields the true nearest neighbour. The inner loop is restructured from octet-per-query DPP reductions to per-thread vector loads. This is meant to cut candidate-fetch bandwidth, but it adds a pack kernel at target setup, gates the coop path on the encoding fitting, and loosens the candidate filter band, which may admit more candidates for exact refinement.

```diff
diff --git a/include/visma_icp_testing.h b/include/visma_icp_testing.h
--- a/include/visma_icp_testing.h
+++ b/include/visma_icp_testing.h
@@ -31,6 +31,12 @@
                                            double *cell_out, int *rings);
 VISMA_ICP_API int visma_icp_ring_visiting_order(int rings, int capacity, short *dy, short *dz, float *base, int *nrows);
 
+VISMA_ICP_API int visma_icp_compact_encode(const float mn[3], const float mx[3], double max_dist, const double *xyz, int64_t n,
+                                           uint64_t *words, int *e, int *fits);
+VISMA_ICP_API int visma_icp_compact_distance(const float mn[3], const float mx[3], double max_dist, const uint64_t *words, int64_t n,
+                                             const double q[3], float r, float *d2, float *E);
+VISMA_ICP_API int visma_icp_compact_exp_device(const float mn[3], const float mx[3], double max_dist, int *e);
+
 VISMA_ICP_API int visma_icp_get_tile_config(int *s_tile, int *t_chunk, int *block);
 VISMA_ICP_API int visma_icp_get_launch_config(visma_icp_ctx *ctx, int *src_tiles,
                                               int *tgt_splits);
diff --git a/visma_amd/csrc/compact_target.h b/visma_amd/csrc/compact_target.h
--- /dev/null
+++ b/visma_amd/csrc/compact_target.h
@@ -0,0 +1,81 @@
+#pragma once
+
+#include <math.h>
+
+#include "kernels.h"
+
+namespace visma {
+
+constexpr int kCompactBits = 21;
+constexpr unsigned kCompactMask = (1u << kCompactBits) - 1u;
+constexpr double kCompactBias = 65536.0;
+constexpr int kCompactExpMin = -60, kCompactExpMax = 60;
+
+__host__ __device__ inline int compact_exp(const GridParams &g)
+{
+    const float ext = fmaxf(fmaxf((float)g.dim[0] * g.h, (float)g.dim[1] * g.hs), (float)g.dim[2] * g.hs);
+    const unsigned b = __builtin_bit_cast(unsigned, ext);
+    const int be = (int)((b >> 23) & 0xFFu);
+    if (be == 0xFF) return kCompactExpMax;
+    if (be == 0) return kCompactExpMin;
+    int e = be - 147;
+    if ((b & 0x7FFFFFu) + 0x800000u > 15u * (1u << 20)) e++;
+    return e < kCompactExpMin ? kCompactExpMin : (e > kCompactExpMax ? kCompactExpMax : e);
+}
+
+__host__ __device__ inline float compact_pow2f(int k) { return __builtin_bit_cast(float, (unsigned)(k + 127) << 23); }
+__host__ __device__ inline double compact_pow2(int k)
+{
+    return __builtin_bit_cast(double, (unsigned long long)(k + 1023) << 52);
+}
+
+inline bool compact_fits(const GridParams &g, const float mn[3], const float mx[3])
+{
+    const int e = compact_exp(g);
+    const double step = compact_pow2(e);
+    for (int k = 0; k < 3; k++) {
+        const double slack = 1.2e-7 * fmax(fabs((double)mn[k]), fabs((double)mx[k]));
+        const double lo = ((double)mn[k] - slack - (double)g.mn[k]) / step + kCompactBias;
+        const double hi = ((double)mx[k] + slack - (double)g.mn[k]) / step + kCompactBias;
+        if (!(lo >= 1.0) || !(hi <= (double)kCompactMask - 1.0)) return false;
+    }
+    return true;
+}
+
+__host__ __device__ inline unsigned long long compact_encode(double x, double y, double z, const GridParams &g, int e)
+{
+    const double s = compact_pow2(-e);
+    const double p[3] = {x, y, z};
+    unsigned long long w = 0ull;
+    for (int k = 0; k < 3; k++) {
+        double t = rint((p[k] - (double)g.mn[k]) * s) + kCompactBias;
+        t = t > 0.0 ? (t < (double)kCompactMask ? t : (double)kCompactMask) : 0.0;
+        w |= (unsigned long long)(unsigned)t << (kCompactBits * k);
+    }
+    return w;
+}
+
+__host__ __device__ inline void compact_query(double x, double y, double z, const GridParams &g, double sinv, float q[3])
+{
+    q[0] = (float)((x - (double)g.mn[0]) * sinv + kCompactBias);
+    q[1] = (float)((y - (double)g.mn[1]) * sinv + kCompactBias);
+    q[2] = (float)((z - (double)g.mn[2]) * sinv + kCompactBias);
+}
+
+__host__ __device__ inline float compact_d2(unsigned long long w, float qx, float qy, float qz)
+{
+    const float dx = (float)(unsigned)(w & kCompactMask) - qx;
+    const float dy = (float)(unsigned)((w >> kCompactBits) & kCompactMask) - qy;
+    const float dz = (float)(unsigned)(w >> (2 * kCompactBits)) - qz;
+    float d = dx * dx;
+    d += dy * dy;
+    d += dz * dz;
+    return d;
+}
+
+__host__ __device__ inline float compact_band(float step, float qx, float qy, float qz, float rup)
+{
+    return step * (0.87f + 6e-8f * (fabsf(qx) + fabsf(qy) + fabsf(qz))) + 4.8e-7f * rup;
+}
+
+}
diff --git a/visma_amd/csrc/driver.cpp b/visma_amd/csrc/driver.cpp
--- a/visma_amd/csrc/driver.cpp
+++ b/visma_amd/csrc/driver.cpp
@@ -2,6 +2,7 @@
 #ifdef VISMA_TEST_SEAMS
 #include "../../include/visma_icp_testing.h"
 #endif
+#include "compact_target.h"
 
 namespace {
 
@@ -1054,6 +1055,46 @@
     return VISMA_ICP_OK;
 }
 
+int visma_icp_compact_encode(const float mn[3], const float mx[3], double max_dist, const double *xyz, int64_t n, uint64_t *words, int *e,
+                             int *fits)
+{
+    if (!mn || !mx || n < 0 || (n > 0 && (!xyz || !words))) return VISMA_ICP_ERR_INVALID;
+    const visma::GridParams g = visma::grid_plan(mn, mx, max_dist, visma::kGridMaxCells);
+    const int ge = visma::compact_exp(g);
+    for (int64_t i = 0; i < n; i++) words[i] = visma::compact_encode(xyz[3 * i], xyz[3 * i + 1], xyz[3 * i + 2], g, ge);
+    if (e) *e = ge;
+    if (fits) *fits = visma::compact_fits(g, mn, mx) ? 1 : 0;
+    return VISMA_ICP_OK;
+}
+
+int visma_icp_compact_distance(const float mn[3], const float mx[3], double max_dist, const uint64_t *words, int64_t n, const double q[3],
+                               float r, float *d2, float *E)
+{
+    if (!mn || !mx || !q || n < 0 || (n > 0 && (!words || !d2))) return VISMA_ICP_ERR_INVALID;
+    const visma::GridParams g = visma::grid_plan(mn, mx, max_dist, visma::kGridMaxCells);
+    const int ge = visma::compact_exp(g);
+    float qc[3];
+    visma::compact_query(q[0], q[1], q[2], g, visma::compact_pow2(-ge), qc);
+    const float s2 = visma::compact_pow2f(2 * ge);
+    for (int64_t i = 0; i < n; i++) d2[i] = visma::compact_d2(words[i], qc[0], qc[1], qc[2]) * s2;
+    const float r2f = r * r;
+    if (E) *E = visma::compact_band(visma::compact_pow2f(ge), qc[0], qc[1], qc[2], sqrtf(r2f) * (1.0f + 2.4e-7f));
+    return VISMA_ICP_OK;
+}
+
+int visma_icp_compact_exp_device(const float mn[3], const float mx[3], double max_dist, int *e)
+{
+    if (!mn || !mx || !e) return VISMA_ICP_ERR_INVALID;
+    const visma::GridParams g = visma::grid_plan(mn, mx, max_dist, visma::kGridMaxCells);
+    int *d = nullptr;
+    if (hipMalloc(&d, sizeof(int)) != hipSuccess) { (void)hipGetLastError(); return VISMA_ICP_ERR_ENGINE; }
+    hipError_t err = visma::launch_compact_exp(g, d, nullptr);
+    if (err == hipSuccess) err = hipMemcpy(e, d, sizeof(int), hipMemcpyDeviceToHost);
+    (void)hipFree(d);
+    if (err != hipSuccess) { (void)hipGetLastError(); return VISMA_ICP_ERR_ENGINE; }
+    return VISMA_ICP_OK;
+}
+
 int visma_icp_ring_visiting_order(int rings, int capacity, short *dy, short *dz, float *base, int *nrows)
 {
     const std::vector<visma::RingRow> rows = visma::ring_visiting_order(rings);
diff --git a/visma_amd/csrc/grid.hip b/visma_amd/csrc/grid.hip
--- a/visma_amd/csrc/grid.hip
+++ b/visma_amd/csrc/grid.hip
@@ -1,4 +1,5 @@
 #include "device_common.h"
+#include "compact_target.h"
 
 #include <stdlib.h>
 #include <algorithm>
@@ -177,6 +178,28 @@
 hipError_t launch_pack12(const float4 *src, float *dst, int64_t n, hipStream_t stream)
 {
     if (n > 0) hipLaunchKernelGGL(pack12_kernel, dim3((unsigned)((n + 255) / 256)), dim3(256), 0, stream, src, dst, (long long)n);
+    return hipGetLastError();
+}
+
+__global__ void pack_compact_kernel(const Pt64 *__restrict__ src, unsigned long long *__restrict__ dst, long long n,
+                                    long long slack, GridParams g)
+{
+    const long long i = (long long)blockIdx.x * blockDim.x + threadIdx.x;
+    const int e = compact_exp(g);
+    if (i < n) { const Pt64 p = src[i]; dst[i] = compact_encode(p.x, p.y, p.z, g, e); }
+    else if (i < n + slack) dst[i] = 0ull;
+}
+hipError_t launch_pack_compact(const Pt64 *sorted64, unsigned long long *dst, int64_t n, const GridParams &g, hipStream_t stream)
+{
+    const long long tot = (long long)n + kSortedSlack;
+    hipLaunchKernelGGL(pack_compact_kernel, dim3((unsigned)((tot + 255) / 256)), dim3(256), 0, stream, sorted64, dst, (long long)n,
+                       (long long)kSortedSlack, g);
+    return hipGetLastError();
+}
+__global__ void compact_exp_kernel(GridParams g, int *e) { if (threadIdx.x == 0) *e = compact_exp(g); }
+hipError_t launch_compact_exp(const GridParams &g, int *e, hipStream_t stream)
+{
+    hipLaunchKernelGGL(compact_exp_kernel, dim3(1), dim3(64), 0, stream, g, e);
     return hipGetLastError();
 }
 
@@ -879,7 +902,7 @@
                                  int nprob, int64_t out_stride, hipStream_t stream, const Pt64 *src64,
                                  const Pt64 *sorted64, double r2d, const Pt64 *nrm64, int exact,
                                  const FoldArgs *fold, double *d64_out, Pt64 *prevq_io, int warm, const Xform64 *Tprev,
-                                 const PersistArgs *persist, Pt64 *ru_io, const RingTable *ring)
+                                 const PersistArgs *persist, Pt64 *ru_io, const RingTable *ring, const unsigned long long *c8)
 {
     if ((src64 == nullptr) != (sorted64 == nullptr)) return hipErrorInvalidValue;
     if (persist && !(lanes_per_query == kCoopLanes && src64 && exact && g.sub == 1 && prevq_io)) return hipErrorInvalidValue;
@@ -907,7 +930,7 @@
             hipError_t e = launch_nn_coop(nblocks * nprob, nblocks, nprob, nullptr, (int)ns, (const float *)sorted, start, g,
                                           tgt_normals, nrm64, T64, off, r2f, point_to_plane, one ? 1 : 0, idx_out, d2_out,
                                           partials, cand_count, st, (long long)out_stride, src64, sorted64, fa, d64_out,
-                                          prevq_io, warm, stream, Tprev, persist, ru_io);
+                                          prevq_io, warm, stream, Tprev, persist, ru_io, c8);
             if (nblocks_out) *nblocks_out = nblocks;
             return e;
         }
diff --git a/visma_amd/csrc/grid_coop.hip b/visma_amd/csrc/grid_coop.hip
--- a/visma_amd/csrc/grid_coop.hip
+++ b/visma_amd/csrc/grid_coop.hip
@@ -1,5 +1,6 @@
 #include <cstdlib>
 
+#include "compact_target.h"
 #include "device_common.h"
 #include "grid_coop_probe.h"
 
@@ -7,7 +8,6 @@
 
 namespace {
 
-struct P12 { float x, y, z; };
 #ifndef VISMA_COOP_RU
 #define VISMA_COOP_RU 0
 #endif
@@ -16,28 +16,14 @@
 #endif
 constexpr bool kCoopRu = VISMA_COOP_RU != 0;
 constexpr int kCoopCap = VISMA_COOP_CAP;
-#ifndef VISMA_COOP_DEPTH
-#define VISMA_COOP_DEPTH 7
+#ifndef VISMA_COOP_CDEPTH
+#define VISMA_COOP_CDEPTH 1
 #endif
-constexpr int kCoopDepth = VISMA_COOP_DEPTH;
+constexpr int kCoopCDepth = VISMA_COOP_CDEPTH;
 #ifndef VISMA_COOP_ROOM
 #define VISMA_COOP_ROOM 0.04f
 #endif
 constexpr float kCoopRoom = VISMA_COOP_ROOM;
-
-__device__ __forceinline__ float octet_min(float d)
-{
-    float r;
-    asm volatile("s_nop 1\n\t"
-                 "v_min_f32_dpp %0, %1, %1 quad_perm:[1,0,3,2] row_mask:0xf bank_mask:0xf\n\t"
-                 "s_nop 1\n\t"
-                 "v_min_f32_dpp %0, %0, %0 quad_perm:[2,3,0,1] row_mask:0xf bank_mask:0xf\n\t"
-                 "s_nop 1\n\t"
-                 "v_min_f32_dpp %0, %0, %0 row_half_mirror row_mask:0xf bank_mask:0xf"
-                 : "=&v"(r)
-                 : "v"(d));
-    return r;
-}
 
 __device__ __forceinline__ unsigned pack_sec(float sec, float third, unsigned lane)
 {
@@ -85,7 +71,7 @@
 
 template <bool PLANE, bool ONE, int NTH, bool PERSIST = false>
 __device__ __forceinline__ bool coop_body(
-    int ns, const float *__restrict__ s12f, const unsigned *__restrict__ start, GridParams g,
+    int ns, const unsigned long long *__restrict__ c8, const unsigned *__restrict__ start, GridParams g,
     const float4 *__restrict__ nrm, Xform64 T64, Offset64 off, float r2f, int *__restrict__ idx_out,
     float *__restrict__ d2_out, double *__restrict__ partials, unsigned long long *__restrict__ cand_count,
     const DevIcpState *__restrict__ st, int bpp, long long out_stride, const ProbDesc *__restrict__ descs,
@@ -95,7 +81,6 @@
     const CoopRes res = CoopRes{})
 {
     constexpr int NACC = Acc<PLANE>::N;
-    const P12 *s12 = reinterpret_cast<const P12 *>(s12f);
     int prob, lb;
     long long row0;
     if (descs) {
@@ -114,7 +99,7 @@
         bpp = d.nblocks;
         src64 += d.src_off;
         ns = d.ns;
-        s12 += d.sorted_off;
+        c8 += d.sorted_off;
         sorted64 += d.sorted_off;
         if constexpr (PLANE) {
             if (nrm) nrm += d.sorted_off;
@@ -158,7 +143,6 @@
     for (int a = 0; a < NACC; a++) acc[a] = 0.0;
 
     const int tid = thread_number<PERSIST, NTH>(), lane = tid & 63, wave = tid >> 6;
-    const int oct = lane >> 3, l8 = lane & 7;
     constexpr int NW = NTH / 64;
     constexpr unsigned kCapAll = (unsigned)(NW * kCoopCap);
     int vb, per_group;
@@ -478,15 +462,18 @@
                 const float px = (float)pxd, py = (float)pyd, pz = (float)pzd;
                 COOP_MARK(0);
                 const float rup = sqrtf(r2f) * (1.0f + 2.4e-7f);
-                const float E = 2.4e-7f * (fabsf(px) + fabsf(py) + fabsf(pz) + rup) + 4.8e-7f * rup;
+                const float E0 = 2.4e-7f * (fabsf(px) + fabsf(py) + fabsf(pz) + rup) + 4.8e-7f * rup;
+                const int ce = compact_exp(g);
+                float qc[3];
+                compact_query(pxd, pyd, pzd, g, compact_pow2(-ce), qc);
+                const float E = compact_band(compact_pow2f(ce), qc[0], qc[1], qc[2], rup);
                 const float tlim = rup + 2.0f * E;
                 const float L = tlim * tlim * (1.0f + 6e-7f);
-                const float W = (4.0f * E * tlim + 4.0f * E * E) * (1.0f + 1e-6f) + L * 5e-7f;
-                s_qp[tid] = make_float4(px, py, pz, W);
+                s_qp[tid] = make_float4(qc[0], qc[1], qc[2], E * compact_pow2f(-ce));
                 float bound0 = L;
                 if (dprev < L) bound0 = dprev;
                 unsigned looked;
-                list_rows(px, py, pz, E, bound0, sact, xb, xe, lbgeo2, looked);
+                list_rows(px, py, pz, E0 + 0.5f * E, bound0, sact, xb, xe, lbgeo2, looked);
                 asm volatile("" : "+v"(lbgeo2));
                 if (cand_count) {
                     unsigned long long c = 0, ca = looked;
@@ -555,43 +542,63 @@
                 __syncthreads();
                 set_phase_prio(2);
                 const unsigned mw = min(m_all - w0, kCapAll);
-                for (unsigned tb = 0; tb < mw; tb += (unsigned)(NW * 8 * kCoopDepth)) {
-                    const unsigned t = tb + (unsigned)(wave * 8 + oct);
-                    P12 c4[kCoopDepth];
-                    unsigned meta[kCoopDepth];
-#pragma unroll
-                    for (int u = 0; u < kCoopDepth; u++) {
-                        const unsigned c = t + (unsigned)(u * NW * 8);
-                        uint2 dsc = make_uint2(0u, 0u);
-                        if (c < mw) dsc = s_item[c];
-                        meta[u] = dsc.y;
-                        c4[u] = *reinterpret_cast<const P12 *>(reinterpret_cast<const char *>(s12) + (((dsc.x * 3u) << 2) + (unsigned)l8 * 12u));
-                    }
-#pragma unroll
-                    for (int u = 0; u < kCoopDepth; u++) {
-                        const unsigned c = t + (unsigned)(u * NW * 8);
-                        const unsigned cnt = meta[u] >> 16;
-                        const float4 p = *reinterpret_cast<const float4 *>(reinterpret_cast<const char *>(s_qp) + (meta[u] & 0xFFF0u));
-                        float d = sqdist_f32(make_float4(c4[u].x, c4[u].y, c4[u].z, 0.f), p.x, p.y, p.z);
-                        const bool mine = (unsigned)l8 < cnt;
-                        d = mine ? d : INFINITY;
-                        const float m = octet_min(d);
-                        const bool fl = d <= m + p.w;
-                        const unsigned long long bal = __builtin_amdgcn_ballot_w64(fl);
-                        const unsigned flags = (unsigned)(bal >> (oct * 8)) & 0xFFu;
-                        const float dn = fl ? INFINITY : d;
-                        const float sec = octet_min(dn);
+                const int ce = compact_exp(g);
+                const float s2 = compact_pow2f(2 * ce);
+                typedef unsigned long long u2a __attribute__((ext_vector_type(2), aligned(8)));
+                for (unsigned tb = 0; tb < mw; tb += (unsigned)(NTH * kCoopCDepth)) {
+                    uint2 dsc[kCoopCDepth];
+                    u2a v[kCoopCDepth][4];
+#pragma unroll
+                    for (int u = 0; u < kCoopCDepth; u++) {
+                        const unsigned c = tb + (unsigned)(u * NTH + tid);
+                        dsc[u] = make_uint2(0u, 0u);
+                        if (c < mw) dsc[u] = s_item[c];
+                        const unsigned cnt = dsc[u].y >> 16;
+                        const char *rec = reinterpret_cast<const char *>(c8) + (dsc[u].x << 3);
+#pragma unroll
+                        for (int k = 0; k < 4; k++) {
+                            v[u][k] = u2a{0ull, 0ull};
+                            if ((unsigned)(2 * k) < cnt) v[u][k] = *reinterpret_cast<const u2a *>(rec + 16 * k);
+                        }
+                    }
+#pragma unroll
+                    for (int u = 0; u < kCoopCDepth; u++) {
+                        const unsigned c = tb + (unsigned)(u * NTH + tid);
+                        const unsigned cnt = dsc[u].y >> 16;
+                        const float4 p = *reinterpret_cast<const float4 *>(reinterpret_cast<const char *>(s_qp) + (dsc[u].y & 0xFFF0u));
+                        float d[8];
+                        float m = INFINITY;
+#pragma unroll
+                        for (int j = 0; j < 8; j++) {
+                            d[j] = (unsigned)j < cnt ? compact_d2(v[u][j >> 1][j & 1], p.x, p.y, p.z) : INFINITY;
+                            m = fminf(m, d[j]);
+                        }
+                        const float Wm = (4.0f * p.w * sqrtf(m) + 4.0f * p.w * p.w) * (1.0f + 1e-6f) + m * 5e-7f;
+                        const float lim = m + Wm;
+                        unsigned flags = 0u;
+                        float sec = INFINITY;
+#pragma unroll
+                        for (int j = 0; j < 8; j++) {
+                            const bool fl = d[j] <= lim;
+                            flags |= fl ? 1u << j : 0u;
+                            sec = fminf(sec, fl ? INFINITY : d[j]);
+                        }
                         unsigned secl = 0u;
                         float third = INFINITY;
                         if constexpr (kCoopRu) {
-                            const unsigned long long bs = __builtin_amdgcn_ballot_w64(dn == sec && sec < INFINITY);
-                            const unsigned b8 = (unsigned)(bs >> (oct * 8)) & 0xFFu;
-                            secl = b8 ? (unsigned)__builtin_ctz(b8) : 0u;
-                            third = octet_min((b8 != 0u && (unsigned)l8 == secl) ? INFINITY : dn);
-                        }
-                        if (l8 == 0 && mine) {
-                            s_item[c].y = (__float_as_uint(m) & 0xFFFFFF00u) | flags;
-                            s_sec[c] = pack_sec(sec, third, secl);
+                            bool seen = false;
+#pragma unroll
+                            for (int j = 0; j < 8; j++) {
+                                const bool fl = (flags >> j) & 1u;
+                                const bool is_sec = !fl && !seen && sec < INFINITY && d[j] == sec;
+                                secl = is_sec ? (unsigned)j : secl;
+                                third = (fl || is_sec) ? third : fminf(third, d[j]);
+                                seen = seen || is_sec;
+                            }
+                        }
+                        if (cnt != 0u) {
+                            s_item[c].y = (__float_as_uint(m * s2) & 0xFFFFFF00u) | flags;
+                            s_sec[c] = pack_sec(sec * s2, third * s2, secl);
                         }
                     }
                 }
@@ -627,12 +634,19 @@
                 double bd = r2d;
                 unsigned bidx = 0xFFFFFFFFu, bpos = 0xFFFFFFFFu;
                 Pt64 bq = Pt64{0.0, 0.0, 0.0, 0ull};
-                auto tail = [&](const double pxd, const double pyd, const double pzd, const float px, const float py, const float pz,
-                                const float W) {
+                auto tail = [&](const double pxd, const double pyd, const double pzd, const float px, const float py, const float pz) {
                 const float rup = sqrtf(r2f) * (1.0f + 2.4e-7f);
-                const float E = 2.4e-7f * (fabsf(px) + fabsf(py) + fabsf(pz) + rup) + 4.8e-7f * rup;
+                const float E0 = 2.4e-7f * (fabsf(px) + fabsf(py) + fabsf(pz) + rup) + 4.8e-7f * rup;
+                const int ce = compact_exp(g);
+                float E;
+                {
+                    float qc[3];
+                    compact_query(pxd, pyd, pzd, g, compact_pow2(-ce), qc);
+                    E = compact_band(compact_pow2f(ce), qc[0], qc[1], qc[2], rup);
+                }
                 const float tlim = rup + 2.0f * E;
                 const float L = tlim * tlim * (1.0f + 6e-7f);
+                const float W = (4.0f * E * tlim + 4.0f * E * E) * (1.0f + 1e-6f) + L * 5e-7f;
                 auto rank = [&](const Pt64 &c8, unsigned pos) {
                     const double dx = c8.x - pxd, dy = c8.y - pyd, dz = c8.z - pzd;
                     double d = dx * dx;
@@ -696,15 +710,18 @@
                     };
                     const float qx = bcast_f(px), qy = bcast_f(py), qz = bcast_f(pz);
                     const double qxd = bcast_d(pxd), qyd = bcast_d(pyd), qzd = bcast_d(pzd);
-                    const float qrup = rup, qE = bcast_f(E);
+                    const float qrup = rup, qE = bcast_f(E), qE0 = bcast_f(E0);
+                    float qc[3];
+                    compact_query(qxd, qyd, qzd, g, compact_pow2(-ce), qc);
                     const float sl = fminf(sqrtf(bcast_f(g_up)), qrup) + 2.0f * qE;
                     const float Ls = sl * sl * (1.0f + 6e-7f);
+                    const float Ls_steps = Ls * compact_pow2f(-2 * ce);
                     unsigned qb[9], pre[10];
                     pre[0] = 0u;
                     {
                         unsigned sb[9], se[9], looked_unused;
                         float geo_unused;
-                        list_rows(px, py, pz, E, Ls, lane == q, sb, se, geo_unused, looked_unused);
+                        list_rows(qx, qy, qz, qE0 + 0.5f * qE, Ls, lane == q, sb, se, geo_unused, looked_unused);
         #pragma unroll
                         for (int k = 0; k < 9; k++) {
                             qb[k] = bcast_u(sb[k]);
@@ -717,7 +734,7 @@
                     for (unsigned f0 = 0; f0 < pre[9]; f0 += 128u) {
                         unsigned j[2];
                         bool in[2];
-                        P12 t[2];
+                        unsigned long long t[2];
         #pragma unroll
                         for (int u = 0; u < 2; u++) {
                             const unsigned f = f0 + (unsigned)u * 64u + (unsigned)lane;
@@ -727,13 +744,13 @@
                             for (int k = 0; k < 9; k++)
                                 if (f >= pre[k] && f < pre[k + 1]) jj = qb[k] + (f - pre[k]);
                             j[u] = jj;
-                            t[u] = P12{0.f, 0.f, 0.f};
-                            if (in[u]) t[u] = s12[jj];
+                            t[u] = 0ull;
+                            if (in[u]) t[u] = c8[jj];
                         }
                         Pt64 c8[2];
         #pragma unroll
                         for (int u = 0; u < 2; u++) {
-                            in[u] = in[u] && sqdist_f32(make_float4(t[u].x, t[u].y, t[u].z, 0.f), qx, qy, qz) <= Ls;
+                            in[u] = in[u] && compact_d2(t[u], qc[0], qc[1], qc[2]) <= Ls_steps;
                             c8[u] = Pt64{0.0, 0.0, 0.0, 0ull};
                             if (in[u]) c8[u] = sorted64[j[u]];
                         }
@@ -779,7 +796,7 @@
                 if (need) {
                     float lb2 = fminf(lbgeo2, fminf(gh1, gsec));
                     if (bpos == 0xFFFFFFFFu) lb2 = fminf(lb2, gh0);
-                    float lb = sqrtf(lb2) * (1.0f - 1e-6f) - 4.0f * E;
+                    float lb = sqrtf(lb2) * (1.0f - 1e-6f) - (4.0f * E0 + E);
                     if (slow || n > 1) lb = 0.f;
                     lb_new = fminf(fmaxf(lb, 0.f), 3.0e38f);
 #ifdef VISMA_COOP_LB_PROBE
@@ -799,7 +816,7 @@
                     const long long i = (long long)(vb * NTH + (int)s_home[tid]) * per_group + it;
                     emit(i, (unsigned)s_home[tid], false, bd, bidx, found, bq.x, bq.y, bq.z, lb_new);
                     if constexpr (kCoopRu) {
-                        const float lb3 = sqrtf(lb3_2) * (1.0f - 1e-6f) - 4.0f * E;
+                        const float lb3 = sqrtf(lb3_2) * (1.0f - 1e-6f) - (4.0f * E0 + E);
                         const bool have = found && rupos != 0xFFFFFFFFu && !(slow || n > 1) && lb3 > 0.f && lb_new > 0.f;
                         if (ru_io) s_item[s_home[tid]] = make_uint2(have ? rupos : 0xFFFFFFFFu, __float_as_uint(fminf(lb3, 3.0e38f)));
                     }
@@ -811,11 +828,10 @@
                     s_dprev[h] = __uint_as_float(found ? bidx : 0xFFFFFFFFu);
                 }
                 };
-                const float4 me = s_qp[tid];
                 const unsigned h = s_home[tid];
                 double hq[3];
                 query_p(h, hq);
-                tail(hq[0], hq[1], hq[2], me.x, me.y, me.z, me.w);
+                tail(hq[0], hq[1], hq[2], (float)hq[0], (float)hq[1], (float)hq[2]);
                 COOP_MARK(11);
             }
         }
@@ -872,7 +888,7 @@
 }
 
 #define VISMA_COOP_PARAMS                                                                                         \
-    int ns, const float *__restrict__ s12f, const unsigned *__restrict__ start, GridParams g,                    \
+    int ns, const unsigned long long *__restrict__ c8, const unsigned *__restrict__ start, GridParams g,         \
         const float4 *__restrict__ nrm, Xform64 T64, Offset64 off, float r2f, int *__restrict__ idx_out,         \
         float *__restrict__ d2_out, double *__restrict__ partials, unsigned long long *__restrict__ cand_count,  \
         const DevIcpState *__restrict__ st, int bpp, long long out_stride, const ProbDesc *__restrict__ descs,   \
@@ -880,7 +896,7 @@
         const Pt64 *__restrict__ nrm64, const FoldArgs fold, double *__restrict__ d64_out,                       \
         Pt64 *__restrict__ wst_io, int warm, Xform64 Tprev, Pt64 *__restrict__ ru_io
 #define VISMA_COOP_ARGS                                                                                          \
-    ns, s12f, start, g, nrm, T64, off, r2f, idx_out, d2_out, partials, cand_count, st, bpp, out_stride, descs,   \
+    ns, c8, start, g, nrm, T64, off, r2f, idx_out, d2_out, partials, cand_count, st, bpp, out_stride, descs,   \
         nprob, src64, sorted64, nrm64, fold, d64_out, wst_io, warm, Tprev, ru_io
 template <bool PLANE>
 __global__ __launch_bounds__(kBlock) __attribute__((amdgpu_waves_per_eu(4, 4))) void nn_coop_kernel_one(VISMA_COOP_PARAMS)
@@ -938,7 +954,7 @@
 }
 
 struct CoopPersistParams {
-    int ns; const float *s12f; const unsigned *start; GridParams g; const float4 *nrm; Xform64 T64; Offset64 off; float r2f;
+    int ns; const unsigned long long *c8; const unsigned *start; GridParams g; const float4 *nrm; Xform64 T64; Offset64 off; float r2f;
     int *idx_out; float *d2_out; double *partials; unsigned long long *cand_count; int bpp; const Pt64 *src64;
     const Pt64 *sorted64; const Pt64 *nrm64; FoldArgs fold; Pt64 *wst_io; int warm; Xform64 Tprev; PersistArgs pa;
     Pt64 *ru_io;
@@ -1026,7 +1042,7 @@
         f.rows_tagged = VISMA_KARG(fold.rows_tagged); f.rows2_tagged = VISMA_KARG(fold.rows2_tagged);
         f.dead_flag = VISMA_KARG(fold.dead_flag); f.poll_ticks = VISMA_KARG(fold.poll_ticks);
         const bool published = coop_body<PLANE, true, kBlock, true>(
-            VISMA_KARG(ns), VISMA_KARG(s12f), VISMA_KARG(start), VISMA_KARG(g), VISMA_KARG(nrm), Tc, VISMA_KARG(off), VISMA_KARG(r2f),
+            VISMA_KARG(ns), VISMA_KARG(c8), VISMA_KARG(start), VISMA_KARG(g), VISMA_KARG(nrm), Tc, VISMA_KARG(off), VISMA_KARG(r2f),
             VISMA_KARG(idx_out), VISMA_KARG(d2_out), VISMA_KARG(partials), VISMA_KARG(cand_count), nullptr, VISMA_KARG(bpp), 0ll,
             nullptr, 1, VISMA_KARG(src64), VISMA_KARG(sorted64), VISMA_KARG(nrm64), f, nullptr, VISMA_KARG(wst_io), w, Tp,
             VISMA_KARG(ru_io), t_begin ? &work : nullptr, CoopRes{r_q64, r_idx, r_lb, r_lb3, pass == 1 ? 1 : 0, nsx, nsy, nsz,
@@ -1107,7 +1123,7 @@
 #undef VISMA_COOP_ARGS
 
 #define VISMA_COOP_LAUNCH(KERNEL_)                                                                               \
-    hipLaunchKernelGGL(KERNEL_, dim3(total_blocks), dim3(kBlock), 0, stream, ns, s12, start, g, nrm, T64, off,   \
+    hipLaunchKernelGGL(KERNEL_, dim3(total_blocks), dim3(kBlock), 0, stream, ns, c8, start, g, nrm, T64, off,    \
                        r2f, idx_out, d2_out, partials, cand_count, st, bpp, out_stride, descs, nprob, src64,     \
                        sorted64, nrm64, fold, d64_out, wst_io, warm, Tp, ru_io)
 
@@ -1117,9 +1133,10 @@
                           int32_t *idx_out, float *d2_out, double *partials, unsigned long long *cand_count,
                           const DevIcpState *st, long long out_stride, const Pt64 *src64, const Pt64 *sorted64,
                           const FoldArgs &fold, double *d64_out, Pt64 *wst_io, int warm, hipStream_t stream,
-                          const Xform64 *Tprev, const PersistArgs *persist, Pt64 *ru_io)
+                          const Xform64 *Tprev, const PersistArgs *persist, Pt64 *ru_io, const unsigned long long *c8)
 {
     if (!src64 || !sorted64 || !s12 || !wst_io) return hipErrorInvalidValue;
+    if (!c8 && !descs) return hipErrorInvalidValue;
     if (persist) {
         if (fold.solve) return hipErrorInvalidValue;
         if (descs || nprob != 1 || !one || st || !fold.rows_tagged || !fold.rows2_tagged || !fold.dead_flag || !fold.host_out ||
@@ -1128,7 +1145,7 @@
             total_blocks > coop_persist_capacity(point_to_plane))
             return hipErrorInvalidValue;
         CoopPersistParams P{};
-        P.ns = ns; P.s12f = s12; P.start = start; P.g = g; P.nrm = nrm; P.T64 = T64; P.off = off; P.r2f = r2f;
+        P.ns = ns; P.c8 = c8; P.start = start; P.g = g; P.nrm = nrm; P.T64 = T64; P.off = off; P.r2f = r2f;
         P.idx_out = idx_out; P.d2_out = d2_out; P.partials = partials; P.cand_count = cand_count; P.bpp = bpp;
         P.src64 = src64; P.sorted64 = sorted64; P.nrm64 = nrm64; P.fold = fold; P.wst_io = wst_io;
         if (Tprev) { P.Tprev = *Tprev; warm |= 4; } else warm &= ~4;
@@ -1141,7 +1158,7 @@
         const char *e = std::getenv("VISMA_ICP_COOP_KERNEL");
         return !e ? 0 : (e[0] == 'c' ? 1 : (e[0] == 'w' ? 2 : 0));
     }();
-    if (forced == 2 || (forced == 0 && (descs || nprob > 1)))
+    if (forced == 2 || (forced == 0 && (descs || nprob > 1)) || !c8)
         return launch_nn_wave(total_blocks, bpp, nprob, descs, ns, s12, start, g, nrm, nrm64, T64, off, r2f, point_to_plane, one,
                               idx_out, d2_out, partials, cand_count, st, out_stride, src64, sorted64, fold, d64_out, wst_io,
                               warm & (3 | 8), stream);
diff --git a/visma_amd/csrc/hip_engine.hpp b/visma_amd/csrc/hip_engine.hpp
--- a/visma_amd/csrc/hip_engine.hpp
+++ b/visma_amd/csrc/hip_engine.hpp
@@ -15,7 +15,7 @@
         if (comm_) g_rccl.CommDestroy(comm_);
         for (int r = 0; r < ipc_n_; r++)
             if (r != ipc_rank_ && peers_.box[r]) (void)hipIpcCloseMemHandle(peers_.box[r]);
-        free_dev(d_mbox_); free_dev(d_ipc_flag_); free_dev(d_raw_); free_dev(d_sorted12_); free_dev(bt_sorted12_);
+        free_dev(d_mbox_); free_dev(d_ipc_flag_); free_dev(d_raw_); free_dev(d_sorted12_); free_dev(d_compact_); free_dev(bt_sorted12_);
         free_dev(d_pend_count_); free_dev(d_pend_q32_); free_dev(d_pend_q64_); free_dev(d_pend_best_); free_dev(d_pend_idx_);
         for (hipEvent_t e : ev_) (void)hipEventDestroy(e);
         free_dev(d_src_); free_dev(d_tgt_); free_dev(d_nrm_); free_dev(d_keys_); free_dev(d_gkeys_);
@@ -108,6 +108,12 @@
     {
         if (exact_ && d_src64_ && d_sorted64_ && d_sorted12_) return (const float4 *)d_sorted12_;
         return (const float4 *)d_sorted_;
+    }
+    void *d_compact_ = nullptr;
+    bool compact_ok_ = false;
+    const unsigned long long *search_compact() const
+    {
+        return (exact_ && d_src64_ && d_sorted64_ && d_compact_ && compact_ok_) ? (const unsigned long long *)d_compact_ : nullptr;
     }
     int set_clouds64(const Pt64 *src, const Pt64 *tgt) override
     {
@@ -503,7 +509,8 @@
     }
     bool coop_ok() const
     {
-        return coop_enabled_ && exact_ && d_src64_ && d_sorted64_ && d_sorted12_ && d_pos_ && grid_.sub == 1 && grid_.ring == 0 &&
+        return coop_enabled_ && exact_ && d_src64_ && d_sorted64_ && d_sorted12_ && search_compact() && d_pos_ && grid_.sub == 1 &&
+               grid_.ring == 0 &&
                (nt_ + kSortedSlack) * 12 < (1ll << 32);
     }
     int pass_kernel(int lanes) const { return grid_.ring > 0 ? 3 : ((lanes == kCoopLanes && coop_ok()) ? 2 : 1); }
diff --git a/visma_amd/csrc/hip_engine_clouds.cpp b/visma_amd/csrc/hip_engine_clouds.cpp
--- a/visma_amd/csrc/hip_engine_clouds.cpp
+++ b/visma_amd/csrc/hip_engine_clouds.cpp
@@ -1,4 +1,5 @@
 #include "hip_engine.hpp"
+#include "compact_target.h"
 
 namespace visma {
 namespace drv {
@@ -618,6 +619,14 @@
             if (prc) return prc;
             HIP_TRY(launch_pack12((const float4 *)d_sorted_, (float *)d_sorted12_, nt_, stream_));
         }
+        free_dev(d_compact_);
+        compact_ok_ = false;
+        if (d_sorted64_) {
+            int prc = pool_alloc(&d_compact_, sizeof(unsigned long long) * (size_t)(nt_ + kSortedSlack));
+            if (prc) return prc;
+            HIP_TRY(launch_pack_compact((const Pt64 *)d_sorted64_, (unsigned long long *)d_compact_, nt_, grid_, stream_));
+            compact_ok_ = compact_fits(grid_, mn, mx);
+        }
         return VISMA_ICP_OK;
     };
     {
diff --git a/visma_amd/csrc/hip_engine_passes.cpp b/visma_amd/csrc/hip_engine_passes.cpp
--- a/visma_amd/csrc/hip_engine_passes.cpp
+++ b/visma_amd/csrc/hip_engine_passes.cpp
@@ -327,7 +327,7 @@
                                   prof ? (unsigned long long *)d_cand_ : nullptr, nullptr,
                                   1, 0, stream_, f64_src(), f64_sorted(), r2d_, (const Pt64 *)d_nrm64_,
                                   exact_ ? 1 : 0, fused ? &fa : nullptr, shard_d64(), (Pt64 *)d_pos_, 1 | (persist ? persist_prio_ << 5 : 0), cert_prev(), persist, ru_state(),
-                                  ring_table()));
+                                  ring_table(), search_compact()));
     if (!early) {
         last_kernel_ = pass_kernel(lanes);
         pos_fresh_ = d_pos_ != nullptr;
@@ -491,7 +491,7 @@
                                       (float *)d_d2_, (double *)d_partials_, reduce_max_blocks(),
                                       &nblocks, (last_kernel_ = pass_kernel(pass_lanes()), pass_lanes()), nullptr, nullptr, 1, 0, stream_,
                                       f64_src(), f64_sorted(), r2d_, (const Pt64 *)d_nrm64_, exact_ ? 1 : 0,
-                                      nullptr, nullptr, (Pt64 *)d_pos_, 1, cert_prev(), nullptr, ru_state(), ring_table()));
+                                      nullptr, nullptr, (Pt64 *)d_pos_, 1, cert_prev(), nullptr, ru_state(), ring_table(), search_compact()));
         pos_fresh_ = d_pos_ != nullptr;
         note_state_pass(T64);
         grid_pending_ = false;
@@ -682,7 +682,7 @@
                                               nprob, loop_out_stride_, stream_, f64_src(), f64_sorted(), r2d_, (const Pt64 *)d_nrm64_,
                                               exact_ ? 1 : 0, fused ? &fa : nullptr, tshard_ ? shard_d64() : nullptr,
                                               (Pt64 *)d_pos_, cert_enabled_ ? 1 : (1 | 8), nullptr, nullptr, nprob == 1 ? ru_state() : nullptr,
-                                              ring_table()));
+                                              ring_table(), search_compact()));
                 last_kernel_ = pass_kernel(lanes);
                 pos_fresh_ = d_pos_ != nullptr;
                 prev_T_valid_ = false;
diff --git a/visma_amd/csrc/kernels.h b/visma_amd/csrc/kernels.h
--- a/visma_amd/csrc/kernels.h
+++ b/visma_amd/csrc/kernels.h
@@ -245,6 +245,8 @@
 
 hipError_t launch_grid_bbox(const float4 *tgt, int64_t nt, unsigned *box6, hipStream_t stream);
 hipError_t launch_pack12(const float4 *src, float *dst, int64_t n, hipStream_t stream);
+hipError_t launch_pack_compact(const Pt64 *sorted64, unsigned long long *dst, int64_t n, const GridParams &g, hipStream_t stream);
+hipError_t launch_compact_exp(const GridParams &g, int *e, hipStream_t stream);
 void grid_decode_bbox(const unsigned box6[6], float mn[3], float mx[3]);
 GridParams grid_plan(const float mn[3], const float mx[3], double max_dist, int64_t max_cells, int max_sub = 1);
 GridParams grid_plan_ring(const float mn[3], const float mx[3], double max_dist, double cell, int64_t max_cells);
@@ -296,7 +298,7 @@
                                  const FoldArgs *fold = nullptr, double *d64_out = nullptr,
                                  Pt64 *wst_io = nullptr, int warm = 0, const Xform64 *Tprev = nullptr,
                                  const PersistArgs *persist = nullptr, Pt64 *ru_io = nullptr,
-                                 const RingTable *ring = nullptr);
+                                 const RingTable *ring = nullptr, const unsigned long long *c8 = nullptr);
 constexpr int kCoopLanes = 9901;
 hipError_t launch_nn_wave(int total_blocks, int bpp, int nprob, const ProbDesc *descs, int ns, const float *s12,
                           const unsigned *start, const GridParams &g, const float4 *nrm, const Pt64 *nrm64,
@@ -332,7 +334,8 @@
                           int32_t *idx_out, float *d2_out, double *partials, unsigned long long *cand_count,
                           const DevIcpState *st, long long out_stride, const Pt64 *src64, const Pt64 *sorted64,
                           const FoldArgs &fold, double *d64_out, Pt64 *wst_io, int warm, hipStream_t stream,
-                          const Xform64 *Tprev = nullptr, const PersistArgs *persist = nullptr, Pt64 *ru_io = nullptr);
+                          const Xform64 *Tprev = nullptr, const PersistArgs *persist = nullptr, Pt64 *ru_io = nullptr,
+                          const unsigned long long *c8 = nullptr);
 int coop_persist_capacity(int point_to_plane);
 hipError_t launch_nn_grid_reduce_batch(const float4 *src, const float4 *sorted, const unsigned *start,
                                        const ProbDesc *descs, int nprob, int total_blocks,
```

After: 51250 ICP iterations/s, median of 2. 0.947x the previous value.
